# AlterPang/Multi_ORB_SLAM

Measured on AMD Instinct MI355X. Metric: frames/sec (N-cam extract+match), higher is better.
Workload: dtype u8; 1 GPU; configs[1]: one 2-cam 640x480 rig per GPU, 8-level pyramid, 1000 feat/cam; HIP FAST+rBRIEF extract + SearchByProjection + cross-camera Hamming top-2; cams_per_gpu=2, rig_cams=2, rigs=1, width=640, height=480, nfeatures=1000, nlevels=8, frame_unit=one rig timestep (2 cameras)

## Files before the change

### include/orb_debug.h

```cpp
#ifndef ORB_DEBUG_H
#define ORB_DEBUG_H
#include "orbx.h"
#include "orbm.h"
#include "orbf.h"
#include "orbv.h"
#ifdef __cplusplus
extern "C" {
#endif

int orbx_debug_candidates(orbx_extractor* ex, int cam, int level, orb_keypoint* out, int cap, int* n);
int orbx_debug_distribute_octree(const orb_keypoint* in, int n, int min_x, int max_x, int min_y, int max_y,
                                 int n_features, orb_keypoint* out, int cap, int* n_out);
int orbx_debug_last_path(const orbx_extractor* ex);
int orbx_debug_level0_in_place(const orbx_extractor* ex);
int orbx_debug_pyramid_form(const orbx_extractor* ex);
int orbx_debug_pyramid_plan(int tile_w, int tile_h, int split);

int orbm_debug_last_resolve(const orbm_matcher* m, int* out4);
#define ORBM_FORM_NONE 0
#define ORBM_FORM_HOST 1
#define ORBM_FORM_MONO2_ANG 2
#define ORBM_FORM_MONO2 3
#define ORBM_FORM_MONO4_WORKLIST 4
#define ORBM_FORM_MONO4_WAVES 5
#define ORBM_FORM_JACOBI_LDSQ 6
#define ORBM_FORM_JACOBI 7
#define ORBM_FORM_CAMS 8
#define ORBM_FORM_SWEEPS 9
int orbm_debug_last_resolve_form(const orbm_matcher* m, int* out2);
int orbm_debug_last_refresh(const orbm_matcher* m, int* out5);
int orbm_debug_last_pose(const orbm_matcher* m, int* out2);
int orbm_debug_last_sim3(const orbm_matcher* m, int* out2);
int orbm_debug_last_sim3opt(const orbm_matcher* m, int* out2);
int orbm_debug_last_pnp(const orbm_matcher* m, int* out4);
int orbm_debug_pnp_buffers(const orbm_matcher* m, unsigned long long* out3);
int orbm_debug_time_project(orbm_matcher* m, const orbm_frame* f, const orbm_query* q, int nq, int th_high, int iters,
                            float* avg_us, long long* n_gated);

int orbv_debug_last_join(const orbv_workspace* w, int* out4);

int orbf_debug_exchange_timing(orbf_frontend* f, int on);
int orbf_debug_exchange_us(const orbf_frontend* f, float* out2);
long orbf_debug_exchange_redos(const orbf_frontend* f);

#ifdef __cplusplus
}
#endif
#endif
```

### multi_orb_slam_amd/_lib.py

```python
import ctypes as C
import os
import subprocess
import numpy as np

_PKG = os.path.dirname(os.path.abspath(__file__))
CSRC = os.path.join(_PKG, "csrc")
LIB_PATH = os.environ.get("MORB_LIB_PATH") or os.path.join(_PKG, "lib", "libmorb.so")

KP_DTYPE = np.dtype([("x", "<f4"), ("y", "<f4"), ("size", "<f4"), ("angle", "<f4"), ("response", "<f4"),
                     ("octave", "<i4"), ("class_id", "<i4")])
QUERY_DTYPE = np.dtype([("u", "<f4"), ("v", "<f4"), ("radius", "<f4"), ("ur", "<f4"), ("min_level", "<i4"),
                        ("max_level", "<i4"), ("cam", "<i4"), ("blocks", "<i4"), ("angle", "<f4"),
                        ("desc", "u1", (32,))])
WINDOW_DTYPE = np.dtype([("u", "<f4"), ("v", "<f4"), ("radius", "<f4"), ("cam", "<i4"), ("min_level", "<i4"), ("max_level", "<i4")])
assert KP_DTYPE.itemsize == 28 and QUERY_DTYPE.itemsize == 68 and WINDOW_DTYPE.itemsize == 24
POINT_DTYPE = np.dtype([("pos", "<f4", (3,)), ("normal", "<f4", (3,)), ("min_dist", "<f4"), ("max_dist", "<f4"),
                        ("blocks", "<i4"), ("desc", "u1", (32,))])
TRACK_DTYPE = np.dtype([("proj_x", "<f4"), ("proj_y", "<f4"), ("proj_xr", "<f4"), ("view_cos", "<f4"), ("level", "<i4"),
                        ("in_view", "<i4")])
assert POINT_DTYPE.itemsize == 68 and TRACK_DTYPE.itemsize == 24
REFRESH_DTYPE = np.dtype([("desc", "u1", (32,)), ("normal", "<f4", (3,)), ("min_dist", "<f4"), ("max_dist", "<f4"),
                          ("best_obs", "<i4"), ("best_median", "<i4")])
assert REFRESH_DTYPE.itemsize == 60
REFRESH_DESCRIPTOR, REFRESH_NORMAL_DEPTH, REFRESH_CAP = 1, 2, 256
# ... 136 lines not shown


_lib = None


def lib():
    global _lib
    if _lib is not None:
        return _lib
    if not os.path.exists(LIB_PATH):
        raise OrbError(ORB_E_NO_DEVICE, "HIP library %s is not built (run `python -c 'import __graft_entry__ as g; "
                       "g.build()'` or `make -C multi_orb_slam_amd/csrc`); there is no CPU fallback" % LIB_PATH)
    L = C.CDLL(LIB_PATH)
    vp, i32, f32 = C.c_void_p, C.c_int, C.c_float
    L.orb_last_error.restype = C.c_char_p
    L.orbx_tables.argtypes = [vp] * 7
    L.orbx_create.argtypes = [vp, i32, i32, i32, i32, vp]
    L.orbx_destroy.argtypes = [vp]; L.orbx_destroy.restype = None
    L.orbx_extract.argtypes = [vp, i32] + [vp] * 8
    L.orbx_upload.argtypes = [vp, i32, vp, i32, i32, i32]
    L.orbx_upload_device.argtypes = [vp, i32, vp, i32, i32, i32]
    L.orbx_run.argtypes = [vp]
    L.orbx_count.argtypes = [vp, i32]
    L.orbx_download.argtypes = [vp, i32, vp, vp, i32]
    L.orbx_device_keypoints.argtypes = [vp, i32]; L.orbx_device_keypoints.restype = vp
    L.orbx_device_descriptors.argtypes = [vp, i32]; L.orbx_device_descriptors.restype = vp
    L.orbx_stream.argtypes = [vp]; L.orbx_stream.restype = vp
    L.orbx_wait_for_stream.argtypes = [vp, vp]
    L.orbx_bind_output.argtypes = [vp, i32, vp, vp, i32]
    L.orbx_debug_level.argtypes = [vp, i32, i32, vp, i32, vp, vp]
    L.orbx_debug_candidates.argtypes = [vp, i32, i32, vp, i32, vp]
    L.orbx_debug_distribute_octree.argtypes = [vp, i32, i32, i32, i32, i32, i32, vp, i32, vp]
    L.orbx_set_profiling.argtypes = [vp, i32]
    L.orbx_stage_times_us.argtypes = [vp, vp]
    L.orbm_create.argtypes = [i32, vp]
    L.orbm_destroy.argtypes = [vp]; L.orbm_destroy.restype = None
    L.orbm_stream.argtypes = [vp]; L.orbm_stream.restype = vp
    L.orbm_descriptor_distance.argtypes = [vp, vp]
    L.orbm_three_maxima.argtypes = [vp, i32, vp]; L.orbm_three_maxima.restype = None
    L.orbm_hamming_top2.argtypes = [vp, vp, i32, vp, i32, vp, vp, vp]
    L.orbm_use_matrix_cores.argtypes = [i32]
    L.orbm_use_fp4_top2.argtypes = [i32]
    L.orbm_top2_scratch_bytes.argtypes = [i32, i32]; L.orbm_top2_scratch_bytes.restype = C.c_size_t
    L.orbm_hamming_top2_device.argtypes = [vp, i32, vp, i32, vp, vp, vp, vp, vp]
    L.orbm_hamming_matrix.argtypes = [vp, vp, i32, vp, i32, vp]
    L.orbm_hamming_matrix_device.argtypes = [vp, i32, vp, i32, vp, vp]
    L.orbm_frame_create.argtypes = [vp, vp, vp]
    L.orbm_frame_create_resident.argtypes = [vp, vp, vp, vp]
    L.orbm_frame_destroy.argtypes = [vp]; L.orbm_frame_destroy.restype = None
    L.orbm_set_stream.argtypes = [vp, vp]
    L.orbm_wait_for_stream.argtypes = [vp, vp]
    L.orbm_frame_from_device.argtypes = [vp, vp, i32, f32, f32, f32, f32, f32, vp]
    L.orbm_frame_download.argtypes = [vp, vp, vp, vp, vp, vp]
    L.orbm_frame_count.argtypes = [vp]
    L.orbx_debug_last_path.argtypes = [vp]
    L.orbx_debug_level0_in_place.argtypes = [vp]
    L.orbx_debug_pyramid_form.argtypes = [vp]
    L.orbx_debug_pyramid_plan.argtypes = [i32, i32, i32]
    L.orbf_create.argtypes = [vp, i32, i32, i32, i32, vp]
    L.orbf_create_depth.argtypes = [vp, i32, i32, i32, i32, i32, vp]
    L.orbf_destroy.argtypes = [vp]; L.orbf_destroy.restype = None
    L.orbf_set_depth.argtypes = [vp, i32, vp, i32]
    L.orbf_configure.argtypes = [vp, f32, i32, i32]
    L.orbf_step.argtypes = [vp, vp, vp, i32, i32, vp]
    L.orbf_step_motion.argtypes = [vp, vp, vp, i32, vp]
    L.orbf_reset.argtypes = [vp]
    L.orbf_run_stream.argtypes = [vp, vp, i32, i32, i32, i32, vp, vp, i32, C.c_float, vp]
    L.orbf_prefetch.argtypes = [vp, vp]
    L.orbf_step_begin.argtypes = [vp, vp, vp, i32, i32, vp]
    L.orbf_step_motion_begin.argtypes = [vp, vp, vp, i32, vp]
    L.orbf_step_end.argtypes = [vp, vp]
    L.orbm_cross_top2_gathered_enqueue.argtypes = [vp, vp, i32, C.c_size_t, i32, i32, i32, vp, i32]
    L.orbm_cross_top2_gathered_collect.argtypes = [vp, vp, vp, vp, vp, vp]
    L.orbf_export_block.argtypes = [vp, vp, vp, vp]
    L.orbf_exchange_unique_id.argtypes = [vp]
    L.orbf_exchange_init.argtypes = [vp, vp, i32, i32]
    L.orbf_exchange_active.argtypes = [vp]
    L.orbf_step_motion_ahead.argtypes = [vp, vp, vp, vp, i32, i32, f32, vp, vp]
    L.orbf_ahead_depth.argtypes = [vp]
    L.orbf_exchange_placement.argtypes = [vp]
    L.orbf_debug_exchange_timing.argtypes = [vp, C.c_int]
    L.orbf_debug_exchange_us.argtypes = [vp, C.POINTER(C.c_float)]
    L.orbf_debug_exchange_redos.argtypes = [vp]; L.orbf_debug_exchange_redos.restype = C.c_long
    L.orbf_exchange_init_loopback.argtypes = [vp, i32, i32, i32]
    L.orbf_exchange_shutdown.argtypes = [vp]
    L.orbf_exchange_peer_handle_bytes.argtypes = []; L.orbf_exchange_peer_handle_bytes.restype = C.c_size_t
    L.orbf_exchange_peer_export.argtypes = [vp, i32, i32, vp]
    L.orbf_exchange_peer_open.argtypes = [vp, vp]
    L.orbf_peek_block.argtypes = [vp, vp, vp, vp, vp]
    L.orbm_cross_top2_gathered_views.argtypes = [vp, vp, vp, vp]
    L.orbm_cross_top2_gathered.argtypes = [vp, vp, i32, C.c_size_t, i32, i32, i32, vp, vp, vp, vp, vp]
    L.orbf_extractor.argtypes = [vp]; L.orbf_extractor.restype = vp
    L.orbf_matcher.argtypes = [vp]; L.orbf_matcher.restype = vp
    L.orbm_debug_last_resolve.argtypes = [vp, vp]
    L.orbm_debug_last_resolve_form.argtypes = [vp, vp]
    L.orbm_queries_from_motion.argtypes = [vp, vp, vp, vp, i32, f32, f32, f32, vp, f32, vp, vp, vp]
    L.orbm_count_ratio_accepted.argtypes = [vp, vp, i32, i32, f32]
    L.orbm_set_calibration.argtypes = [vp, vp]
    L.orbm_undistort_points.argtypes = [vp, vp, vp, i32, vp, vp]
    L.orbm_image_bounds.argtypes = [vp, i32, i32, vp]
    L.orbf_set_calibration.argtypes = [vp, vp]
    L.orbm_cross_top2.argtypes = [vp, vp, vp, vp, vp]
    L.orbm_cross_top2_blocks.argtypes = [vp, vp, vp, i32, i32, i32, vp, vp, vp]
    L.orbm_frame_grid.argtypes = [vp, vp, vp]
    L.orbm_features_in_area.argtypes = [vp, vp, i32, f32, f32, f32, i32, i32, vp, i32, vp]
    L.orbm_project_candidates.argtypes = [vp, vp, vp, i32, i32, vp, vp, vp]
    L.orbm_project_best.argtypes = [vp, vp, vp, i32, vp, i32, vp, i32, vp, vp]
    L.orbm_search_by_projection.argtypes = [vp, vp, vp, i32, vp, i32, i32, vp, vp]
    L.orbm_search_by_projection_windows.argtypes = [vp, vp, vp, vp, i32, vp, i32, i32, vp, vp]
    L.orbm_debug_time_project.argtypes = [vp, vp, vp, i32, i32, i32, vp, vp]
    L.orbm_search_by_projection_points.argtypes = [vp, vp, vp, i32, vp, f32, i32, vp, vp]
    L.orbm_points_create.argtypes = [vp, i32, vp]
    L.orbm_points_destroy.argtypes = [vp]; L.orbm_points_destroy.restype = None
    L.orbm_points_write.argtypes = [vp, vp, i32, i32, vp]
    L.orbm_points_count.argtypes = [vp]
    L.orbm_search_local_points.argtypes = [vp, vp, vp, i32, vp, vp, vp, f32, i32, vp, vp, vp, vp]
    L.orbm_level_thresholds.argtypes = [f32, i32, vp]
    L.orbm_frustum_host.argtypes = [vp, i32, vp, vp, vp, vp, vp]
    L.orbm_refresh_points.argtypes = [vp, vp, vp]
    L.orbm_refresh_points_host.argtypes = [vp, vp]
    L.orbm_debug_last_refresh.argtypes = [vp, vp]
    L.orbm_pose_optimize.argtypes = [vp, vp, i32, vp, vp, vp, vp, vp, vp, vp]
    L.orbm_pose_optimize_host.argtypes = [vp, i32, vp, vp, vp, vp, vp, i32, vp, vp]
    L.orbm_pose_optimize_resident.argtypes = [vp, vp, vp, vp, vp, vp, vp]
    L.orbm_debug_last_pose.argtypes = [vp, vp]
    L.orbm_pose_sincos.argtypes = [C.c_double, vp, vp]; L.orbm_pose_sincos.restype = None
    L.orbm_sim3_ransac.argtypes = [vp, vp, i32, vp, vp, vp, vp, vp, vp, vp, vp, vp, vp, vp]
    L.orbm_sim3_ransac_host.argtypes = [vp, i32, vp, vp, vp, vp, vp, vp, vp, vp, vp, i32, vp, vp]
    L.orbm_sim3_walk.argtypes = [vp, i32, i32, i32, i32, i32, vp]
    L.orbm_sim3_iterations.argtypes = [C.c_double, i32, i32, i32]
    L.orbm_sim3_atan2.argtypes = [C.c_double, C.c_double]; L.orbm_sim3_atan2.restype = C.c_double
    L.orbm_debug_last_sim3.argtypes = [vp, vp]
    L.orbm_sim3_optimize.argtypes = [vp, vp, i32, vp, vp, vp, vp, vp, vp, vp, vp, vp]
    L.orbm_sim3_optimize_host.argtypes = [vp, i32, vp, vp, vp, vp, vp, vp, vp, i32, vp, vp]
    L.orbm_sim3opt_exp.argtypes = [C.c_double]; L.orbm_sim3opt_exp.restype = C.c_double
    L.orbm_sim3opt_expmap.argtypes = [vp, i32, vp]
    L.orbm_sim3opt_ldlt7.argtypes = [vp, vp, vp]
    L.orbm_debug_last_sim3opt.argtypes = [vp, vp]
    L.orbm_pnp_ransac.argtypes = [vp, vp, i32, vp, vp, vp, vp, vp, vp, vp, vp, vp, vp, vp, i32]
    L.orbm_pnp_ransac_host.argtypes = [vp, i32, vp, vp, vp, vp, vp, vp, vp, vp, vp, vp, vp, i32]
    L.orbm_pnp_walk.argtypes = [vp, i32, i32, vp, vp, i32, i32, i32, i32, i32, vp]
    L.orbm_pnp_parameters.argtypes = [C.c_double, i32, i32, i32, C.c_float, i32, vp, vp]
    L.orbm_pnp_svd.argtypes = [vp, i32, i32, vp, vp, vp]
    L.orbm_pnp_qr_solve.argtypes = [vp, i32, i32, vp, vp]
    L.orbm_pnp_compute_pose.argtypes = [vp, vp, i32, vp, vp, vp, vp]; L.orbm_pnp_compute_pose.restype = C.c_double
    L.orbm_debug_last_pnp.argtypes = [vp, vp]
    L.orbm_debug_pnp_buffers.argtypes = [vp, vp]
    f64 = C.c_double
    L.orbv_create.argtypes = [i32, i32, vp, vp, vp, vp, i32, vp]
    L.orbv_load_text.argtypes = [C.c_char_p, i32, vp]
    L.orbv_destroy.argtypes = [vp]; L.orbv_destroy.restype = None
    L.orbv_info.argtypes = [vp, vp, vp, vp, vp]
    L.orbv_stream.argtypes = [vp]; L.orbv_stream.restype = vp
    L.orbv_transform.argtypes = [vp, vp, i32, i32, vp, vp, vp]
    L.orbv_transform_device.argtypes = [vp, vp, i32, i32, vp, vp, vp]
    L.orbv_bow_vectors.argtypes = [vp, vp, i32, i32, vp, vp, vp, vp, vp, vp, vp]
    L.orbv_score_l1.argtypes = [vp, vp, i32, vp, vp, i32]; L.orbv_score_l1.restype = f64
    L.orbv_workspace_create.argtypes = [i32, vp]
    L.orbv_workspace_destroy.argtypes = [vp]; L.orbv_workspace_destroy.restype = None
    L.orbv_search_by_bow.argtypes = [vp, vp, vp, i32, i32, f32, i32, vp, vp]
    L.orbv_search_for_triangulation.argtypes = [vp, vp, vp, vp, i32, i32, vp, vp]
    L.orbv_debug_last_join.argtypes = [vp, vp]
    L.orbv_keyframe_create.argtypes = [vp, vp, vp]
    L.orbv_keyframe_destroy.argtypes = [vp]; L.orbv_keyframe_destroy.restype = None
    L.orbv_keyframe_count.argtypes = [vp]
    L.orbv_keyframe_from_device.argtypes = [vp, vp, vp, i32, vp, vp]
# ... 29 lines not shown
```

### multi_orb_slam_amd/csrc/extractor.hip

```cpp
#include <algorithm>
#include <cfloat>
#include <cstdlib>
#include <chrono>
#include <atomic>
#include <cmath>
#include <condition_variable>
#include <functional>
#include <memory>
#include <mutex>
#include <thread>
#include <vector>

#include "../../include/orbx.h"
#include "../../include/orb_debug.h"
#include "octree.h"
#include "orb_common.h"
#include "frame_sink.h"

namespace {

using morb::DevBuf;

constexpr int EDGE_THRESHOLD = 19;
constexpr int MIN_BORDER = 16;
// ... 2442 lines not shown
    MORB_ARG(ex != nullptr);
    if (ex->inflight == 0) return ORB_OK;
    MORB_HIP(hipSetDevice(ex->device));
    MORB_HIP(hipEventSynchronize(ex->ev_done[(ex->run_seq - (unsigned)ex->inflight) & 1]));
    return finish_device_path(ex);
}

int orbx_finish_completed(orbx_extractor* ex) {
    MORB_ARG(ex != nullptr);
    if (ex->inflight == 0) return ORB_OK;
    return finish_device_path(ex);
}

int orbx_adopt_stream(orbx_extractor* ex, void* stream) {
    MORB_ARG(ex && stream && ex->inflight == 0);
    MORB_HIP(hipSetDevice(ex->device));
    if (ex->stream) {
        MORB_HIP(hipStreamSynchronize(ex->stream));
        if (ex->stream_owned) (void)hipStreamDestroy(ex->stream);
    }
    ex->stream = static_cast<hipStream_t>(stream); ex->stream_owned = false;
    return ORB_OK;
}

int orbx_discard(orbx_extractor* ex) {
    MORB_ARG(ex != nullptr);
    if (ex->inflight == 0) return ORB_OK;
    MORB_HIP(hipSetDevice(ex->device));
    MORB_HIP(hipEventSynchronize(ex->ev_done[(ex->run_seq - (unsigned)ex->inflight) & 1]));
    --ex->inflight;
    return ORB_OK;
}

int orbx_set_defer_done(orbx_extractor* ex, int on) {
    MORB_ARG(ex != nullptr);
    ex->defer_done = on != 0;
    return ORB_OK;
}

int orbx_record_done(orbx_extractor* ex) {
    MORB_ARG(ex && ex->inflight > 0);
    MORB_HIP(hipSetDevice(ex->device));
    MORB_HIP(hipEventRecord(ex->ev_done[(ex->run_seq - 1u) & 1u], ex->stream));
    return ORB_OK;
}

int orbx_set_inplace_level0(orbx_extractor* ex, int on) {
    MORB_ARG(ex != nullptr);
    if (ex->l0_optin != (on != 0)) { ex->l0_optin = on != 0; ex->tables_dirty = true; }
    return ORB_OK;
}

int orbx_set_pinned_ingest(orbx_extractor* ex, int on) {
    MORB_ARG(ex != nullptr);
    ex->pinned_ingest = on != 0;
    return ORB_OK;
}

int orbx_set_chain_graph(orbx_extractor* ex, int on) {
    MORB_ARG(ex != nullptr);
    ex->graph_next_run = on != 0;
    return ORB_OK;
}

int orbx_set_chain_tail(orbx_extractor* ex, orbx_tail_fn fn, void* user, int tag) {
    MORB_ARG(ex != nullptr);
    ex->tail_fn = fn; ex->tail_user = user; ex->tail_tag = tag;
    return ORB_OK;
}

int orbx_set_frame_sink(orbx_extractor* ex, const FrameSink* sink) {
    MORB_ARG(ex != nullptr && (sink == nullptr || ex->n_cams <= 4));
    if (sink) ex->sink = *sink; else memset(&ex->sink, 0, sizeof(ex->sink));
    return ORB_OK;
}

const int* orbx_device_counts(const orbx_extractor* ex) { return ex ? ex->d_n_out.p + ((ex->run_seq - 1u) & 1u) * (ex->n_cams + 1) : nullptr; }
int orbx_pending(const orbx_extractor* ex) { return ex ? ex->inflight : 0; }
int orbx_peek_status(const orbx_extractor* ex) {
    if (!ex || ex->inflight == 0) return -1;
    const unsigned oldest = (ex->run_seq - (unsigned)ex->inflight) & 1u;
    return ex->h_oct[oldest * (ex->n_cams + 1) + ex->n_cams];
}
void* orbx_done_event(const orbx_extractor* ex) { return ex ? (void*)ex->ev_done[(ex->run_seq - 1u) & 1u] : nullptr; }

static inline const L0Src* l0_table(const orbx_extractor* ex) { return ex->l0_on ? (const L0Src*)ex->d_l0.p : nullptr; }

static int launch_pyramid_fast(orbx_extractor* ex, hipStream_t st, const IngestArgs* fused = nullptr) {
    const int ML = ex->max_levels;
    if (ex->profiling) MORB_HIP(hipEventRecord(ex->ev[0], st));
    if (ex->tiled_ok) {
        PyrArgs A;
        for (int c = 0; c < 64; ++c) {
            A.src[c] = fused && c < ex->n_cams ? fused->src[c] : nullptr; A.stride[c] = fused ? fused->stride[c] : 0;
            A.tx[c] = c < ex->n_cams ? ex->pyr_tx[c] : 0; A.ty[c] = c < ex->n_cams ? ex->pyr_ty[c] : 0;
            A.w[c] = c < ex->n_cams ? (short)ex->cur_w[c] : 0; A.h[c] = c < ex->n_cams ? (short)ex->cur_h[c] : 0;
        }
        hipLaunchKernelGGL(k_pyramid_tiled<256>, dim3(ex->pyr_tx_max, ex->pyr_ty_max, ex->n_cams), dim3(256), (size_t)ex->pyr_lds, st, A,
                           (const LevelInfo*)ex->d_levels.p, ML, ex->d_pyr.p, ex->cam_pitch, (const int2*)ex->d_xtab.p,
                           (const int4*)ex->d_ytab.p, (const int4*)ex->d_pyr_sx.p, (const int4*)ex->d_pyr_sy.p, ex->pyr_tx_max, ex->pyr_ty_max,
                           ex->pyr_tab_cap, ex->pyr_tile);
    } else {
    auto level_dims = [&](int l, int* mw, int* mh) {
        *mw = 0; *mh = 0;
        if (l >= ML) return;
        for (int c = 0; c < ex->n_cams; ++c) {
            const LevelInfo& Lv = ex->levels[(size_t)c * ML + l];
            *mw = std::max(*mw, Lv.w); *mh = std::max(*mh, Lv.h);
        }
    };
    if (ex->tiled4) {
        for (int pi = 0; pi < 2; ++pi) {
            const orbx_extractor::TilePlan& P = ex->tp[pi];
            if (P.last <= P.base || P.tx_max == 0) continue;
            Tile4Args T;
            T.L = (const LevelInfo*)ex->d_levels.p; T.pyr = ex->d_pyr.p; T.cam_pitch = ex->cam_pitch; T.xgrp = (const int4*)ex->d_xgrp.p;
            T.ytab = (const int4*)ex->d_ytab.p; T.sx = (const int4*)P.d_sx.p; T.sy = (const int4*)P.d_sy.p; T.l0 = l0_table(ex);
            T.max_levels = ML; T.base = P.base; T.last = P.last; T.tw = P.tw; T.th = P.th; T.halo_x = P.halo_x; T.halo_y = P.halo_y;
            T.tx_max = P.tx_max; T.ty_max = P.ty_max; T.gcap = P.gcap; T.rcap = P.rcap;
            for (int c = 0; c < 64; ++c) { T.tx[c] = c < ex->n_cams ? P.tx[c] : 0; T.ty[c] = c < ex->n_cams ? P.ty[c] : 0; }
            if (P.threads == 512) hipLaunchKernelGGL(k_pyramid_tiled4<512>, dim3(P.tx_max, P.ty_max, ex->n_cams), dim3(512), (size_t)P.lds, st, T);
            else hipLaunchKernelGGL(k_pyramid_tiled4<256>, dim3(P.tx_max, P.ty_max, ex->n_cams), dim3(256), (size_t)P.lds, st, T);
        }
    } else
    for (int l = 1; l < ML; ++l) {
        int mw = 0, mh = 0;
        level_dims(l, &mw, &mh);
        if (mw == 0) continue;
        dim3 grid((mw + 255) / 256, (mh + 3) / 4, ex->n_cams), block(64, 4, 1);
        hipLaunchKernelGGL(k_resize, grid, block, 0, st, (const LevelInfo*)ex->d_levels.p, ML, l, ex->d_pyr.p, ex->cam_pitch,
                           (const int2*)ex->d_xtab.p, (const int4*)ex->d_ytab.p);
    }
    }
    if (ex->profiling) MORB_HIP(hipEventRecord(ex->ev[1], st));
    static const int form_env = [] { const char* e = getenv("MORB_FAST_FORM"); return e ? atoi(e) : 0; }();
    const bool throughput = form_env ? form_env == 2 : ex->total_cells >= 8192;
    if (throughput)
        hipLaunchKernelGGL((k_fast_cells<128, 8>), dim3(ex->total_cells), dim3(128), fast_cells_lds(ex->cell_h_max, ex->cell_px_max), st,
                           (const LevelInfo*)ex->d_levels.p, (const int2*)ex->d_cell_map.p, (const uint8_t*)ex->d_pyr.p, ex->cam_pitch, ML,
                           ex->d_cell_cnt.p, ex->d_cell_items.p, ex->cell_h_max, ex->cell_px_max, l0_table(ex));
    else
        hipLaunchKernelGGL((k_fast_cells<256, 4>), dim3(ex->total_cells), dim3(256), fast_cells_lds(ex->cell_h_max, ex->cell_px_max), st,
                           (const LevelInfo*)ex->d_levels.p, (const int2*)ex->d_cell_map.p, (const uint8_t*)ex->d_pyr.p, ex->cam_pitch, ML,
                           ex->d_cell_cnt.p, ex->d_cell_items.p, ex->cell_h_max, ex->cell_px_max, l0_table(ex));
    if (ex->profiling) MORB_HIP(hipEventRecord(ex->ev[2], st));
    MORB_HIP(hipGetLastError());
    return ORB_OK;
}

static int launch_tree_describe(orbx_extractor* ex, hipStream_t st, unsigned slot, const FrameSink& sink) {
    const int ML = ex->max_levels;
    int* d_h_oct = ex->d_h_oct + slot * (ex->n_cams + 1);
    MirrorArgs mir;
    mir.kps = nullptr; mir.desc = nullptr;
    if (ex->mirror_kps) { mir.kps = ex->mirror_kps; mir.desc = ex->mirror_desc; }
    for (int c = 0; c < 64; ++c) mir.base[c] = 0;
    hipLaunchKernelGGL(k_octree, dim3(ex->n_cams * ML), dim3(1024), sizeof(OctLdsR), st, (const LevelInfo*)ex->d_levels.p,
                       (const int*)ex->d_cell_cnt.p, (const uint32_t*)ex->d_cell_items.p, ex->d_sel_oct.p, ex->d_sel_cnt.p,
                       ex->d_oct_status.p, ML, ex->oct_max_keys);
    if (ex->profiling) MORB_HIP(hipEventRecord(ex->ev[4], st));
    hipLaunchKernelGGL(k_describe, dim3((ex->total_sel_slots + 3) / 4), dim3(256), 0, st, (const LevelInfo*)ex->d_levels.p, ML,
                       (const uint8_t*)ex->d_pyr.p, ex->cam_pitch, (const SelKp*)ex->d_sel_oct.p, ex->total_sel_slots,
                       (orb_keypoint* const*)ex->d_out_kps.p, (uint8_t* const*)ex->d_out_desc.p, mir,
                       SelListArgs{(const unsigned short*)ex->d_slot_blk.p, (const int*)ex->d_sel_cnt.p,
                                   (const int*)ex->d_oct_status.p, ex->d_n_out.p + slot * (ex->n_cams + 1), d_h_oct, ex->n_cams},
                       sink, l0_table(ex), (const DescribeTables*)ex->d_desc_tabs.p);
// ... 401 lines not shown
```

### multi_orb_slam_amd/csrc/frame_sink.h

```cpp
#pragma once
#include <stdint.h>
#include "../../include/orb_types.h"

struct orbx_extractor;

struct FrameSink {
    float *x, *y, *ur, *depth, *ang;
    int* oct;
    orb_keypoint* kps;
    uint32_t* desc;
    int* cell_of;
    float *h_ur, *h_depth;
    float *h_unx, *h_uny;
    orb_calibration calib;
    const float* cam_depth[4];
    int cam_depth_stride[4];
    float mbf, minX, minY, invW, invH;
};

extern "C" int orbx_set_frame_sink(orbx_extractor* ex, const FrameSink* sink);

extern "C" void* orbx_done_event(const orbx_extractor* ex);
extern "C" int orbx_peek_status(const orbx_extractor* ex);

typedef int (*orbx_tail_fn)(void* user, void* stream);
extern "C" int orbx_set_chain_tail(orbx_extractor* ex, orbx_tail_fn fn, void* user, int tag);
extern "C" int orbx_set_chain_graph(orbx_extractor* ex, int on);
extern "C" int orbx_set_defer_done(orbx_extractor* ex, int on);
extern "C" int orbx_set_pinned_ingest(orbx_extractor* ex, int on);
extern "C" int orbx_set_inplace_level0(orbx_extractor* ex, int on);
extern "C" int orbx_record_done(orbx_extractor* ex);
extern "C" int orbx_finish_completed(orbx_extractor* ex);
extern "C" int orbx_discard(orbx_extractor* ex);
extern "C" int orbx_adopt_stream(orbx_extractor* ex, void* stream);
```

### multi_orb_slam_amd/csrc/frontend.hip

```cpp
#include <algorithm>
#include <atomic>
#include <chrono>
#include <cmath>
#include <cstdarg>
#include <cstdlib>
#include <condition_variable>
#include <mutex>
#include <string>
#include <thread>
#include <vector>

#include "../../include/orbm.h"
#include "orb_common.h"
#include "frame_sink.h"
#include "matcher_internal.h"
#include <deque>
#include "../../include/orbf.h"
#include "../../include/orb_debug.h"

using namespace morb;


struct orbf_frontend {
    int device = 0, n_cams = 0, max_w = 0, max_h = 0;
// ... 10 lines not shown
    float mbf = 40.f;
    int th_high = ORBM_TH_HIGH, check_ori = 1;
    orb_calibration calib = {0, 0, 0, 0, 0, 0, 0, 0, 0};
    int cap_total = 0;
    static constexpr int NSETS = NEX + 3;
    struct ResultSet {
        PinnedBuf<orb_keypoint> kps; PinnedBuf<uint8_t> desc; PinnedBuf<float> ur, depth, unx, uny;
        CrossOut cross;
        bool cross_valid = false;
    } rs[NSETS];
    int last_flags = 0;
    int cur = 0;
    int last_set = 0;
    morb::StageBuf h_queries;
    std::vector<orbm_query> q_host;
    bool motion_on_device = true;
    PinnedBuf<int32_t> h_match;
    orbm_frame* pframe[NSETS] = {};
    int pframe_W[NSETS] = {}, pframe_H[NSETS] = {};
    struct InFlight { std::vector<orbf_image> images; std::vector<uint64_t> fp; int set = 0, W = 0, H = 0, e = 0; bool done = false; };
    std::deque<InFlight> inflight;
    std::deque<std::vector<orbf_image>> announced;
    int last_e = 0;
    bool poll_ok = true;
    static constexpr int NX = 8, NXC = 3;
    struct XSlot {
        DevBuf<uint8_t> recv, list;
        DevBuf<int32_t> gstart;
        PinnedBuf<int32_t> gcnt;
        CrossOut out;
        hipEvent_t done = nullptr, t_done = nullptr;
        long seq = -1;
        long job = 0;
        std::vector<orbf_image> images; std::vector<uint64_t> fp;
    } xs[NX];
    void* xcomm = nullptr; int xworld = 0, xrank = 0;
    void* xc[NXC + 1] = {};
    int x_placement = 0;
    long step_seq = 0, x_next = 0;
    long x_redos = 0;
    long x_spare_until = -1;
    struct XJob { long id, seq; const uint8_t* send; int rows; hipStream_t st; bool redo; };
    std::thread x_thread;
    std::mutex x_mu;
    std::condition_variable x_cv;
    std::deque<XJob> x_jobs;
    long x_pushed = 0, x_issued = 0;
    int x_rc = 0; std::string x_err;
    bool x_quit = false, x_async = false;
    long set_xseq[NEX + 3] = {-1, -1, -1, -1, -1, -1};
    bool x_timing = false; hipEvent_t ev_x[2] = {nullptr, nullptr}; float x_us[2] = {0.f, 0.f};
    bool xloop = false;
    morb::PeerComm* xpeer = nullptr;
    bool x_one_comm = false;
    bool x_broken = false;
    long x_timeout_ms = 15000;
    bool overlap_ok = true;
    int clean_steps = 0;
    struct Pending {
        bool active = false, async_path = false, fr_persistent = false, block_ready = false, cross_from_set = false, forked = false;
        long seq = 0;
        bool seq_taken = false;
        bool inline_match = false;
        bool mirror_requested = false, mirror_pending = false;
        int set = 0, e = 0, W = 0, H = 0, nq = 0, flags = 0, n = 0;
        bool ext_done = false;
        bool use_ms = false; MotionSrc ms; orbf_motion motion;
        bool from_motion = false;
        orbm_frame* fr = nullptr;
        SearchJob J{nullptr, nullptr, 0, nullptr, false, 0.f, 0, 0, 64, false};
        std::vector<orbf_image> images;
        std::vector<orbm_cam_features> cams;
        std::chrono::steady_clock::time_point t_impl, t_enqueued;
    } pending;
    hipEvent_t ev_extracted = nullptr;
    hipEvent_t ev_ready[NSETS] = {};
    hipEvent_t ev_cross[NSETS] = {};
    bool cross_pending[NSETS] = {};
    orbm_frame* last_frame = nullptr; bool last_frame_owned = false;
    int prev_n = 0;
    std::vector<int32_t> prev_cam_of;
    std::vector<float> scale_factors;
    std::chrono::steady_clock::time_point t_entry;
};

static int getenv_int(const char* name, int dflt) { const char* e = getenv(name); return e ? atoi(e) : dflt; }

static bool small_rig(const orbf_frontend* f) { return f->n_cams <= 4 && f->cap_total <= 8192 && !f->mt->host_resolve; }


int orbf_create(const orbx_params* params, int n_cams, int max_width, int max_height, int device, orbf_frontend** out) {
    return orbf_create_depth(params, n_cams, max_width, max_height, device, 0, out);
}

int orbf_create_depth(const orbx_params* params, int n_cams, int max_width, int max_height, int device, int ahead_depth, orbf_frontend** out) {
    MORB_ARG(params && out && n_cams >= 1 && n_cams <= 64 && ahead_depth >= 0 && ahead_depth <= orbf_frontend::NEX);
    orbf_frontend* f = new orbf_frontend();
    f->device = device; f->n_cams = n_cams; f->max_w = max_width; f->max_h = max_height;
    int rc = orbx_create(params, n_cams, max_width, max_height, device, &f->exs[0]);
    f->ex = f->exs[0];
    if (!rc) rc = orbx_set_inplace_level0(f->exs[0], 1);
    if (!rc) rc = orbm_create(device, &f->mt);
    if (rc) { orbf_destroy(f); return rc; }
    f->d_depth.assign(n_cams, nullptr); f->depth_stride.assign(n_cams, 0); f->counts.assign(n_cams, 0);
    { const char* pe = getenv("MORB_POLL"); f->poll_ok = !(pe && atoi(pe) == 0); }
    f->motion_on_device = getenv_int("MORB_MOTION_ON_DEVICE", 1) != 0;
    f->x_timeout_ms = std::max(1L, (long)getenv_int("MORB_EXCHANGE_TIMEOUT_MS", 15000));
    f->scale_factors.assign(params[0].nlevels, 1.f);
    if ((rc = orbx_tables(&params[0], f->scale_factors.data(), nullptr, nullptr, nullptr, nullptr, nullptr))) { orbf_destroy(f); return rc; }
    for (int c = 0; c < n_cams; ++c) { f->cam_cap.push_back(params[c].nfeatures + 4 * params[c].nlevels); f->cap_total += f->cam_cap.back(); }
    const size_t cap = (size_t)f->cap_total;
    if (hipEventCreateWithFlags(&f->ev_extracted, hipEventDisableTiming) != hipSuccess) { morb::set_error("hipEventCreate failed"); orbf_destroy(f); return ORB_E_HIP; }
    for (int k = 0; k < orbf_frontend::NSETS; ++k)
        if (hipEventCreateWithFlags(&f->ev_ready[k], hipEventDisableTiming | hipEventReleaseToSystem) != hipSuccess ||
            hipEventCreateWithFlags(&f->ev_cross[k], hipEventDisableTiming | hipEventReleaseToSystem) != hipSuccess) { morb::set_error("hipEventCreate failed"); orbf_destroy(f); return ORB_E_HIP; }
    { const int d = ahead_depth > 0 ? ahead_depth : getenv_int("MORB_AHEAD_DEPTH", 3); f->n_ex = d < 1 ? 1 : (d > orbf_frontend::NEX ? orbf_frontend::NEX : d); }
    f->params.assign(params, params + n_cams);
    for (int e = 1; e < f->n_ex && !rc; ++e) {
        rc = orbx_create(params, n_cams, max_width, max_height, device, &f->exs[e]);
        if (!rc) rc = orbx_set_inplace_level0(f->exs[e], 1);
    }
    for (int k = 0; k < orbf_frontend::NSETS && !rc; ++k)
        if ((rc = f->rs[k].kps.reserve(cap)) || (rc = f->rs[k].desc.reserve(cap * 32)) || (rc = f->rs[k].ur.reserve(cap)) ||
            (rc = f->rs[k].depth.reserve(cap)) || (rc = f->rs[k].unx.reserve(cap)) || (rc = f->rs[k].uny.reserve(cap))) break;
    if (!rc) rc = f->h_match.reserve(cap);
    if (rc) { orbf_destroy(f); return rc; }
    *out = f;
    return ORB_OK;
}

static void x_stop(orbf_frontend* f);

void orbf_destroy(orbf_frontend* f) {
    if (!f) return;
    (void)hipSetDevice(f->device);
    if (f->xcomm) (void)orbf_exchange_shutdown(f);
    x_stop(f);
    if (f->xpeer) { morb::peer_close(f->xpeer); f->xpeer = nullptr; }
    for (int i = 0; i < 2; ++i) if (f->ev_x[i]) (void)hipEventDestroy(f->ev_x[i]);
    for (auto& X : f->xs) {
        X.recv.release(); X.list.release(); X.gstart.release(); X.gcnt.release(); X.out.release();
        if (X.done) (void)hipEventDestroy(X.done);
        if (X.t_done) (void)hipEventDestroy(X.t_done);
    }
    for (int e = 0; e < orbf_frontend::NEX_ALL; ++e) if (f->exs[e]) (void)hipStreamSynchronize((hipStream_t)orbx_stream(f->exs[e]));
    if (f->mt) (void)hipStreamSynchronize(f->mt->stream);
    if (f->last_frame && f->last_frame_owned) orbm_frame_destroy(f->last_frame);
    for (int k = 0; k < orbf_frontend::NSETS; ++k) if (f->pframe[k]) orbm_frame_destroy(f->pframe[k]);
    if (f->exs[orbf_frontend::SPARE]) { orbx_destroy(f->exs[orbf_frontend::SPARE]); f->exs[orbf_frontend::SPARE] = nullptr; }
    if (f->mt) orbm_destroy(f->mt);
    for (int e = 0; e < orbf_frontend::NEX_ALL; ++e) if (f->exs[e]) orbx_destroy(f->exs[e]);
    for (int k = 0; k < orbf_frontend::NSETS; ++k) { f->rs[k].kps.release(); f->rs[k].desc.release(); f->rs[k].ur.release(); f->rs[k].depth.release(); f->rs[k].unx.release(); f->rs[k].uny.release(); f->rs[k].cross.release(); }
    f->h_queries.release(); f->h_match.release();
    if (f->ev_extracted) (void)hipEventDestroy(f->ev_extracted);
    for (int k = 0; k < orbf_frontend::NSETS; ++k) if (f->ev_ready[k]) (void)hipEventDestroy(f->ev_ready[k]);
    for (int k = 0; k < orbf_frontend::NSETS; ++k) if (f->ev_cross[k]) (void)hipEventDestroy(f->ev_cross[k]);
    delete f;
}

orbx_extractor* orbf_extractor(orbf_frontend* f) { return f ? f->ex : nullptr; }
orbm_matcher* orbf_matcher(orbf_frontend* f) { return f ? f->mt : nullptr; }

int orbf_set_depth(orbf_frontend* f, int cam, const float* d_depth, int stride_floats) {
    MORB_ARG(f && cam >= 0 && cam < f->n_cams);
    f->d_depth[cam] = d_depth; f->depth_stride[cam] = stride_floats;
    return ORB_OK;
}

static int orbf_drain(orbf_frontend* f);

int orbf_set_calibration(orbf_frontend* f, const orb_calibration* calib) {
    MORB_ARG(f != nullptr);
    int rc = orbf_drain(f);
    if (rc) return rc;
    f->announced.clear();
    if (calib) f->calib = *calib; else memset(&f->calib, 0, sizeof(f->calib));
    return orbm_set_calibration(f->mt, calib);
}

int orbf_configure(orbf_frontend* f, float mbf, int th_high, int check_orientation) {
    MORB_ARG(f && th_high >= 0 && th_high <= 256);
    f->mbf = mbf; f->th_high = th_high; f->check_ori = check_orientation ? 1 : 0;
    return ORB_OK;
}

static int orbf_step_impl(orbf_frontend* f, const orbf_image* images, const orbm_query* queries, int nq, int flags,
                          orbf_result* out, bool queries_in_pinned, const orbf_motion* motion = nullptr);
static int orbf_step_begin_impl(orbf_frontend* f, const orbf_image* images, const orbm_query* queries, int nq, int flags,
                                bool queries_in_pinned, int* block_ready, const orbf_motion* motion = nullptr);
static int orbf_step_end_impl(orbf_frontend* f, orbf_result* out);
static int orbf_drain(orbf_frontend* f);

int orbf_step(orbf_frontend* f, const orbf_image* images, const orbm_query* queries, int nq, int flags, orbf_result* out) {
    MORB_ARG(f && images && out && nq >= 0 && (nq == 0 || queries));
    f->t_entry = std::chrono::steady_clock::now();
    return orbf_step_impl(f, images, queries, nq, flags, out, false);
}

static int orbf_drain(orbf_frontend* f);

int orbf_reset(orbf_frontend* f) {
    MORB_ARG(f != nullptr);
    f->prev_n = 0; f->announced.clear(); f->overlap_ok = true;
    if (f->pending.active) {
        if (f->pending.fr && !f->pending.fr_persistent) { (void)hipStreamSynchronize(f->mt->stream); orbm_frame_destroy(f->pending.fr); }
        f->pending.active = false; f->pending.fr = nullptr;
    }
    const int rc = orbf_drain(f);
    if (f->xcomm && f->x_next > f->step_seq) f->step_seq = f->x_next;
    return rc;
}

int orbf_export_block(orbf_frontend* f, const uint8_t** d_block, size_t* block_bytes, int* cap_rows) {
    MORB_ARG(f && d_block && block_bytes && cap_rows);
    const orbm_frame* F = (f->pending.active && f->pending.fr) ? f->pending.fr : f->last_frame;
    if (!F) { morb::set_error("no step to export"); return ORB_E_ARG; }
    *d_block = F->b->d_desc.p;
    *cap_rows = F->desc_rows;
    *block_bytes = (size_t)F->desc_rows * 32 + ORBM_BLOCK_TRAILER;
    return ORB_OK;
}

int orbf_exchange_unique_id(uint8_t* out128) {
    MORB_ARG(out128 != nullptr);
    return exchange_unique_id(out128);
}

static int orbf_drain(orbf_frontend* f);
static void x_issuer_main(orbf_frontend* f);
static void x_stop(orbf_frontend* f);
static int exchange_queues(orbf_frontend* f) {
    int placement = 3;
    if (const char* e = getenv("MORB_EXCHANGE_PLACEMENT")) { if (!strcmp(e, "inline")) placement = 1; }
    if (f->x_one_comm) placement = 1;
    f->x_broken = false;
    f->x_placement = placement;
    f->mt->side_inline = true;
    f->x_next = f->step_seq;
    for (auto& X : f->xs) {
        X.seq = -1; X.job = 0;
        if (!X.done) MORB_HIP(hipEventCreateWithFlags(&X.done, hipEventDisableTiming));
    }
    f->x_rc = 0; f->x_err.clear(); f->x_pushed = f->x_issued = 0;
    f->x_async = placement == 3;
    if (f->x_async) f->x_thread = std::thread(x_issuer_main, f);
    return ORB_OK;
}

int orbf_exchange_placement(const orbf_frontend* f) { return f ? (f->xcomm ? f->x_placement : 0) : ORB_E_ARG; }

int orbf_debug_exchange_timing(orbf_frontend* f, int on) {
    MORB_ARG(f != nullptr);
    MORB_HIP(hipSetDevice(f->device));
    if (on) for (int i = 0; i < 2; ++i) if (!f->ev_x[i]) MORB_HIP(hipEventCreate(&f->ev_x[i]));
    if (on) for (auto& X : f->xs) if (!X.t_done) MORB_HIP(hipEventCreate(&X.t_done));
    f->x_timing = on != 0;
    return ORB_OK;
}
long orbf_debug_exchange_redos(const orbf_frontend* f) { return f ? f->x_redos : -1; }
int orbf_debug_exchange_us(const orbf_frontend* f, float* out2) {
    MORB_ARG(f && out2);
    out2[0] = f->x_us[0]; out2[1] = f->x_us[1];
    return ORB_OK;
}

int orbf_exchange_init(orbf_frontend* f, const uint8_t* uid128, int world, int rank) {
    MORB_ARG(f && uid128 && world >= 1 && rank >= 0 && rank < world && world * f->n_cams <= 512 && !f->xcomm);
    MORB_HIP(hipSetDevice(f->device));
    void* comm = nullptr;
    int rc = exchange_comm_init(&comm, world, uid128, rank);
    if (rc) return rc;
    f->xc[0] = comm;
    int mine = 1;
    for (int k = 1; k <= orbf_frontend::NXC; ++k) {
        (void)exchange_comm_clone(comm, world, rank, &f->xc[k]);
        if (!f->xc[k]) { mine = 0; break; }
    }
    int all = mine;
    {
        uint8_t* d = nullptr;
        bool ok = hipMalloc((void**)&d, (size_t)world + 1) == hipSuccess;
        const uint8_t v = (uint8_t)mine;
        ok = ok && hipMemcpy(d, &v, 1, hipMemcpyHostToDevice) == hipSuccess;
        hipStream_t ts = nullptr;
        ok = ok && hipStreamCreateWithFlags(&ts, hipStreamNonBlocking) == hipSuccess;
        ok = ok && exchange_allgather(comm, d, d + 1, 1, ts) == ORB_OK && hipStreamSynchronize(ts) == hipSuccess;
        if (ts) (void)hipStreamDestroy(ts);
        std::vector<uint8_t> flags(world, 0);
        ok = ok && hipMemcpy(flags.data(), d + 1, world, hipMemcpyDeviceToHost) == hipSuccess;
        if (d) (void)hipFree(d);
        if (!ok) { (void)hipGetLastError(); exchange_comm_destroy(comm); f->xc[0] = nullptr; morb::set_error("multi-GPU exchange: the ranks could not agree on their communicators"); return ORB_E_HIP; }
        for (int r = 0; r < world; ++r) all = all && flags[r];
    }
    f->x_one_comm = !all;
    if (!all) for (int k = 1; k <= orbf_frontend::NXC; ++k) { if (f->xc[k]) exchange_comm_destroy(f->xc[k]); f->xc[k] = nullptr; }
    f->xcomm = comm; f->xworld = world; f->xrank = rank;
    return exchange_queues(f);
}

size_t orbf_exchange_peer_handle_bytes(void) { return morb::peer_handle_bytes(); }

int orbf_exchange_peer_export(orbf_frontend* f, int world, int rank, uint8_t* handle_out) {
    MORB_ARG(f && handle_out && world >= 1 && world <= 64 && rank >= 0 && rank < world && world * f->n_cams <= 512 && !f->xcomm && !f->xpeer);
    MORB_HIP(hipSetDevice(f->device));
    const size_t block = (size_t)f->cap_total * 32 + ORBM_BLOCK_TRAILER;
    return morb::peer_export(&f->xpeer, world, rank, block, orbf_frontend::NX, f->x_timeout_ms, handle_out);
}

int orbf_exchange_peer_open(orbf_frontend* f, const uint8_t* handles) {
    MORB_ARG(f && handles && f->xpeer && !f->xcomm);
    MORB_HIP(hipSetDevice(f->device));
    int rc = morb::peer_open(f->xpeer, handles);
    if (rc) { morb::peer_close(f->xpeer); f->xpeer = nullptr; return rc; }
    f->xcomm = f->xpeer; f->xworld = morb::peer_world(f->xpeer); f->xrank = morb::peer_rank(f->xpeer);
    f->x_one_comm = false;
    return exchange_queues(f);
}

int orbf_exchange_active(const orbf_frontend* f) { return f && f->xcomm ? f->xworld : 0; }

int orbf_exchange_init_loopback(orbf_frontend* f, int group, int world, int rank) {
    MORB_ARG(f && world >= 1 && rank >= 0 && rank < world && world * f->n_cams <= 512 && !f->xcomm);
    MORB_HIP(hipSetDevice(f->device));
    int rc;
    for (int k = 0; k <= orbf_frontend::NXC; ++k) {
        LoopComm* C = nullptr;
        if ((rc = loop_join(group * (orbf_frontend::NXC + 1) + k, world, rank, &C))) {
            for (int j = 0; j < k; ++j) { loop_leave(static_cast<LoopComm*>(f->xc[j])); f->xc[j] = nullptr; }
            return rc;
        }
        f->xc[k] = C;
    }
    f->xcomm = f->xc[0]; f->xworld = world; f->xrank = rank; f->xloop = true;
    return exchange_queues(f);
}

int orbf_exchange_shutdown(orbf_frontend* f) {
    MORB_ARG(f != nullptr);
    x_stop(f);
    if (!f->xcomm) {
        if (f->xpeer) { (void)hipSetDevice(f->device); morb::peer_close(f->xpeer); f->xpeer = nullptr; }
        return ORB_OK;
    }
    MORB_HIP(hipSetDevice(f->device));
    if (f->x_broken && !f->xloop && !f->xpeer)
        for (int k = orbf_frontend::NXC; k >= 0; --k) if (f->xc[k]) { exchange_comm_abort(f->xc[k]); f->xc[k] = nullptr; }
    for (int e = 0; e < orbf_frontend::NEX_ALL; ++e) if (f->exs[e]) (void)hipStreamSynchronize((hipStream_t)orbx_stream(f->exs[e]));
    if (f->mt) { if (f->mt->side_stream) (void)hipStreamSynchronize(f->mt->side_stream); (void)hipStreamSynchronize(f->mt->stream); }
    if (f->xpeer) { morb::peer_close(f->xpeer); f->xpeer = nullptr; }
    else for (int k = orbf_frontend::NXC; k >= 0; --k) {
        if (!f->xc[k]) continue;
        if (f->xloop) loop_leave(static_cast<LoopComm*>(f->xc[k]));
        else exchange_comm_destroy(f->xc[k]);
        f->xc[k] = nullptr;
    }
    f->xcomm = nullptr; f->xworld = 0; f->xrank = 0; f->xloop = false; f->x_placement = 0; f->x_one_comm = false; f->x_broken = false;
    if (f->mt) f->mt->side_inline = false;
    return ORB_OK;
}

static std::vector<uint64_t> image_fingerprints(const orbf_image* images, int n);

static int exchange_calls(orbf_frontend* f, const orbf_frontend::XJob& J) {
    orbf_frontend::XSlot& X = f->xs[J.seq % orbf_frontend::NX];
    const size_t block = (size_t)J.rows * 32 + ORBM_BLOCK_TRAILER;
    int rc;
    const uint8_t* recv = X.recv.p;
    if (f->xpeer) {
        const int slot = (int)(J.seq % orbf_frontend::NX);
        rc = morb::peer_allgather(f->xpeer, slot, J.redo ? 1 : 0, (unsigned)(J.seq + 1), J.send, J.st);
        recv = morb::peer_recv(f->xpeer, slot, J.redo ? 1 : 0);
    } else {
        void* comm = f->x_one_comm ? f->xc[0] : f->xc[J.redo ? orbf_frontend::NXC : (int)(J.seq % orbf_frontend::NXC)];
        rc = f->xloop ? loop_allgather(static_cast<LoopComm*>(comm), J.send, X.recv.p, block, J.st)
                      : exchange_allgather(comm, J.send, X.recv.p, block, J.st);
    }
    if (rc) return rc;
    if ((rc = gathered_enqueue_to(J.st, recv, f->xworld, block, J.rows, f->n_cams, f->xrank, X.list.p, X.gstart.p, X.gcnt.dp, X.out))) return rc;
    if (f->x_timing && X.t_done) (void)hipEventRecord(X.t_done, J.st);
    MORB_HIP(hipEventRecord(X.done, J.st));
    return ORB_OK;
}

static void x_issuer_main(orbf_frontend* f) {
    (void)hipSetDevice(f->device);
    std::unique_lock<std::mutex> lk(f->x_mu);
    for (;;) {
        f->x_cv.wait(lk, [&] { return f->x_quit || !f->x_jobs.empty(); });
        if (f->x_jobs.empty()) return;
        const orbf_frontend::XJob J = f->x_jobs.front();
        lk.unlock();
        const int rc = f->x_rc ? f->x_rc : exchange_calls(f, J);
        lk.lock();
        if (rc && !f->x_rc) { f->x_rc = rc; f->x_err = orb_last_error(); }
        f->x_jobs.pop_front();
        f->x_issued = J.id;
        f->x_cv.notify_all();
    }
}

static int x_failed(orbf_frontend* f) {
    if (f->x_rc) morb::set_error("%s", f->x_err.c_str());
    return f->x_rc;
}
static int x_wait_job(orbf_frontend* f, long id) {
    if (!f->x_async || id <= 0) return ORB_OK;
    std::unique_lock<std::mutex> lk(f->x_mu);
    f->x_cv.wait(lk, [&] { return f->x_issued >= id; });
    return x_failed(f);
}
static int x_wait_stream(orbf_frontend* f, hipStream_t st) {
    if (!f->x_async) return ORB_OK;
    std::unique_lock<std::mutex> lk(f->x_mu);
    f->x_cv.wait(lk, [&] { for (const auto& J : f->x_jobs) if (!st || J.st == st) return false; return true; });
    return x_failed(f);
}
static void x_stop(orbf_frontend* f) {
    if (!f->x_thread.joinable()) return;
    { std::lock_guard<std::mutex> lk(f->x_mu); f->x_quit = true; f->x_cv.notify_all(); }
    f->x_thread.join();
    f->x_quit = false; f->x_async = false;
// ... 29 lines not shown
            std::string who;
            for (int r = 0; r < f->xworld; ++r) if ((miss >> r) & 1) who += (who.empty() ? "" : ", ") + std::to_string(r);
            morb::set_error("multi-GPU exchange: rank(s) %s did not deliver the %sblock of step %ld within %ld ms (MORB_EXCHANGE_TIMEOUT_MS): dead or far behind",
                            who.c_str(), redo ? "re-shipped " : "", seq, f->x_timeout_ms);
            return ORB_E_TIMEOUT;
        }
    }
    return ORB_OK;
}

static int exchange_issue(orbf_frontend* f, long seq, const orbm_frame* F, hipStream_t st, bool redo, const orbf_image* images, int set = -1) {
    orbf_frontend::XSlot& X = f->xs[seq % orbf_frontend::NX];
    const size_t block = (size_t)F->desc_rows * 32 + ORBM_BLOCK_TRAILER;
    MORB_ARG(F->desc_rows == f->cap_total);
    const int n_cams = f->xworld * f->n_cams;
    int rc;
    if ((rc = x_wait_job(f, X.job))) return rc;
    if ((!f->xpeer && (rc = X.recv.reserve((size_t)f->xworld * block))) || (rc = X.list.reserve((size_t)f->xworld * F->desc_rows * 32)) ||
        (rc = X.gstart.reserve(n_cams + 1 + 4)) || (rc = X.gcnt.reserve(n_cams + 3)) || (rc = X.out.reserve(F->desc_rows, f->xworld * F->desc_rows)))
        return rc;
    orbf_frontend::XJob J{0, seq, F->b->d_desc.p, F->desc_rows, st, redo};
    if (f->x_async) {
        std::lock_guard<std::mutex> lk(f->x_mu);
        if ((rc = x_failed(f))) return rc;
        J.id = ++f->x_pushed;
        f->x_jobs.push_back(J);
        f->x_cv.notify_all();
    } else if ((rc = exchange_calls(f, J))) return rc;
    X.job = J.id;
    if (!redo) {
        X.seq = seq;
        if (images) { X.images.assign(images, images + f->n_cams); X.fp = image_fingerprints(images, f->n_cams); }
        else { X.images.clear(); X.fp.clear(); }
        f->x_next = seq + 1;
        if (set >= 0) f->set_xseq[set] = seq;
    }
    return ORB_OK;
}

static bool same_images(const std::vector<orbf_image>& a, const orbf_image* b, int n);
static bool same_content(const std::vector<uint64_t>& fp, const orbf_image* b, int n);
static std::vector<uint64_t> image_fingerprints(const orbf_image* images, int n);

int orbf_peek_block(orbf_frontend* f, const orbf_image* images, const uint8_t** d_block, size_t* block_bytes, int* cap_rows) {
    MORB_ARG(f && images && d_block && block_bytes && cap_rows);
    *d_block = nullptr; *block_bytes = 0; *cap_rows = 0;
    if (f->pending.active || f->inflight.empty() || !same_images(f->inflight.front().images, images, f->n_cams) ||
        !same_content(f->inflight.front().fp, images, f->n_cams)) return ORB_OK;
    const orbf_frontend::InFlight& I = f->inflight.front();
    MORB_HIP(hipSetDevice(f->device));
    if (hipEventQuery(f->ev_ready[I.set]) != hipSuccess) { (void)hipGetLastError(); return ORB_OK; }
    if (orbx_peek_status(f->exs[I.e]) != 0) return ORB_OK;
    const orbm_frame* F = f->pframe[I.set];
    if (!F) return ORB_OK;
    *d_block = F->b->d_desc.p; *cap_rows = F->desc_rows; *block_bytes = (size_t)F->desc_rows * 32 + ORBM_BLOCK_TRAILER;
    return ORB_OK;
}

int orbf_export_features(orbf_frontend* f, orbf_device_features* out) {
    MORB_ARG(f && out);
    const orbm_frame* F = f->last_frame;
    if (!F || (f->pending.active && f->pending.fr)) { morb::set_error("orbf_export_features: no completed step (call it after orbf_step / orbf_step_end)"); return ORB_E_ARG; }
    memset(out, 0, sizeof(*out));
    out->n_cams = f->n_cams; out->n_total = 0;
    for (int c = 0; c < f->n_cams && c < 8; ++c) { out->counts[c] = f->counts[c]; out->n_total += f->counts[c]; }
    out->d_desc = F->b->d_desc.p; out->d_angle = F->b->d_ang.p; out->d_un_x = F->b->d_x.p; out->d_un_y = F->b->d_y.p;
    out->d_octave = F->b->d_oct.p; out->d_uright = F->b->d_ur.p;
    out->stream = f->mt->stream;
    return ORB_OK;
}

int orbf_prefetch(orbf_frontend* f, const orbf_image* next_images) {
    MORB_ARG(f && next_images);
    if ((int)(f->inflight.size() + f->announced.size()) >= f->n_ex + 1) { morb::set_error("too many future timesteps announced (at most %d beyond the next step)", f->n_ex); return ORB_E_ARG; }
    f->announced.emplace_back(next_images, next_images + f->n_cams);
    return ORB_OK;
}

int orbf_ahead_depth(const orbf_frontend* f) { return f ? f->n_ex : ORB_E_ARG; }

static void begin_failed(orbf_frontend* f) {
    if (f->pending.seq_taken && f->step_seq == f->pending.seq + 1) f->step_seq = f->pending.seq;
    f->pending.active = false; f->pending.seq_taken = false;
}

int orbf_step_begin(orbf_frontend* f, const orbf_image* images, const orbm_query* queries, int nq, int flags, int* block_ready) {
    MORB_ARG(f && images && nq >= 0 && (nq == 0 || queries));
    f->t_entry = std::chrono::steady_clock::now();
    int rc = orbf_step_begin_impl(f, images, queries, nq, flags, false, block_ready);
    if (rc) begin_failed(f);
    return rc;
}

static int queries_from_previous_step(orbf_frontend* f, const orbf_motion* motion, int* nq_out);

int orbf_step_motion_begin(orbf_frontend* f, const orbf_image* images, const orbf_motion* motion, int flags, int* block_ready) {
    MORB_ARG(f && images && motion);
    f->t_entry = std::chrono::steady_clock::now();
    int rc = orbf_step_begin_impl(f, images, nullptr, 0, flags, true, block_ready, motion);
    if (rc) begin_failed(f);
    return rc;
}

int orbf_step_end(orbf_frontend* f, orbf_result* out) {
    MORB_ARG(f && out);
    return orbf_step_end_impl(f, out);
}

static int queries_from_previous_step(orbf_frontend* f, const orbf_motion* motion, int* nq_out) {
    const int nq = f->prev_n;
    *nq_out = nq;
    if (!nq) return ORB_OK;
    int rc;
    if ((rc = f->h_queries.reserve((size_t)nq * sizeof(orbm_query)))) return rc;
    const orbf_frontend::ResultSet& R = f->rs[f->cur];
    return orbm_queries_from_motion(R.kps.p, R.desc.p, R.depth.p, f->prev_cam_of.data(), nq, motion->du, motion->dv, motion->th,
                                    f->scale_factors.data(), f->mbf, reinterpret_cast<orbm_query*>(f->h_queries.p),
                                    R.unx.p, R.uny.p);
}

int orbf_run_stream(orbf_frontend* f, const orbf_image* ring, int ring_len, int t0, int steps, int ahead, int* announced_upto,
                    const orbf_motion* motion, int th_low, float ratio, orbf_stream_stats* out) {
    MORB_ARG(f && ring && ring_len >= 1 && t0 >= 0 && steps >= 0 && ahead >= 0 && announced_upto && motion && out);
    const int ahead_max = std::min(f->n_ex + 1, (int)orbf_frontend::NEX);
    if (ahead > ahead_max) { morb::set_error("orbf_run_stream: ahead = %d, this handle takes at most %d (min(orbf_ahead_depth() + 1, 3))", ahead, ahead_max); return ORB_E_ARG; }
    memset(out, 0, sizeof(*out));
    const auto t_start = std::chrono::steady_clock::now();
    auto images_of = [&](int t) { return ring + (size_t)(t % ring_len) * f->n_cams; };
    orbf_result r;
    for (int t = t0; t < t0 + steps; ++t) {
        for (int a = std::max(*announced_upto + 1, t + 1); ahead > 0 && a <= t + ahead; ++a) {
            int rc = orbf_prefetch(f, images_of(a));
            if (rc) return rc;
            *announced_upto = a;
        }
        int rc = orbf_step_motion(f, images_of(t), motion, ORBF_NO_QUERY_RECORDS, &r);
        if (rc) return rc;
        if (*announced_upto < t) *announced_upto = t;
        const int nx = r.cross_best_dist ? orbm_count_ratio_accepted(r.cross_best_dist, r.cross_second_dist, r.n_total, th_low, ratio) : 0;
        if (nx < 0) return nx;
        out->features += r.n_total; out->temporal_matches += r.nmatches; out->cross_accepted += nx;
        uint64_t h = out->digest ^ ((uint64_t)(uint32_t)r.n_total << 40) ^ ((uint64_t)(uint32_t)r.nmatches << 20) ^ (uint64_t)(uint32_t)nx;
        h *= 0x9E3779B97F4A7C15ull; h ^= h >> 29;
        out->digest = h;
    }
    out->seconds = std::chrono::duration<double>(std::chrono::steady_clock::now() - t_start).count();
    return ORB_OK;
}

int orbf_step_motion(orbf_frontend* f, const orbf_image* images, const orbf_motion* motion, int flags, orbf_result* out) {
    MORB_ARG(f && images && motion && out);
    f->t_entry = std::chrono::steady_clock::now();
    return orbf_step_impl(f, images, nullptr, 0, flags, out, true, motion);
}

int orbf_step_motion_ahead(orbf_frontend* f, const orbf_image* images, const orbf_image* next_images, const orbf_motion* motion,
                           int flags, int th_low, float ratio, orbf_result* out, int* n_cross) {
    MORB_ARG(f && images && motion && out && n_cross);
    int rc;
    if (next_images && (rc = orbf_prefetch(f, next_images))) return rc;
    if ((rc = orbf_step_motion(f, images, motion, flags, out))) return rc;
    *n_cross = out->cross_best_dist ? orbm_count_ratio_accepted(out->cross_best_dist, out->cross_second_dist, out->n_total, th_low, ratio) : -1;
    return *n_cross < -1 ? *n_cross : ORB_OK;
}

static uint64_t image_fingerprint(const orbf_image& im) {
    if (im.generation || im.on_device || !im.data || im.width <= 0 || im.height <= 0) return 0;
    uint64_t h = 0x9E3779B97F4A7C15ull ^ ((uint64_t)im.width << 32) ^ (uint64_t)im.height;
    const int span = std::min(64, im.width);
    for (int k = 0; k < 32; ++k) {
        const int row = (int)(((long long)k * im.height) / 32);
        const int col = im.width > span ? (k * 149) % (im.width - span + 1) : 0;
        const uint8_t* p = im.data + (size_t)row * im.stride + col;
        for (int b = 0; b + 8 <= span; b += 8) { uint64_t v; memcpy(&v, p + b, 8); h = (h ^ v) * 0x9E3779B97F4A7C15ull; h ^= h >> 29; }
    }
    return h | 1;
}

static std::vector<uint64_t> image_fingerprints(const orbf_image* images, int n) {
    std::vector<uint64_t> fp(n);
    for (int c = 0; c < n; ++c) fp[c] = image_fingerprint(images[c]);
    return fp;
}

static bool same_content(const std::vector<uint64_t>& fp, const orbf_image* b, int n) {
    if ((int)fp.size() != n) return false;
    for (int c = 0; c < n; ++c) if (fp[c] != image_fingerprint(b[c])) return false;
    return true;
}

static bool same_images(const std::vector<orbf_image>& a, const orbf_image* b, int n) {
    if ((int)a.size() != n) return false;
    for (int c = 0; c < n; ++c)
        if (a[c].data != b[c].data || a[c].width != b[c].width || a[c].height != b[c].height || a[c].stride != b[c].stride ||
            (a[c].on_device != 0) != (b[c].on_device != 0) || a[c].generation != b[c].generation)
            return false;
    return true;
}


static void fill_cam_capacities(orbf_frontend* f, orbx_extractor* ex, orbm_cam_features* cams) {
    for (int c = 0; c < f->n_cams; ++c) {
        cams[c].d_kps = orbx_device_keypoints(ex, c); cams[c].d_desc = orbx_device_descriptors(ex, c);
        cams[c].n = f->cam_cap[c]; cams[c].d_depth = f->d_depth[c]; cams[c].depth_stride = f->depth_stride[c];
    }
}

static int enqueue_extract(orbf_frontend* f, int e, const orbf_image* images, int set, int* W_out, int* H_out, int* went_async,
                           bool with_cross, bool defer_events = false, bool defer_mirror = false, long seq = -1) {
    orbm_matcher* m = f->mt;
    orbx_extractor* ex = f->exs[e];
    int rc, W = 0, H = 0;
    for (int c = 0; c < f->n_cams; ++c) {
        const orbf_image& im = images[c];
        rc = im.on_device ? orbx_upload_device(ex, c, im.data, im.width, im.height, im.stride)
                          : orbx_upload(ex, c, im.data, im.width, im.height, im.stride);
        if (rc) return rc;
        W = std::max(W, im.width); H = std::max(H, im.height);
    }
    if (W == 0 || H == 0) { W = f->max_w; H = f->max_h; }
    *W_out = W; *H_out = H;
    orbf_frontend::ResultSet& R = f->rs[set];
    R.cross_valid = false;
    if (f->xcomm && (rc = x_wait_stream(f, (hipStream_t)orbx_stream(ex)))) return rc;
    if (f->xcomm && f->set_xseq[set] >= 0) {
        const orbf_frontend::XSlot& X = f->xs[f->set_xseq[set] % orbf_frontend::NX];
        if (X.seq == f->set_xseq[set]) MORB_HIP(hipStreamWaitEvent((hipStream_t)orbx_stream(ex), X.done, 0));
        f->set_xseq[set] = -1;
    }
    if ((rc = orbx_set_host_mirror(ex, defer_mirror ? nullptr : R.kps.dp, defer_mirror ? nullptr : R.desc.dp, f->cap_total))) return rc;
    *went_async = 0;
    const bool small = small_rig(f);
    std::vector<orbm_cam_features> cams(f->n_cams);
    fill_cam_capacities(f, ex, cams.data());
    float bd[4];
    if ((rc = orbm_image_bounds(&f->calib, W, H, bd))) return rc;
    if (f->pframe[set] && (f->pframe_W[set] != W || f->pframe_H[set] != H || f->pframe[set]->minX != bd[0] ||
                           f->pframe[set]->minY != bd[1] || f->pframe[set]->maxX != bd[2] || f->pframe[set]->maxY != bd[3])) {
        if (f->xcomm) {
            if ((rc = x_wait_stream(f, nullptr))) return rc;
            for (auto& X : f->xs) if (X.done && X.seq >= 0 && !f->x_broken) (void)x_wait_done(f, X, X.seq, false);
        }
        orbm_frame_destroy(f->pframe[set]); f->pframe[set] = nullptr;
    }
// ... 6 lines not shown
            rc = frame_prepare_sink(m, cams.data(), f->n_cams, f->mbf, bd[0], bd[1], bd[2], bd[3], &f->pframe[set], &sink);
            f->pframe_W[set] = W; f->pframe_H[set] = H;
        } else {
            orbm_frame* F = f->pframe[set];
            F->n_total = f->cap_total; F->counts_on_device = true; F->host_valid = false;
            rc = frame_sink_of(m, F, cams.data(), f->n_cams, f->mbf, &sink);
        }
        if (rc) return rc;
        if ((rc = orbx_set_frame_sink(ex, &sink))) return rc;
    } else {
        if (!f->pframe[set]) {
            m->frame_min_rows = f->cap_total;
            rc = frame_shell(m, f->cap_total, f->n_cams, bd[0], bd[1], bd[2], bd[3], true, &f->pframe[set]);
            m->frame_min_rows = 0;
            if (rc) return rc;
            f->pframe_W[set] = W; f->pframe_H[set] = H;
        } else {
            orbm_frame* F = f->pframe[set];
            F->n_total = f->cap_total; F->counts_on_device = true; F->host_valid = false;
        }
    }
    struct Tail {
        orbf_frontend* f; orbx_extractor* ex; orbm_cam_features* cams; const float* bd; int set; bool small, with_cross;
        int phases = 3;
        static int run(void* u, void* stream) {
            Tail& T = *static_cast<Tail*>(u);
            orbm_matcher* m = T.f->mt;
            orbf_frontend::ResultSet& R = T.f->rs[T.set];
            orbm_frame* frp = T.f->pframe[T.set];
            hipStream_t keep = m->stream;
            m->stream = (hipStream_t)stream;
            int rc = ORB_OK;
            if (T.phases & 1)
                rc = frame_from_device_impl(m, T.cams, T.f->n_cams, T.f->mbf, T.bd[0], T.bd[1], T.bd[2], T.bd[3], orbx_device_counts(T.ex),
                                            &frp, T.small);
            if (!rc && (T.phases & 2) && T.with_cross && T.f->n_cams > 1) {
                const int ncap = frp->n_total;
                rc = cross_enqueue_to(m->stream, frp->b->d_desc.p, ncap, frp->b->d_cam_start.p, T.f->n_cams, 0, ncap, frp->b->d_ntotal.p,
                                      R.cross.i.dp, R.cross.b.dp, R.cross.s.dp, R.cross.scratch.p);
            }
            m->stream = keep;
            return rc;
        }
    } tail{f, ex, cams.data(), bd, set, small, with_cross};
    const bool cross_here = with_cross && f->n_cams > 1;
    if (cross_here && (rc = R.cross.reserve(f->cap_total, f->cap_total))) return rc;
    if (small) { if ((rc = m->h_ring.reserve((64 * sizeof(CamFeat) + 65 * sizeof(int) + 64 * sizeof(int)) * 4))) return rc; }
    if (small && (rc = orbx_set_chain_tail(ex, &Tail::run, &tail, 1 + set * 2 + (cross_here ? 1 : 0)))) return rc;
    const int before = orbx_pending(ex);
    rc = orbx_run_async(ex);
    if (small) { (void)orbx_set_frame_sink(ex, nullptr); (void)orbx_set_chain_tail(ex, nullptr, nullptr, 0); }
    if (rc) return rc;
    *went_async = orbx_pending(ex) > before ? 1 : 0;
    f->cross_pending[set] = false;
    if (*went_async) {
        const bool split = !small && cross_here && !defer_events;
        if (!small) { tail.phases = split ? 1 : 3; if ((rc = Tail::run(&tail, orbx_stream(ex)))) return rc; }
        R.cross_valid = cross_here;
        if (!defer_events) {
            hipError_t he = hipEventRecord(f->ev_ready[set], (hipStream_t)orbx_stream(ex));
            if (he != hipSuccess) { morb::set_error("hipEventRecord: %s", hipGetErrorString(he)); return ORB_E_HIP; }
        }
        if (split) {
            tail.phases = 2;
            if ((rc = Tail::run(&tail, orbx_stream(ex)))) return rc;
            MORB_HIP(hipEventRecord(f->ev_cross[set], (hipStream_t)orbx_stream(ex)));
            f->cross_pending[set] = true;
        }
        if (f->xcomm && f->x_placement == 3 && seq >= 0 && seq == f->x_next && (rc = exchange_issue(f, seq, f->pframe[set], (hipStream_t)orbx_stream(ex), false, images, set)))
            return rc;
    }
    return ORB_OK;
}

static int ensure_extractor(orbf_frontend* f, int e) {
    if (f->exs[e]) return ORB_OK;
    int rc = orbx_create(f->params.data(), f->n_cams, f->max_w, f->max_h, f->device, &f->exs[e]);
    if (!rc) rc = orbx_set_inplace_level0(f->exs[e], 1);
    if (!rc && e == orbf_frontend::SPARE) rc = orbx_adopt_stream(f->exs[e], f->mt->stream);
    return rc;
}

static int orbf_drain(orbf_frontend* f) {
    MORB_HIP(hipSetDevice(f->device));
    if (f->xcomm) { const int xr = x_wait_stream(f, nullptr); if (xr) return xr; }
    if (f->xcomm && f->x_placement == 3 && !f->inflight.empty()) f->x_spare_until = std::max(f->x_spare_until, f->x_next - 1);
    if (f->xcomm && f->x_placement == 3) {
        for (const auto& I : f->inflight) MORB_HIP(hipEventSynchronize(f->ev_ready[I.set]));
    } else
    for (int e = 0; e < orbf_frontend::NEX_ALL; ++e) if (f->exs[e]) MORB_HIP(hipStreamSynchronize((hipStream_t)orbx_stream(f->exs[e])));
    MORB_HIP(hipStreamSynchronize(f->mt->stream));
    if (f->mt->side_stream) MORB_HIP(hipStreamSynchronize(f->mt->side_stream));
    for (int e = 0; e < orbf_frontend::NEX_ALL; ++e)
        while (f->exs[e] && orbx_pending(f->exs[e]) > 0) { int rc = orbx_discard(f->exs[e]); if (rc < 0) return rc; }
    f->inflight.clear();
    return ORB_OK;
}

static void next_slot(orbf_frontend* f, int* e, int* set, long seq) {
    *set = (f->last_set + 1) % orbf_frontend::NSETS;
    if (*set == f->cur) *set = (*set + 1) % orbf_frontend::NSETS;
    *e = (f->inflight.empty() || f->n_ex < 2) ? 0 : (f->last_e + 1) % f->n_ex;
    if (f->xcomm && seq <= f->x_spare_until) *e = orbf_frontend::SPARE;
    f->last_set = *set; f->last_e = *e;
}

static int step_enqueue(orbf_frontend* f, orbf_frontend::Pending& P, bool first_attempt);

static int queries_from_previous_step(orbf_frontend* f, const orbf_motion* motion, int* nq_out);

static int orbf_step_begin_impl(orbf_frontend* f, const orbf_image* images, const orbm_query* queries, int nq, int flags,
                                bool queries_in_pinned, int* block_ready, const orbf_motion* motion) {
    orbf_frontend::Pending& P = f->pending;
    MORB_ARG(!P.active);
    P = orbf_frontend::Pending();
    P.t_impl = std::chrono::steady_clock::now();
    MORB_HIP(hipSetDevice(f->device));
    orbm_matcher* m = f->mt;
    int rc, went_async = 0;
    const orbm_frame* prev_frame = f->last_frame && !f->last_frame_owned ? f->last_frame : nullptr;
    if (f->last_frame && f->last_frame_owned) orbm_frame_destroy(f->last_frame);
    f->last_frame = nullptr; f->last_frame_owned = false;
    if (f->xcomm) flags |= ORBF_SKIP_CROSS;
    P.images.assign(images, images + f->n_cams);
    P.nq = nq; P.flags = flags; P.from_motion = motion != nullptr;
    P.seq = f->step_seq++; P.seq_taken = true;
    if (f->xcomm && f->x_next > P.seq) {
        const orbf_frontend::XSlot& X = f->xs[P.seq % orbf_frontend::NX];
        if (X.seq != P.seq || !same_images(X.images, images, f->n_cams) || !same_content(X.fp, images, f->n_cams)) {
            morb::set_error("multi-GPU exchange: the images of this step differ from the ones announced for it (orbf_prefetch), whose "
                            "descriptors have been shipped to the other ranks already -- with an exchange active announcements are binding");
            return ORB_E_ARG;
        }
    }

    if (!f->inflight.empty() && same_images(f->inflight.front().images, images, f->n_cams) &&
        same_content(f->inflight.front().fp, images, f->n_cams)) {
        const orbf_frontend::InFlight& I = f->inflight.front();
        P.set = I.set; P.e = I.e; P.W = I.W; P.H = I.H; went_async = 1;
        P.ext_done = I.done;
        f->inflight.pop_front();
    } else {
        if (!f->inflight.empty()) {
            if ((rc = orbf_drain(f))) return rc;
            f->announced.clear();
        }
        if (!f->announced.empty() && same_images(f->announced.front(), images, f->n_cams)) f->announced.pop_front();
        next_slot(f, &P.e, &P.set, P.seq);
        if ((rc = ensure_extractor(f, P.e))) return rc;
        P.inline_match = small_rig(f) && !f->xcomm;
        if (P.inline_match) { (void)orbx_set_chain_graph(f->exs[P.e], 0); (void)orbx_set_defer_done(f->exs[P.e], 1); }
        P.mirror_requested = P.inline_match && !(flags & ORBF_SKIP_CROSS) && f->n_cams > 1;
        (void)orbx_set_pinned_ingest(f->exs[P.e], 1);
        rc = enqueue_extract(f, P.e, images, P.set, &P.W, &P.H, &went_async, !(flags & ORBF_SKIP_CROSS) && !P.inline_match, P.inline_match,
                             P.mirror_requested, P.seq);
        (void)orbx_set_pinned_ingest(f->exs[P.e], 0);
        P.mirror_pending = P.mirror_requested;
        if (P.inline_match) { (void)orbx_set_chain_graph(f->exs[P.e], 1); (void)orbx_set_defer_done(f->exs[P.e], 0); }
        if (rc) return rc;
        if (P.inline_match && !went_async) P.inline_match = false;
    }
    if (motion && f->motion_on_device && prev_frame && f->prev_n > 0 && prev_frame->n_total == f->prev_n &&
        prev_frame->n_cams == f->n_cams && f->scale_factors.size() <= 16) {
        const FrameBufs* B = prev_frame->b;
        nq = f->prev_n; P.nq = nq;
        P.use_ms = true; P.motion = *motion;
        P.ms = MotionSrc{B->d_x.p, B->d_y.p, B->d_depth.p, B->d_ang.p, B->d_oct.p, (const uint4*)B->d_desc.p, B->d_cam_start.p, f->n_cams,
                         {}, motion->du, motion->dv, motion->th, f->mbf, nullptr};
        for (size_t l = 0; l < f->scale_factors.size(); ++l) P.ms.scale[l] = f->scale_factors[l];
        f->q_host.resize((size_t)nq);
        queries = nullptr;
    } else if (motion) {
        if ((rc = queries_from_previous_step(f, motion, &nq))) return rc;
        queries = reinterpret_cast<const orbm_query*>(f->h_queries.p); queries_in_pinned = true;
        P.nq = nq;
    }
    if (nq && !P.use_ms) {
        if ((rc = f->h_queries.reserve((size_t)nq * sizeof(orbm_query))) || (rc = m->d_queries.reserve((size_t)nq * sizeof(orbm_query))))
            return rc;
        if (!queries_in_pinned) memcpy(f->h_queries.p, queries, (size_t)nq * sizeof(orbm_query));
        f->h_queries.publish();
    }
    P.J = SearchJob{nullptr, P.use_ms ? f->q_host.data() : reinterpret_cast<const orbm_query*>(f->h_queries.p), nq, nullptr, false, 0.f,
                    f->th_high, f->check_ori, 64, false};
    P.J.q_dev = nq && !P.use_ms ? reinterpret_cast<const orbm_query*>(f->h_queries.dp) : nullptr;
    P.J.msrc = P.use_ms ? &P.ms : nullptr;
    if (P.use_ms && (int)prev_frame->cam_start.size() == f->n_cams + 1)
    {
        for (int c = 0; c < f->n_cams; ++c) P.J.q_cam_max = std::max(P.J.q_cam_max, prev_frame->cam_start[c + 1] - prev_frame->cam_start[c]);
        P.J.q_cam_start = prev_frame->cam_start.data();
    }
    P.J.want_tags = f->poll_ok;
    if ((rc = f->h_match.reserve(std::max(f->cap_total, 1)))) return rc;
    P.async_path = went_async != 0;
    P.block_ready = false;
    if (P.async_path && !P.inline_match && (P.ext_done || hipEventQuery(f->ev_ready[P.set]) == hipSuccess)) {
        P.ext_done = true;
        P.block_ready = orbx_peek_status(f->exs[P.e]) == 0;
    } else { P.ext_done = false; (void)hipGetLastError(); }
    if ((rc = step_enqueue(f, P, true))) return rc;
    P.active = true;
    if (block_ready) *block_ready = P.block_ready ? 1 : 0;
    return ORB_OK;
}

static int step_enqueue(orbf_frontend* f, orbf_frontend::Pending& P, bool first_attempt) {
    orbm_matcher* m = f->mt;
    hipStream_t st = m->stream;
    orbx_extractor* ex = f->exs[P.e];
    hipStream_t st_e = (hipStream_t)orbx_stream(ex);
    orbf_frontend::ResultSet& R = f->rs[P.set];
    const bool do_cross = !(P.flags & ORBF_SKIP_CROSS);
    int rc;
    std::vector<orbm_cam_features>& cams = P.cams;
    cams.resize(f->n_cams);
    const bool inline_match = P.async_path && P.inline_match;
    struct StreamSwap {
        orbm_matcher* m; hipStream_t keep; bool on;
        ~StreamSwap() { if (on) m->stream = keep; }
    } swap{m, m->stream, inline_match};
    if (inline_match) { m->stream = st_e; st = st_e; }
    if (P.async_path) {
        P.fr = f->pframe[P.set]; P.fr_persistent = true;
        if (!inline_match && !P.ext_done) MORB_HIP(hipStreamWaitEvent(st, f->ev_ready[P.set], 0));
        P.n = P.fr->n_total;
    } else {
        rc = orbx_finish(ex);
        if (rc < 0) return rc;
        MORB_HIP(hipEventRecord(f->ev_extracted, st_e));
        MORB_HIP(hipStreamWaitEvent(st, f->ev_extracted, 0));
        P.n = 0;
        for (int c = 0; c < f->n_cams; ++c) {
            cams[c].d_kps = orbx_device_keypoints(ex, c); cams[c].d_desc = orbx_device_descriptors(ex, c);
            cams[c].n = orbx_count(ex, c);
            cams[c].d_depth = f->d_depth[c]; cams[c].depth_stride = f->depth_stride[c];
            P.n += cams[c].n;
        }
        m->mirror_kps = nullptr; m->mirror_desc = nullptr; m->mirror_ur = R.ur.dp; m->mirror_depth = R.depth.dp;
        m->mirror_unx = R.unx.dp; m->mirror_uny = R.uny.dp;
        m->frame_min_rows = f->cap_total;
        float bd[4];
        rc = orbm_image_bounds(&f->calib, P.W, P.H, bd);
        P.fr = nullptr;
        if (!rc) rc = frame_from_device_impl(m, cams.data(), f->n_cams, f->mbf, bd[0], bd[1], bd[2], bd[3], nullptr, &P.fr);
        m->frame_min_rows = 0;
        m->mirror_ur = nullptr; m->mirror_depth = nullptr; m->mirror_unx = nullptr; m->mirror_uny = nullptr;
        if (rc) return rc;
        P.fr_persistent = false;
    }
    orbm_frame* fr = P.fr;
    const int n = P.n;
    P.J.cur = fr; P.J.cap = 64; P.J.device_path = false;
    P.cross_from_set = do_cross && P.async_path && R.cross_valid;
    bool forked = do_cross && n > 0 && !P.cross_from_set;
    SideJob side;
    const bool fused_side = forked && inline_match && first_attempt && P.nq > 0 && P.nq <= 65535 && !m->host_resolve &&
                            morb::side_fusable(n, n);
    if (fused_side) {
        if ((rc = morb::side_reserve(m, n, n))) return rc;
        memset(&side, 0, sizeof(side));
        side.d_desc = fr->b->d_desc.p; side.n = n; side.d_cam_start = fr->b->d_cam_start.p; side.n_cams = f->n_cams;
        side.d_range = fr->b->d_ntotal.p;
        side.o_idx = m->h_c0.dp; side.o_best = m->h_c1.dp; side.o_second = m->h_c2.dp;
        side.scratch = m->d_cscratch.p;
        side.with_mirror = P.mirror_pending;
        if (P.mirror_pending && (rc = morb::frame_mirror_job(fr, R.kps.dp, R.desc.dp, R.unx.dp, R.uny.dp, R.ur.dp, R.depth.dp, &side.mirror)))
            return rc;
        P.mirror_pending = false;
        P.J.side = &side;
        forked = false;
    }
    P.forked = forked;
    hipStream_t sd = forked ? morb::side_stream(m) : nullptr;
    if (forked && !sd) { if (!P.fr_persistent) orbm_frame_destroy(fr); P.fr = nullptr; return ORB_E_HIP; }
    if (forked) {
        hipError_t fe = hipEventRecord(m->ev_fork, st);
        if (fe == hipSuccess) fe = hipStreamWaitEvent(sd, m->ev_fork, 0);
        if (fe != hipSuccess) { morb::set_error("stream fork: %s", hipGetErrorString(fe)); if (!P.fr_persistent) orbm_frame_destroy(fr); P.fr = nullptr; return ORB_E_HIP; }
    }
    const bool x_probe = f->x_timing && f->xcomm && first_attempt;
    if (x_probe) (void)hipEventRecord(f->ev_x[0], st);
    rc = search_enqueue(m, P.J, true);
    if (x_probe) (void)hipEventRecord(f->ev_x[1], st);
    if (P.mirror_pending && !forked) {
        if (!rc) rc = frame_mirror_enqueue(fr, st, R.kps.dp, R.desc.dp, R.unx.dp, R.uny.dp, R.ur.dp, R.depth.dp);
        P.mirror_pending = false;
    }
    if (forked) {
        if (!rc) rc = cross_enqueue(m, sd, fr->b->d_desc.p, n, fr->b->d_cam_start.p, f->n_cams, 0, n,
                                    P.async_path ? fr->b->d_ntotal.p : nullptr);
        if (P.mirror_pending) {
            if (!rc) rc = frame_mirror_enqueue(fr, sd, R.kps.dp, R.desc.dp, R.unx.dp, R.uny.dp, R.ur.dp, R.depth.dp);
            P.mirror_pending = false;
        }
        hipError_t je = hipEventRecord(m->ev_join, sd);
        if (je == hipSuccess) je = hipStreamWaitEvent(st, m->ev_join, 0);
        if (!rc && je != hipSuccess) { morb::set_error("stream join: %s", hipGetErrorString(je)); rc = ORB_E_HIP; }
    }
    if (inline_match && first_attempt) {
        const int rd = orbx_record_done(ex);
        hipError_t he = hipEventRecord(f->ev_ready[P.set], st);
        if (!rc && rd) rc = rd;
        if (!rc && he != hipSuccess) { morb::set_error("hipEventRecord: %s", hipGetErrorString(he)); rc = ORB_E_HIP; }
    }
    if (rc) { (void)hipStreamSynchronize(st); if (!P.fr_persistent) orbm_frame_destroy(fr); P.fr = nullptr; return rc; }
    if (first_attempt && f->xcomm && P.async_path && P.block_ready && f->x_next == P.seq) {
        if ((rc = exchange_issue(f, P.seq, fr, st, false, P.images.data()))) return rc;
        m->foreign_work = true;
    }
    while (P.async_path && first_attempt && f->overlap_ok && !f->announced.empty() && (int)f->inflight.size() < std::max(f->n_ex, 2)) {
        if (f->xcomm && P.seq + 1 + (long)f->inflight.size() <= f->x_spare_until) break;
        const int prev_e = f->inflight.empty() ? P.e : f->inflight.back().e;
        const int e2 = f->n_ex > 1 ? (prev_e + 1) % f->n_ex : 0;
        if ((rc = ensure_extractor(f, e2))) { (void)hipStreamSynchronize(st); return rc; }
        if (orbx_pending(f->exs[e2]) >= 2) break;
        int set2 = (f->last_set + 1) % orbf_frontend::NSETS;
        if (set2 == f->cur) set2 = (set2 + 1) % orbf_frontend::NSETS;
        if (set2 == P.set) set2 = (set2 + 1) % orbf_frontend::NSETS;
        int w2 = 0, h2 = 0, async2 = 0;
        rc = enqueue_extract(f, e2, f->announced.front().data(), set2, &w2, &h2, &async2, !(P.flags & ORBF_SKIP_CROSS), false, false,
                             P.seq + 1 + (long)f->inflight.size());
        if (rc) { (void)hipStreamSynchronize(st); return rc; }
        f->last_set = set2; f->last_e = e2;
        if (async2) {
            orbf_frontend::InFlight I;
            I.images = f->announced.front(); I.set = set2; I.W = w2; I.H = h2; I.e = e2;
            I.fp = image_fingerprints(I.images.data(), f->n_cams);
            f->inflight.push_back(std::move(I));
            f->announced.pop_front();
        } else {
            f->overlap_ok = false;
            f->announced.clear();
        }
    }
    P.t_enqueued = std::chrono::steady_clock::now();
    return ORB_OK;
}

static int orbf_step_end_impl(orbf_frontend* f, orbf_result* out) {
    orbf_frontend::Pending& P = f->pending;
    MORB_ARG(P.active && out);
    P.active = false;
    auto us_between = [](std::chrono::steady_clock::time_point a, std::chrono::steady_clock::time_point b) {
        return std::chrono::duration<float, std::micro>(b - a).count();
    };
    MORB_HIP(hipSetDevice(f->device));
    orbm_matcher* m = f->mt;
    orbx_extractor* ex = f->exs[P.e];
    struct StreamSwap {
        orbm_matcher* m; hipStream_t keep; bool on;
        ~StreamSwap() { if (on) m->stream = keep; }
    } swap{m, m->stream, P.async_path && P.inline_match};
    if (swap.on) m->stream = (hipStream_t)orbx_stream(ex);
    hipStream_t st = m->stream;
    orbf_frontend::ResultSet& R = f->rs[P.set];
    int rc, nmatches = 0;
    auto t_synced = P.t_impl;
    struct FillQ {
        static void run(void* ctx) {
            orbf_frontend* f = static_cast<orbf_frontend*>(ctx);
            const orbf_frontend::Pending& P = f->pending;
            const orbf_frontend::ResultSet& Rp = f->rs[f->cur];
            (void)orbm_queries_from_motion(Rp.kps.p, Rp.desc.p, Rp.depth.p, f->prev_cam_of.data(), P.nq, P.motion.du, P.motion.dv, P.motion.th,
                                           f->scale_factors.data(), f->mbf, f->q_host.data(), Rp.unx.p, Rp.uny.p);
        }
    };
    bool have_records = !P.use_ms;
    if (P.use_ms && P.nq > 0) {
        if (P.flags & ORBF_NO_QUERY_RECORDS) { P.J.q_fill = &FillQ::run; P.J.q_fill_ctx = f; }
        else { FillQ::run(f); have_records = true; }
    }
    if (!f->inflight.empty() && !f->inflight.front().done) {
        if (hipEventQuery(f->ev_ready[f->inflight.front().set]) == hipSuccess) f->inflight.front().done = true;
        else (void)hipGetLastError();
    }
    for (int attempt = 0; attempt < 2; ++attempt) {
        if (attempt == 1 && (rc = step_enqueue(f, P, false))) return rc;
        const auto t0 = std::chrono::steady_clock::now();
        hipError_t herr = hipSuccess;
        bool polled = false;
        if (f->poll_ok && P.async_path && P.J.pollable && !P.forked && !m->foreign_work) {
            volatile int32_t* flag = m->h_match.p;
            for (int spin = 0; spin < 400000; ++spin) {
                if ((*flag >> 20) == P.J.seq) { polled = true; break; }
                __builtin_ia32_pause();
            }
        }
        if (!polled) herr = hipStreamSynchronize(st);
        m->foreign_work = false;
        out->gpu_wait_us = std::chrono::duration<float, std::micro>(std::chrono::steady_clock::now() - t0).count();
        out->host_us[0] = us_between(f->t_entry, P.t_impl); out->host_us[1] = us_between(P.t_impl, P.t_enqueued); out->host_us[2] = out->gpu_wait_us;
        t_synced = std::chrono::steady_clock::now();
        if (herr != hipSuccess) {
            morb::set_error("hipStreamSynchronize: %s", hipGetErrorString(herr));
            if (!P.fr_persistent && P.fr) orbm_frame_destroy(P.fr);
            return ORB_E_HIP;
        }
        if (P.async_path) {
            rc = polled ? orbx_finish_completed(ex) : orbx_finish(ex);
            if (rc < 0) return rc;
            if (rc == 1 || rc == 2) {
                if (rc == 2 || !f->inflight.empty()) {
                    if ((rc = orbf_drain(f))) return rc;
                    f->announced.clear();
                    f->overlap_ok = false;
                    int w2, h2, a2;
                    if (f->xcomm && P.seq <= f->x_spare_until) {
                        P.e = orbf_frontend::SPARE;
                        if ((rc = ensure_extractor(f, P.e))) return rc;
                        ex = f->exs[P.e];
                    }
                    if ((rc = enqueue_extract(f, P.e, P.images.data(), P.set, &w2, &h2, &a2, false))) return rc;
                    if (a2) { rc = orbx_finish(ex); if (rc < 0) return rc; }
                }
                P.fr = nullptr; P.fr_persistent = false;
                P.async_path = false;
                P.mirror_pending = P.mirror_requested;
                f->clean_steps = 0;
                continue;
            }
            for (int c = 0; c < f->n_cams; ++c) f->counts[c] = orbx_count(ex, c);
            frame_set_counts(P.fr, f->counts.data());
            P.n = P.fr->n_total;
            if (!f->overlap_ok && ++f->clean_steps >= 3) f->overlap_ok = true;
        } else {
            for (int c = 0; c < f->n_cams; ++c) f->counts[c] = P.cams[c].n;
        }
        break;
    }
    if (!P.async_path || !f->overlap_ok) f->announced.clear();
    const int n = P.n, nq = P.nq;
    const bool do_cross = !(P.flags & ORBF_SKIP_CROSS) && n > 0;
    rc = search_finish(m, P.J, f->h_match.p, &nmatches);
    if (rc) { if (!P.fr_persistent) orbm_frame_destroy(P.fr); return rc; }
    f->last_frame = P.fr; f->last_frame_owned = !P.fr_persistent;
    f->cur = P.set;
    f->prev_n = n;
    f->prev_cam_of.resize(n);
    for (int c = 0, g = 0; c < f->n_cams; ++c)
        for (int k = 0; k < f->counts[c]; ++k) f->prev_cam_of[g++] = c;
    out->n_queries = nq;
    if (P.use_ms && (P.flags & ORBF_NO_QUERY_RECORDS)) have_records = P.J.q_fill == nullptr;
    out->queries = !P.use_ms ? reinterpret_cast<const orbm_query*>(f->h_queries.p) : (have_records && nq > 0 ? f->q_host.data() : nullptr);
    if (P.from_motion && (P.flags & ORBF_NO_QUERY_RECORDS) && !P.use_ms) out->queries = nullptr;
    out->n_cams = f->n_cams; out->n_total = n; out->counts = f->counts.data();
    out->kps = R.kps.p; out->desc = R.desc.p; out->uright = R.ur.p; out->depth = R.depth.p;
    out->un_x = R.unx.p; out->un_y = R.uny.p;
    out->nmatches = nmatches; out->match_of_feature = f->h_match.p;
    const bool from_set = P.cross_from_set && P.async_path;
    if (f->cross_pending[P.set]) {
        if (from_set && do_cross) MORB_HIP(hipEventSynchronize(f->ev_cross[P.set]));
        f->cross_pending[P.set] = false;
    }
    out->cross_best_idx = do_cross ? (from_set ? R.cross.i.p : m->h_c0.p) : nullptr;
    out->cross_best_dist = do_cross ? (from_set ? R.cross.b.p : m->h_c1.p) : nullptr;
    out->cross_second_dist = do_cross ? (from_set ? R.cross.s.p : m->h_c2.p) : nullptr;
    out->rig_cams = 0; out->rig_counts = nullptr;
    if (f->xcomm) {
        orbf_frontend::XSlot& X = f->xs[P.seq % orbf_frontend::NX];
        if (f->x_next == P.seq && (rc = exchange_issue(f, P.seq, f->last_frame, st, false, P.images.data()))) return rc;
        MORB_ARG(X.seq == P.seq);
        if ((rc = x_wait_job(f, X.job))) return rc;
        if ((rc = x_wait_done(f, X, P.seq, false))) return rc;
        const int gc = f->xworld * f->n_cams;
        if (X.gcnt.p[gc + 2] != 0) {
            if ((rc = exchange_issue(f, P.seq, f->last_frame, st, true, nullptr))) return rc;
            ++f->x_redos;
            if ((rc = x_wait_job(f, X.job))) return rc;
            if ((rc = x_wait_done(f, X, P.seq, true))) return rc;
            if (X.gcnt.p[gc + 2] != 0) { morb::set_error("multi-GPU exchange: a block shipped again is still marked unfinished"); return ORB_E_HIP; }
        }
        m->foreign_work = false;
        if (f->x_timing && f->ev_x[0] && X.t_done) {
            float a = 0.f, b = 0.f;
            if (hipEventElapsedTime(&a, f->ev_x[0], f->ev_x[1]) == hipSuccess) f->x_us[0] = a * 1000.f; else (void)hipGetLastError();
            if (hipEventElapsedTime(&b, f->ev_x[0], X.t_done) == hipSuccess) f->x_us[1] = b * 1000.f;
            else { (void)hipGetLastError(); f->x_us[1] = 0.f; }
        }
        out->cross_best_idx = X.out.i.p; out->cross_best_dist = X.out.b.p; out->cross_second_dist = X.out.s.p;
        out->rig_cams = gc; out->rig_counts = X.gcnt.p;
        if (X.gcnt.p[gc + 1] != 0) {
            morb::set_error("multi-GPU exchange: %d per-camera counts of the gathered blocks were out of range (ranks disagree on "
                            "their capacities, or a block is corrupt)", X.gcnt.p[gc + 1]);
            return ORB_E_ARG;
        }
    }
    if (f->exs[orbf_frontend::SPARE] && P.e != orbf_frontend::SPARE && P.seq > f->x_spare_until && orbx_pending(f->exs[orbf_frontend::SPARE]) == 0) {
        (void)hipStreamSynchronize((hipStream_t)orbx_stream(f->exs[orbf_frontend::SPARE]));
        orbx_destroy(f->exs[orbf_frontend::SPARE]);
        f->exs[orbf_frontend::SPARE] = nullptr;
    }
    out->host_us[3] = us_between(t_synced, std::chrono::steady_clock::now());
    return ORB_OK;
}

static int orbf_step_impl(orbf_frontend* f, const orbf_image* images, const orbm_query* queries, int nq, int flags,
                          orbf_result* out, bool queries_in_pinned, const orbf_motion* motion) {
    int rc = orbf_step_begin_impl(f, images, queries, nq, flags, queries_in_pinned, nullptr, motion);
    if (rc) { begin_failed(f); return rc; }
    return orbf_step_end_impl(f, out);
}
```

### multi_orb_slam_amd/csrc/matcher_internal.h

```cpp
#pragma once
#include <hip/hip_runtime.h>
#include <condition_variable>
#include <map>
#include <mutex>
#include <vector>
#include "../../include/orbm.h"
#include "../../include/orbx.h"
#include "orb_common.h"
#include "frame_sink.h"
#include "mirror_dev.h"

using morb::DevBuf;
using morb::PinnedBuf;

struct FrameDev {
    int n_total, n_cams;
    const int* n_total_dev;
    const float* un_x; const float* un_y; const float* uright;
    const int* octave;
    const uint4* desc;
    const int* cell_start; const int* items;
    float minX, minY, invW, invH;
};

// ... 93 lines not shown
    mutable std::vector<int32_t> octave, cell_start, items;
    mutable std::vector<float> angle;
    mutable bool host_valid = false;
    std::vector<int32_t> cam_start;
    bool camera_major = true;
    FrameDev dev() const {
        FrameDev F;
        F.n_total = n_total; F.n_cams = n_cams; F.n_total_dev = counts_on_device ? b->d_ntotal.p : nullptr; F.un_x = b->d_x.p; F.un_y = b->d_y.p; F.uright = b->d_ur.p;
        F.octave = b->d_oct.p; F.desc = (const uint4*)b->d_desc.p; F.cell_start = b->d_cell_start.p; F.items = b->d_items.p;
        F.minX = minX; F.minY = minY; F.invW = invW; F.invH = invH;
        return F;
    }
};

struct MotionSrc {
    const float* x; const float* y; const float* depth; const float* angle;
    const int* octave; const uint4* desc; const int* cam_start; int n_cams;
    float scale[16];
    float du, dv, th, mbf;
    orbm_query* rec_out;
};

struct SearchJob {
    const orbm_frame* cur; const orbm_query* q; int nq; const uint8_t* occupied;
    bool points; float nnratio; int th_high, check_ori;
    int cap; bool device_path;
    bool pollable = false;
    bool want_tags = false; int seq = 0;
    const orbm_query* q_dev = nullptr;
    const uint8_t* occ_dev = nullptr;
    const orbm_window* win2_dev = nullptr;
    const struct SideJob* side = nullptr;
    bool multi = false;
    const MotionSrc* msrc = nullptr;
    int q_cam_max = 0;
    const int* q_cam_start = nullptr;
    void (*q_fill)(void*) = nullptr; void* q_fill_ctx = nullptr;
    int form = 0;
};

struct MergeJob;
struct SideJob {
    const uint8_t* d_desc; int n; const int* d_cam_start; int n_cams; const int* d_range;
    int *o_idx, *o_best, *o_second;
    void* scratch;
    bool with_mirror; morb::MirrorJob mirror;
};

struct CrossOut {
    PinnedBuf<int32_t> i, b, s;
    DevBuf<uint8_t> scratch;
    int reserve(int nq, int n);
    void release() { i.release(); b.release(); s.release(); scratch.release(); }
};

namespace morb {
FrameBufs* take_bufs(orbm_matcher* m);
int reserve_frame(FrameBufs* b, int n, int n_cams);
int ensure_host_copies(const orbm_frame* f);
int frame_raise_lds_limit();
int frame_shell(orbm_matcher* m, int n, int n_cams, float min_x, float min_y, float max_x, float max_y, bool counts_on_device,
                orbm_frame** out);
int frame_prepare_sink(orbm_matcher* m, const orbm_cam_features* cams, int n_cams, float mbf, float min_x, float min_y,
                       float max_x, float max_y, orbm_frame** out, FrameSink* sink);
int frame_sink_of(orbm_matcher* m, orbm_frame* F, const orbm_cam_features* cams, int n_cams, float mbf, FrameSink* sink);
int frame_mirror_enqueue(orbm_frame* F, void* stream, orb_keypoint* h_kps, uint8_t* h_desc, float* h_unx, float* h_uny, float* h_ur,
                         float* h_depth);
int frame_mirror_job(orbm_frame* F, orb_keypoint* h_kps, uint8_t* h_desc, float* h_unx, float* h_uny, float* h_ur, float* h_depth,
                     MirrorJob* out);
struct ProjectArgs;
int launch_project_side(hipStream_t st, const ProjectArgs& P, const SideJob& S, struct ::MergeJob* defer_merge = nullptr);
int launch_merge(hipStream_t st, const struct ::MergeJob& M);
bool side_fusable(int nq, int n);
int side_reserve(orbm_matcher* m, int nq, int n);
int frame_from_device_impl(orbm_matcher* m, const orbm_cam_features* cams, int n_cams, float mbf, float min_x, float min_y,
                           float max_x, float max_y, const int* d_counts, orbm_frame** out, bool sink_filled = false);
void frame_set_counts(orbm_frame* F, const int* counts);
int phases_frame_build(unsigned long long* out64);
int points_view(const orbm_points* p, const orbm_matcher* m, const orbm_point** d_rows, const orbm_point** h_rows, int* count);
int search_raise_lds_limits();
int search_enqueue(orbm_matcher* m, SearchJob& J, bool queries_already_on_device = false);
int search_finish(orbm_matcher* m, SearchJob& J, int32_t* match_of_feature, int* nmatches);
int phases_resolve(unsigned long long* out64);
int cross_enqueue_to(hipStream_t st, const uint8_t* d_desc, int n, const int* d_cam_start, int n_cams, int q_off, int nq,
                     const int* d_n, int* o_idx, int* o_best, int* o_second, void* scratch);
int cross_enqueue(orbm_matcher* m, hipStream_t st, const uint8_t* d_desc, int n, const int* d_cam_start, int n_cams, int q_off,
                  int nq, const int* d_n = nullptr);
int gathered_enqueue_to(hipStream_t st, const uint8_t* d_gathered, int world, size_t block_bytes, int cap_rows, int cams_per_rank, int rank,
                        uint8_t* d_list, int* d_gstart, int* h_gcnt_dp, CrossOut& out);
struct LoopComm;
int exchange_rccl_available();
int exchange_unique_id(uint8_t* out128);
int exchange_comm_init(void** comm, int world, const uint8_t* uid128, int rank);
int exchange_comm_clone(void* comm, int world, int rank, void** out);
int exchange_comm_async_error(void* comm);
void exchange_comm_abort(void* comm);
void exchange_comm_destroy(void* comm);
int exchange_allgather(void* comm, const void* sendbuf, void* recvbuf, size_t bytes, hipStream_t st);
int loop_join(int group, int world, int rank, LoopComm** out);
void loop_leave(LoopComm* c);
int loop_allgather(LoopComm* C, const void* sendbuf, void* recvbuf, size_t bytes, hipStream_t st);
struct PeerComm;
size_t peer_handle_bytes();
int peer_world(const PeerComm* C);
int peer_rank(const PeerComm* C);
int peer_export(PeerComm** out, int world, int rank, size_t block, int nslots, long timeout_ms, uint8_t* handle);
int peer_open(PeerComm* C, const uint8_t* handles);
void peer_close(PeerComm* C);
const uint8_t* peer_recv(const PeerComm* C, int slot, int gen);
int peer_allgather(PeerComm* C, int slot, int gen, unsigned version, const void* send, hipStream_t st);
unsigned long long peer_missing(const PeerComm* C, int slot, int gen);
}
```

### multi_orb_slam_amd/csrc/search.hip

```cpp
#include <algorithm>
#include <cmath>
#include <cstdlib>
#include <type_traits>
#include <vector>

#include "../../include/orbm.h"
#include "../../include/orb_debug.h"
#include "orb_common.h"
#include "frame_sink.h"
#include "matcher_internal.h"
#include "hamming_dev.h"
#include "project_dev.h"
#include "resolve_dev.h"

using namespace morb;

namespace {
__global__ __launch_bounds__(256) void k_project(ProjectArgs A) {
    MORB_LATENCY_KERNEL_WIDE();
    const int qi = __builtin_amdgcn_readfirstlane(blockIdx.x * 4 + (threadIdx.x >> 6));
    if (qi >= A.nq) return;
    project_wave(A, qi, threadIdx.x & 63);
}

constexpr int RESOLVE_MAX_Q = 65535;
MORB_PHASE_DECL(g_ph_res);
MORB_PHASE_DECL(g_ph_chg);
#ifdef MORB_PHASE_CLOCKS
#define MORB_CHG_SLOT(it) ((it) < 15 ? (unsigned long long*)&g_ph_chg[it] : nullptr)
#else
#define MORB_CHG_SLOT(it) nullptr
#endif


template <bool POINTS, bool LDSQ>
__global__ __launch_bounds__(1024) void k_resolve(FrameDev F, const int2* __restrict__ qmeta , int nq, int cap,
                                                  const int* __restrict__ cand_idx, const uint16_t* __restrict__ cand_dist,
                                                  const int* __restrict__ cand_count, const uint8_t* __restrict__ occupied,
                                                  const float* __restrict__ f_angle, int th_high, float nnratio,
                                                  int check_ori, int max_it, int* __restrict__ choice,
                                                  const int* __restrict__ topk ,
                                                  int* __restrict__ match_of_feature, int* __restrict__ status, int tagb) {
    extern __shared__ __attribute__((aligned(16))) int s_claim[];
    __shared__ int s_hist[ORBM_HISTO_LENGTH];
    __shared__ int s_keep[3];
    __shared__ int s_red, s_nres2[2];
    const int tid = threadIdx.x, T = blockDim.x;
    const int lane = tid & 63;
    MORB_PHASE(g_ph_res, 0);
    const int NT = F.n_total_dev ? *F.n_total_dev : F.n_total;
    const int* tk_key = topk;
    const int* tk_g = topk + RESOLVE_K * nq;
    const JacobiLds L(F.n_total, nq);
    int* s_claim2 = lds_at<int>(s_claim, L.claim2());
    unsigned short* l_cnt = lds_at<unsigned short>(s_claim, L.cnt());
    int* l_choice = lds_at<int>(s_claim, L.choice());
    int* l_gd = lds_at<int>(s_claim, L.gd());
    float* l_ang = lds_at<float>(s_claim, L.ang());
    float* l_fang = lds_at<float>(s_claim, L.fang());
    unsigned char* l_fl = lds_at<unsigned char>(s_claim, L.fl());
    if (tid == 0) { s_red = 0; s_nres2[0] = 0; s_nres2[1] = 0; }
    for (int g = tid; g < F.n_total; g += T) {
        s_claim[g] = 0x7fffffff; s_claim2[g] = 0x7fffffff;
        if (LDSQ && !POINTS && check_ori) l_fang[g] = f_angle[g];
    }
    int mx = 0;
    for (int i = tid; i < nq; i += T) {
        const int cnt_i = cand_count[i];
        mx = max(mx, cnt_i);
        l_cnt[i] = (unsigned short)min(cnt_i, 65535);
        if (LDSQ) {
            l_choice[i] = -1;
            const int2 qm = qmeta[i];
            l_fl[i] = (unsigned char)((qm.x & 1) | (topk[(2 * RESOLVE_K) * nq + i] > RESOLVE_K ? 2 : 0));
            l_ang[i] = __int_as_float(qm.y);
#pragma unroll
            for (int k = 0; k < RESOLVE_K; ++k) {
                l_gd[k * nq + i] = (tk_key[k * nq + i] & 0xffff0000) | (tk_g[k * nq + i] & 0xffff);
            }
        } else {
            choice[i] = -1;
        }
    }
    mx = (int)(0x7fffffffu - wave_min_u32(0x7fffffffu - (unsigned)mx));
    if (lane == 0) atomicMax(&s_red, mx);
    __syncthreads();
    const int maxcount = s_red;
    if (maxcount > cap) {
        if (tid == 0) { status[1] = tagb | 0; status[2] = tagb | 0; status[3] = tagb | maxcount; status[0] = tagb | 2; }
        return;
    }
    MORB_PHASE(g_ph_res, 2);
    constexpr int NEED = POINTS ? 2 : 1;
    int it = 0, changed = 1;
    constexpr int RQ = LDSQ ? 2 : 4;
    int gdr[RQ][RESOLVE_K], flr[RQ], chr[RQ];
// ... 785 lines not shown
    }
    return 0;
    };
    const int code = run();
    __syncthreads();
    if (code == 0 && tid < ORBM_HISTO_LENGTH) { const int v = s_hist[tid]; if (v) atomicAdd(&state[48 + tid], v); }
    if (tid == 64 && code == 1) atomicOr(&state[8], 1);
    if (tid == 65) atomicMax(&state[6], it);
    __threadfence();
    __syncthreads();
    if (tid == 0) {
        __hip_atomic_fetch_add(&state[9], 1, __ATOMIC_ACQ_REL, __HIP_MEMORY_SCOPE_AGENT);
        int spins = 0;
        while (__hip_atomic_load(&state[9], __ATOMIC_ACQUIRE, __HIP_MEMORY_SCOPE_AGENT) < n_res && ++spins < (1 << 22)) __builtin_amdgcn_s_sleep(1);
        if (spins >= (1 << 22)) atomicOr(&state[8], 1);
        const int gmax = __hip_atomic_load(&state[0], __ATOMIC_RELAXED, __HIP_MEMORY_SCOPE_AGENT);
        s_code = gmax > cap ? 2 : (__hip_atomic_load(&state[8], __ATOMIC_RELAXED, __HIP_MEMORY_SCOPE_AGENT) ? 1 : 0);
    }
    __syncthreads();
    const int all = s_code;
    MORB_PHASE(g_ph_res, 6);
    if (all == 0) {
        int kept = 0;
        if (check_ori) {
            if (tid < 64) {
                int keep[3];
                three_maxima_wave(tid < ORBM_HISTO_LENGTH ? __hip_atomic_load(&state[48 + tid], __ATOMIC_RELAXED, __HIP_MEMORY_SCOPE_AGENT) : 0, lane, keep);
                if (tid == 0) { s_keep[0] = keep[0]; s_keep[1] = keep[1]; s_keep[2] = keep[2]; }
            }
            __syncthreads();
#pragma unroll
            for (int b = 0; b < RQ; ++b) {
                const int c = cur[b], bin = bin_of[b];
                if (c >= 0 && bin >= 0 && bin != s_keep[0] && bin != s_keep[1] && bin != s_keep[2]) { s_owner[c] = -2; --acc; }
            }
        }
        kept = __builtin_amdgcn_readlane(wave_incl_scan(acc), 63);
        if (lane == 0 && kept) atomicAdd(&state[1], kept);
        __syncthreads();
        const int NT = F.n_total_dev ? *F.n_total_dev : F.n_total;
        write_matches(match_of_feature + f0, s_owner, nf, tagb, tid, T);
        if (cam == 0) write_no_match_tail(match_of_feature, NT, F.n_total, tagb, tid, T);
    }
    __threadfence_system();
    __syncthreads();
    if (tid == 0) s_last = __hip_atomic_fetch_add(&state[10], 1, __ATOMIC_ACQ_REL, __HIP_MEMORY_SCOPE_AGENT) == n_res - 1;
    __syncthreads();
    if (!s_last) return;
    const bool merged = merge_wait(MJ, &s_code);
    if (tid == 0) {
        const int matches = __hip_atomic_load(&state[1], __ATOMIC_RELAXED, __HIP_MEMORY_SCOPE_AGENT);
        status[1] = tagb | (all ? 0 : matches); status[2] = tagb | __hip_atomic_load(&state[6], __ATOMIC_RELAXED, __HIP_MEMORY_SCOPE_AGENT);
        status[3] = tagb | __hip_atomic_load(&state[0], __ATOMIC_RELAXED, __HIP_MEMORY_SCOPE_AGENT);
        status[0] = tagb | (all ? all : (merged ? 0 : 3));
    }
    __syncthreads();
    if (tid < RS_STATE_INTS) state[tid] = 0;
    MORB_PHASE(g_ph_res, 7);
#ifdef MORB_PHASE_CLOCKS
    if (tid == 0) { g_ph_res[1] = 2; g_ph_res[62] = (unsigned long long)it; }
#endif
}

}

int morb::search_raise_lds_limits() {
    const void* fns[] = {(const void*)k_resolve<true, false>, (const void*)k_resolve<false, false>, (const void*)k_resolve<true, true>,
                         (const void*)k_resolve<false, true>, (const void*)k_resolve_mono<2, true>, (const void*)k_resolve_mono<2, false>,
                         (const void*)k_resolve_mono<4, true>, (const void*)k_resolve_mono<4, false>, (const void*)k_resolve_cams};
    for (const void* fn : fns) MORB_HIP(hipFuncSetAttribute(fn, hipFuncAttributeMaxDynamicSharedMemorySize, 150 * 1024));
    return ORB_OK;
}

int morb::phases_resolve(unsigned long long* out64) {
#ifdef MORB_PHASE_CLOCKS
    if (out64[0] == 0xC4A26Eull)
        return hipMemcpyFromSymbol(out64, HIP_SYMBOL(g_ph_chg), 64 * sizeof(unsigned long long)) == hipSuccess ? 0 : -1;
    return hipMemcpyFromSymbol(out64, HIP_SYMBOL(g_ph_res), 64 * sizeof(unsigned long long)) == hipSuccess ? 0 : -1;
#else
    (void)out64; return -1;
#endif
}

static int run_project(orbm_matcher* m, const orbm_frame* f, const orbm_query* q, int nq, int cap, int gate_right,
                       int with_dist, bool upload_queries, bool to_host, int transposed = 0,
                       const uint8_t* d_occupied = nullptr, int* d_topk = nullptr, int short_th = 256,
                       const float* d_inv_sigma2 = nullptr, const orbm_query* q_device_visible = nullptr, int2* d_qmeta = nullptr,
                       const orbm_window* d_win2 = nullptr, const SideJob* side = nullptr, const MotionSrc* msrc = nullptr,
                       bool msrc_records = false, MergeJob* defer_merge = nullptr) {
    int rc;
    if ((rc = m->d_queries.reserve((size_t)nq * sizeof(orbm_query))) || (rc = m->d_i0.reserve((size_t)nq * cap)) ||
        (rc = m->d_u16.reserve((size_t)nq * cap)) || (rc = m->d_i1.reserve(nq)))
        return rc;
    if (upload_queries)
        MORB_HIP(hipMemcpyAsync(m->d_queries.p, q, (size_t)nq * sizeof(orbm_query), hipMemcpyHostToDevice, m->stream));
    ProjectArgs A;
    A.F = f->dev(); A.q = q_device_visible ? q_device_visible : (const orbm_query*)m->d_queries.p; A.nq = nq; A.cap = cap;
    A.gate_right = gate_right; A.with_dist = with_dist; A.transposed = transposed;
    A.cand_idx = m->d_i0.p; A.cand_dist = m->d_u16.p; A.cand_count = m->d_i1.p;
    A.occupied = d_occupied; A.topk = d_topk; A.short_th = short_th; A.inv_sigma2 = d_inv_sigma2; A.qmeta = d_qmeta; A.win2 = d_win2;
    if (msrc) {
        A.from_motion = 1; A.ms = *msrc; A.q = nullptr;
        A.ms.rec_out = msrc_records ? (orbm_query*)m->d_queries.p : nullptr;
    }
    if (side) {
        if ((rc = launch_project_side(m->stream, A, *side, defer_merge))) return rc;
    } else {
        hipLaunchKernelGGL(k_project, dim3((nq + 3) / 4), dim3(256), 0, m->stream, A);
    }
    MORB_HIP(hipGetLastError());
    if (to_host) {
        if ((rc = m->h_i0.reserve((size_t)nq * cap)) || (rc = m->h_u16.reserve((size_t)nq * cap)) || (rc = m->h_i1.reserve(nq)))
            return rc;
        MORB_HIP(hipMemcpyAsync(m->h_i1.p, m->d_i1.p, (size_t)nq * 4, hipMemcpyDeviceToHost, m->stream));
        MORB_HIP(hipMemcpyAsync(m->h_i0.p, m->d_i0.p, (size_t)nq * cap * 4, hipMemcpyDeviceToHost, m->stream));
        if (with_dist) MORB_HIP(hipMemcpyAsync(m->h_u16.p, m->d_u16.p, (size_t)nq * cap * 2, hipMemcpyDeviceToHost, m->stream));
        MORB_HIP(hipStreamSynchronize(m->stream));
    }
    return ORB_OK;
}

static int project_all(orbm_matcher* m, const orbm_frame* f, const orbm_query* q, int nq, int gate_right, int with_dist,
                       int* cap_out, int cap0 = 64, const orbm_window* d_win2 = nullptr) {
    int cap = cap0;
    bool first = true;
    for (;;) {
        int rc = run_project(m, f, q, nq, cap, gate_right, with_dist, first, true, 0, nullptr, nullptr, 256, nullptr, nullptr, nullptr, d_win2);
        if (rc) return rc;
        first = false;
        int mx = 0;
        for (int i = 0; i < nq; i++) mx = std::max(mx, m->h_i1.p[i]);
        if (mx <= cap) break;
        cap = (mx + 63) & ~63;
    }
    *cap_out = cap;
    return ORB_OK;
}

int orbm_features_in_area(orbm_matcher* m, const orbm_frame* f, int cam, float x, float y, float r, int min_level,
                          int max_level, int32_t* out, int cap, int* n) {
    MORB_ARG(m && f && n && (cap == 0 || out));
    MORB_HIP(hipSetDevice(m->device));
    orbm_query Q;
    memset(&Q, 0, sizeof(Q));
    Q.u = x; Q.v = y; Q.radius = r; Q.min_level = min_level; Q.max_level = max_level; Q.cam = cam;
    int pc = 0;
    int rc = project_all(m, f, &Q, 1, 0, 0, &pc);
    if (rc) return rc;
    *n = m->h_i1.p[0];
    for (int i = 0; i < *n && i < cap; i++) out[i] = m->h_i0.p[i];
    return ORB_OK;
}

int orbm_project_candidates(orbm_matcher* m, const orbm_frame* f, const orbm_query* q, int nq, int cap_per_query,
                            int32_t* cand_idx, uint16_t* cand_dist, int32_t* cand_count) {
    MORB_ARG(m && f && nq >= 0 && cap_per_query > 0);
    if (nq == 0) return ORB_OK;
    MORB_ARG(q && cand_idx && cand_dist && cand_count);
    MORB_HIP(hipSetDevice(m->device));
    int rc = run_project(m, f, q, nq, cap_per_query, 1, 1, true, true);
    if (rc) return rc;
    bool overflow = false;
    for (int i = 0; i < nq; i++) {
        cand_count[i] = m->h_i1.p[i];
        if (cand_count[i] > cap_per_query) overflow = true;
    }
    memcpy(cand_idx, m->h_i0.p, (size_t)nq * cap_per_query * 4);
    memcpy(cand_dist, m->h_u16.p, (size_t)nq * cap_per_query * 2);
    if (overflow) { morb::set_error("candidate list longer than cap_per_query=%d", cap_per_query); return ORB_E_CAPACITY; }
    return ORB_OK;
}

int orbm_project_best(orbm_matcher* m, const orbm_frame* f, const orbm_query* q, int nq, const uint8_t* occupied, int gate,
                      const float* inv_level_sigma2, int n_levels, int32_t* best_idx, int32_t* best_dist) {
    MORB_ARG(m && f && nq >= 0 && gate >= 0 && gate <= 2);
    if (nq == 0) return ORB_OK;
    MORB_ARG(q && best_idx && best_dist);
    MORB_ARG(gate != ORBM_GATE_CHI2 || (inv_level_sigma2 && n_levels > 0 && n_levels <= 64));
    MORB_HIP(hipSetDevice(m->device));
    const int n = f->n_total;
    if (n == 0) { for (int i = 0; i < nq; ++i) { best_idx[i] = -1; best_dist[i] = 256; } return ORB_OK; }
    int rc;
    if ((rc = m->d_claim.reserve((size_t)(2 * RESOLVE_K + 1) * nq)) || (rc = m->d_occ.reserve(std::max(n, 16) + 512)) ||
        (rc = m->h_i2.reserve((size_t)2 * nq)))
        return rc;
    if (occupied) MORB_HIP(hipMemcpyAsync(m->d_occ.p, occupied, (size_t)n, hipMemcpyHostToDevice, m->stream));
    float* d_sig = nullptr;
    if (gate == ORBM_GATE_CHI2) {
        if (ensure_host_copies(f)) return ORB_E_HIP;
        for (int g = 0; g < n; ++g) MORB_ARG(f->octave[g] >= 0 && f->octave[g] < n_levels);
        d_sig = (float*)(m->d_occ.p + ((std::max(n, 16) + 15) & ~15));
// ... 6 lines not shown
    MORB_HIP(hipStreamSynchronize(m->stream));
    for (int i = 0; i < nq; ++i) {
        const int key = m->h_i2.p[i], g = m->h_i2.p[nq + i];
        best_idx[i] = g; best_dist[i] = g >= 0 ? (key >> 16) : 256;
    }
    return ORB_OK;
}

int orbm_debug_time_project(orbm_matcher* m, const orbm_frame* f, const orbm_query* q, int nq, int th_high, int iters, float* avg_us,
                            long long* n_gated) {
    MORB_ARG(m && f && q && nq > 0 && iters > 0 && avg_us && n_gated && f->n_total > 0);
    MORB_HIP(hipSetDevice(m->device));
    int rc;
    if ((rc = m->d_claim.reserve((size_t)(2 * RESOLVE_K + 1) * nq)) || (rc = m->d_qmeta.reserve(nq)) || (rc = m->h_i1.reserve(nq)))
        return rc;
    if ((rc = run_project(m, f, q, nq, 64, 1, 1, true, false, 1, nullptr, m->d_claim.p, th_high, nullptr, nullptr, m->d_qmeta.p))) return rc;
    hipEvent_t e0, e1;
    MORB_HIP(hipEventCreate(&e0)); MORB_HIP(hipEventCreate(&e1));
    MORB_HIP(hipEventRecord(e0, m->stream));
    for (int it = 0; it < iters && !rc; ++it)
        rc = run_project(m, f, q, nq, 64, 1, 1, false, false, 1, nullptr, m->d_claim.p, th_high, nullptr, nullptr, m->d_qmeta.p);
    hipError_t he = hipEventRecord(e1, m->stream);
    if (he == hipSuccess) he = hipEventSynchronize(e1);
    float ms = 0.f;
    if (he == hipSuccess) he = hipEventElapsedTime(&ms, e0, e1);
    (void)hipEventDestroy(e0); (void)hipEventDestroy(e1);
    if (rc) return rc;
    MORB_HIP(he);
    MORB_HIP(hipMemcpyAsync(m->h_i1.p, m->d_i1.p, (size_t)nq * 4, hipMemcpyDeviceToHost, m->stream));
    MORB_HIP(hipStreamSynchronize(m->stream));
    long long tot = 0;
    for (int i = 0; i < nq; ++i) tot += m->h_i1.p[i];
    *avg_us = ms * 1e3f / (float)iters; *n_gated = tot;
    return ORB_OK;
}

static int host_resolve(orbm_matcher* m, const orbm_frame* cur, const orbm_query* q, int nq, const uint8_t* occupied,
                        bool points, float nnratio, int th_high, int check_orientation, int cap0, int32_t* match_of_feature,
                        int* nmatches, const orbm_window* d_win2 = nullptr) {
    int rc = ensure_host_copies(cur);
    if (rc) return rc;
    int cap = 0;
    if ((rc = project_all(m, cur, q, nq, 1, 1, &cap, cap0, d_win2))) return rc;
    for (int g = 0; g < cur->n_total; g++) match_of_feature[g] = -1;
    std::vector<int32_t> rot[ORBM_HISTO_LENGTH];
    int nm = 0;
    for (int i = 0; i < nq; i++) {
        const int cnt = m->h_i1.p[i];
        const int32_t* ci = m->h_i0.p + (size_t)i * cap;
        const uint16_t* cd = m->h_u16.p + (size_t)i * cap;
        int best = 256, best2 = 256, lvl = -1, lvl2 = -1, bidx = -1;
        for (int k = 0; k < cnt; k++) {
            const int g = ci[k];
            const int owner = match_of_feature[g];
            if (owner >= 0 ? q[owner].blocks != 0 : (occupied && occupied[g])) continue;
            const int d = cd[k];
            if (points) {
                if (d < best) { best2 = best; best = d; lvl2 = lvl; lvl = cur->octave[g]; bidx = g; }
                else if (d < best2) { lvl2 = cur->octave[g]; best2 = d; }
            } else if (d < best) { best = d; bidx = g; }
        }
        if (best <= th_high && bidx >= 0) {
            if (points && lvl == lvl2 && (float)best > nnratio * (float)best2) continue;
            match_of_feature[bidx] = i;
            nm++;
            if (!points && check_orientation) {
                const int bin = rotation_bin(q[i].angle, cur->angle[bidx]);
                if (bin >= 0) rot[bin].push_back(bidx);
            }
        }
    }
    if (!points && check_orientation) {
        int sizes[ORBM_HISTO_LENGTH], ind[3];
        for (int b = 0; b < ORBM_HISTO_LENGTH; b++) sizes[b] = (int)rot[b].size();
        orbm_three_maxima(sizes, ORBM_HISTO_LENGTH, ind);
        for (int b = 0; b < ORBM_HISTO_LENGTH; b++)
            if (b != ind[0] && b != ind[1] && b != ind[2])
                for (int g : rot[b]) { match_of_feature[g] = -2; nm--; }
    }
    *nmatches = nm;
    return ORB_OK;
}

int morb::search_enqueue(orbm_matcher* m, SearchJob& J, bool queries_already_on_device) {
    const int n = J.cur->n_total;
    J.device_path = false; J.pollable = false; J.multi = false;
    J.form = ORBM_FORM_NONE;
    if (J.nq == 0 || n == 0) return ORB_OK;
    J.form = ORBM_FORM_HOST;
    constexpr size_t LDS_LIMIT = 150 * 1024;
    const JacobiLds jacobi(n, J.nq);
    const bool multi = jacobi.bytes(false) > LDS_LIMIT;
    if (m->host_resolve || J.nq > RESOLVE_MAX_Q) return ORB_OK;
    if (multi) { int rcg = m->d_gclaim.reserve((size_t)2 * n + RS_STATE_INTS); if (rcg) return rcg; }
    int rc;
    if ((rc = m->d_choice.reserve(J.nq)) || (rc = m->d_claim.reserve((size_t)(2 * RESOLVE_K + 1) * J.nq)) || (rc = m->d_match.reserve(n)) ||
        (rc = m->d_status.reserve(4)) || (rc = m->h_match.reserve((size_t)n + 4)) || (rc = m->d_occ.reserve(std::max(n, 16))))
        return rc;
    if (J.occupied && !J.occ_dev) MORB_HIP(hipMemcpyAsync(m->d_occ.p, J.occupied, (size_t)n, hipMemcpyHostToDevice, m->stream));
    const uint8_t* d_occ = J.occ_dev ? J.occ_dev : (J.occupied ? m->d_occ.p : nullptr);
    const orbm_frame* cur = J.cur;
    const int nq = J.nq, cap = J.cap, th_high = J.th_high;
    const float nnratio = J.nnratio;
    if ((rc = m->d_qmeta.reserve(nq))) return rc;
    const orbm_query* q_in_place = (J.q_dev && !multi) ? J.q_dev : nullptr;
    if (J.q_dev && multi && !J.msrc) {
        if ((rc = m->d_queries.reserve((size_t)nq * sizeof(orbm_query)))) return rc;
        MORB_HIP(hipMemcpyAsync(m->d_queries.p, J.q_dev, (size_t)nq * sizeof(orbm_query), hipMemcpyDefault, m->stream));
    }
    MergeJob MJ{nullptr, nullptr, nullptr, 0, 0, nullptr, nullptr, nullptr, nullptr};
    if ((rc = run_project(m, cur, J.q, nq, cap, 1, 1, !queries_already_on_device && !J.q_dev && !J.msrc, false, 1, d_occ,
                          m->d_claim.p, J.points ? 256 : th_high, nullptr, q_in_place, m->d_qmeta.p, J.win2_dev, J.side, J.msrc, multi,
                          (J.side && !multi && !J.points) ? &MJ : nullptr)))
        return rc;
    J.side = nullptr;
    J.seq = 0;
    if (J.want_tags) { m->resolve_seq = m->resolve_seq % 2047 + 1; J.seq = m->resolve_seq; }
    static const int cam_env = [] { const char* e = getenv("MORB_RS_PER_CAMERA"); return e ? atoi(e) : 1; }();
    const int cams_min_q = cam_env > 1 ? cam_env : 0x7fffffff;
    int nf_cap = 0, q_cam_max = J.q_cam_max;
    QRanges QR; QR.n = 0;
    const bool starts_ok = cur->camera_major && (int)cur->cam_start.size() == cur->n_cams + 1 && cur->cam_start[cur->n_cams] == n;
    const bool cams_want = cam_env && !J.points && !J.win2_dev && starts_ok && (multi || (cur->n_cams >= 2 && nq >= cams_min_q));
    if (cams_want) {
        for (int c = 0; c < cur->n_cams; ++c) nf_cap = std::max(nf_cap, cur->cam_start[c + 1] - cur->cam_start[c]);
        if (!q_cam_max && !J.msrc && J.q) {
            std::vector<int>& per = m->rs_cam_count;
            per.assign((size_t)cur->n_cams, 0);
            bool sorted = cur->n_cams <= 64;
            int last = 0;
            for (int i = 0; i < nq; ++i) {
                const int c = J.q[i].cam;
                if (c >= 0 && c < cur->n_cams) q_cam_max = std::max(q_cam_max, ++per[c]);
                if (c < last || c >= cur->n_cams) sorted = false; else last = c;
            }
            if (!q_cam_max) q_cam_max = 1;
            if (sorted) { QR.n = cur->n_cams; int b = 0; for (int c = 0; c < cur->n_cams; ++c) { QR.start[c] = b; b += per[c]; } QR.start[cur->n_cams] = b; }
        } else if (J.q_cam_start && cur->n_cams <= 64 && J.q_cam_start[cur->n_cams] == nq) {
            QR.n = cur->n_cams;
            for (int c = 0; c <= cur->n_cams; ++c) QR.start[c] = J.q_cam_start[c];
        }
    }
    const size_t lds_cam = CamsLds(nf_cap, RSC_RQ * 1024).bytes();
    const bool cams_fit = cams_want && nf_cap > 0 && q_cam_max > 0 && q_cam_max <= RSC_RQ * 1024 && nq < 65536 && lds_cam <= LDS_LIMIT;
    auto launch_cams = [&](MergeJob MJc, int merge_blocks) -> int {
        int rcl;
        if (!m->d_rsync.p) {
            if ((rcl = m->d_rsync.reserve(RS_STATE_INTS))) return rcl;
            MORB_HIP(hipMemsetAsync(m->d_rsync.p, 0, RS_STATE_INTS * sizeof(int), m->stream));
        }
        hipLaunchKernelGGL(k_resolve_cams, dim3(cur->n_cams + merge_blocks), dim3(1024), lds_cam, m->stream, cur->dev(), (const int*)cur->b->d_cam_start.p,
                           (const int2*)m->d_qmeta.p, nq, cap, nf_cap, (const int*)m->d_i0.p, (const uint16_t*)m->d_u16.p,
                           (const int*)m->d_i1.p, d_occ, (const float*)cur->b->d_ang.p, th_high, J.check_ori, 4096,
                           (const int*)m->d_claim.p, m->d_rsync.p, m->h_match.dp + 4, m->h_match.dp, J.seq << 20, cur->n_cams, MJc, QR);
        MORB_HIP(hipGetLastError());
        return ORB_OK;
    };
    if (multi) {
        int* tab0 = m->d_gclaim.p; int* tab1 = tab0 + n; int* state = tab1 + n;
        if (!cams_fit) MORB_HIP(hipMemsetAsync(state, 0, RS_STATE_INTS * sizeof(int), m->stream));
        const int nb_all = (std::max(n, nq) + 255) / 256, nb_q = (nq + 255) / 256, nb_f = (n + 255) / 256;
        if (cams_fit) {
            if ((rc = launch_cams(MergeJob{nullptr, nullptr, nullptr, 0, 0, nullptr, nullptr, nullptr, nullptr}, 0))) return rc;
            J.device_path = true; J.form = ORBM_FORM_CAMS;
            J.pollable = J.seq != 0;
            return ORB_OK;
        }
        J.seq = 0;
        const int n_sweeps = std::min(RS_MAX_SWEEPS, std::max(12, m->rs_sweeps_hint));
        hipLaunchKernelGGL(k_rs_init, dim3(nb_all), dim3(256), 0, m->stream, n, nq, tab0, tab1, m->d_match.p, m->d_choice.p,
                           (const int*)m->d_i1.p, state, n_sweeps);
        J.multi = true;
        const auto sweep = J.points ? k_rs_sweep<true> : k_rs_sweep<false>;
        for (int it = 0; it < n_sweeps; ++it) {
            const int* rd = (it & 1) ? tab1 : tab0;
            int* wr = (it & 1) ? tab0 : tab1;
            hipLaunchKernelGGL(sweep, dim3(nb_q), dim3(256), 0, m->stream, cur->dev(), (const orbm_query*)m->d_queries.p, nq,
                               cap, it, (const int*)m->d_i0.p, (const uint16_t*)m->d_u16.p, (const int*)m->d_i1.p, d_occ, th_high,
                               nnratio, m->d_choice.p, (const int*)m->d_claim.p, rd, wr, state);
        }
        const int ori = J.points ? 0 : J.check_ori;
        hipLaunchKernelGGL(k_rs_owner, dim3(nb_q), dim3(256), 0, m->stream, (const orbm_query*)m->d_queries.p, nq, cap,
                           (const int*)m->d_choice.p, (const float*)cur->b->d_ang.p, ori, m->d_match.p, state);
        if (ori)
            hipLaunchKernelGGL(k_rs_reject, dim3(nb_q), dim3(256), 0, m->stream, (const orbm_query*)m->d_queries.p, nq, cap,
                               (const int*)m->d_choice.p, (const float*)cur->b->d_ang.p, m->d_match.p, state);
        hipLaunchKernelGGL(k_rs_write, dim3(nb_f), dim3(256), 0, m->stream, n, cur->dev().n_total_dev, cap, (const int*)m->d_match.p,
                           (const int*)state, m->h_match.dp + 4, m->h_match.dp);
        MORB_HIP(hipGetLastError());
        J.device_path = true; J.form = ORBM_FORM_SWEEPS;
        return ORB_OK;
    }
    const bool ldsq = jacobi.bytes(true) <= LDS_LIMIT && n < 65535;
    const size_t lds_use = jacobi.bytes(ldsq);
#define MORB_RESOLVE_LAUNCH(PT, LQ)                                                                                      \
    hipLaunchKernelGGL((k_resolve<PT, LQ>), dim3(1), dim3(1024), lds_use, m->stream, cur->dev(), (const int2*)m->d_qmeta.p, \
                       nq, cap, (const int*)m->d_i0.p, (const uint16_t*)m->d_u16.p, (const int*)m->d_i1.p, d_occ,            \
                       (const float*)cur->b->d_ang.p, th_high, nnratio, J.points ? 0 : J.check_ori, 256, m->d_choice.p,      \
                       (const int*)m->d_claim.p, m->h_match.dp + 4, m->h_match.dp, J.seq << 20)
    static const int mono_mode = [] { const char* e = getenv("MORB_RESOLVE_MONO"); return e ? atoi(e) : 2; }();
    const bool mono_env = mono_mode != 0;
    const int mono_worklist = mono_mode == 2 && nq > 2048 ? 1 : 0;
    const bool will_mono = !J.points && mono_env && n < 65535 && MonoLds(n, nq, false).bytes() <= LDS_LIMIT;
    if (MJ.S > 1 && !will_mono && !cams_fit) { if ((rc = launch_merge(m->stream, MJ))) return rc; MJ.S = 0; }
    int merge_blocks = 0;
    auto carry_merge = [&]() -> int {
        merge_blocks = MJ.S > 1 ? (MJ.nq + 1023) / 1024 : 0;
        if (!merge_blocks) return ORB_OK;
        int rcm = m->d_mergecnt.reserve(4);
        if (rcm) return rcm;
        if (!m->merge_ready) { MORB_HIP(hipMemsetAsync(m->d_mergecnt.p, 0, 16, m->stream)); m->merge_ready = true; m->merge_target = 0; }
        m->merge_target += (unsigned)merge_blocks;
        MJ.done = reinterpret_cast<unsigned*>(m->d_mergecnt.p); MJ.target = m->merge_target;
        return ORB_OK;
    };
    if (cams_fit) {
        if ((rc = carry_merge()) || (rc = launch_cams(MJ, merge_blocks))) return rc;
        MJ.S = 0;
        J.form = ORBM_FORM_CAMS;
    } else if (will_mono) {
        const bool ang = MonoLds(n, nq, true).bytes() <= LDS_LIMIT;
        const size_t ml = MonoLds(n, nq, ang).bytes();
#define MORB_MONO_LAUNCH(RQ_, ANG_)                                                                                                       \
        hipLaunchKernelGGL((k_resolve_mono<RQ_, ANG_>), dim3(1 + merge_blocks), dim3(1024), ml, m->stream, cur->dev(), (const int2*)m->d_qmeta.p, nq, cap, \
                           (const int*)m->d_i0.p, (const uint16_t*)m->d_u16.p, (const int*)m->d_i1.p, d_occ,                                \
                           (const float*)cur->b->d_ang.p, th_high, J.check_ori, 4096, (const int*)m->d_claim.p, m->h_match.dp + 4,          \
                           m->h_match.dp, J.seq << 20, MJ, mono_worklist)
        if ((rc = carry_merge())) return rc;
        if (nq <= 2048) { if (ang) MORB_MONO_LAUNCH(2, true); else MORB_MONO_LAUNCH(2, false); }
        else { if (ang) MORB_MONO_LAUNCH(4, true); else MORB_MONO_LAUNCH(4, false); }
        MJ.S = 0;
        J.form = nq <= 2048 ? (ang ? ORBM_FORM_MONO2_ANG : ORBM_FORM_MONO2) : (mono_worklist ? ORBM_FORM_MONO4_WORKLIST : ORBM_FORM_MONO4_WAVES);
#undef MORB_MONO_LAUNCH
    } else if (ldsq) { if (J.points) MORB_RESOLVE_LAUNCH(true, true); else MORB_RESOLVE_LAUNCH(false, true); J.form = ORBM_FORM_JACOBI_LDSQ; }
    else { if (J.points) MORB_RESOLVE_LAUNCH(true, false); else MORB_RESOLVE_LAUNCH(false, false); J.form = ORBM_FORM_JACOBI; }
#undef MORB_RESOLVE_LAUNCH
    MORB_HIP(hipGetLastError());
    J.device_path = true;
    J.pollable = J.seq != 0;
    return ORB_OK;
}

int morb::search_finish(orbm_matcher* m, SearchJob& J, int32_t* match_of_feature, int* nmatches) {
    const int n = J.cur->n_total;
    *nmatches = 0;
    m->last_form[0] = J.device_path ? J.form : (J.nq == 0 || n == 0 ? ORBM_FORM_NONE : ORBM_FORM_HOST); m->last_form[1] = 0;
    if (J.nq == 0 || n == 0) { for (int g = 0; g < n; g++) match_of_feature[g] = -1; return ORB_OK; }
    if (!J.device_path) {
        m->last_status[0] = -1; m->last_status[1] = 0; m->last_status[2] = 0; m->last_status[3] = 0;
    }
    auto need_q = [&] { if (J.q_fill) { J.q_fill(J.q_fill_ctx); J.q_fill = nullptr; } };
    if (!J.device_path) {
        need_q();
        return host_resolve(m, J.cur, J.q, J.nq, J.occupied, J.points, J.nnratio, J.th_high, J.check_ori, 64, match_of_feature, nmatches, J.win2_dev);
    }
    bool synced = false;
    auto word = [&](int idx, int bias) -> int {
        volatile int32_t* p = m->h_match.p + idx;
        if (!J.seq) return *p;
        for (int spin = 0;; ++spin) {
            const int w = *p;
            if ((w >> 20) == J.seq) return (w & 0xfffff) - bias;
            if (spin > 100000 && !synced) { (void)hipStreamSynchronize(m->stream); synced = true; spin = 0; }
            else if (spin > 100000) return -3;
            __builtin_ia32_pause();
        }
    };
    for (;;) {
        const int status = word(0, 0);
        m->last_status[0] = status;
        for (int k = 1; k < 4; ++k) m->last_status[k] = word(k, 0);
        if (status == -3) { morb::set_error("resolve results never arrived"); return ORB_E_HIP; }
        if (J.multi) m->rs_sweeps_hint = status == 0 ? m->last_status[2] + 4 : RS_MAX_SWEEPS;
        if (status != 0 && !synced) { MORB_HIP(hipStreamSynchronize(m->stream)); synced = true; }
        if (status == 0 || status == 3) { m->last_status[0] = 0; break; }
        if (status == 2) {
            J.cap = (m->last_status[3] + 63) & ~63;
            int rc = search_enqueue(m, J, true);
            if (rc) return rc;
            m->last_form[0] = J.form; m->last_form[1]++;
            MORB_HIP(hipStreamSynchronize(m->stream));
            synced = true;
            continue;
        }
        need_q();
        m->last_form[0] = ORBM_FORM_HOST;
        return host_resolve(m, J.cur, J.q, J.nq, J.occupied, J.points, J.nnratio, J.th_high, J.check_ori, J.cap, match_of_feature, nmatches, J.win2_dev);
    }
    if (J.seq) {
        for (int g = 0; g < n; ++g) {
            const int v = word(4 + g, 2);
            if (v == -3) { morb::set_error("resolve results never arrived"); return ORB_E_HIP; }
            match_of_feature[g] = v;
        }
    } else if (match_of_feature != m->h_match.p + 4) memcpy(match_of_feature, m->h_match.p + 4, (size_t)n * 4);
    *nmatches = m->last_status[1];
    return ORB_OK;
}

static int search_common(orbm_matcher* m, const orbm_frame* cur, const orbm_query* q, int nq, const uint8_t* occupied,
                         bool points, float nnratio, int th_high, int check_orientation, int32_t* match_of_feature,
                         int* nmatches, const orbm_window* second = nullptr) {
    SearchJob J{cur, q, nq, occupied, points, nnratio, th_high, check_orientation, 64, false};
    int rc;
    if (second && nq > 0) {
        if ((rc = m->d_win2.reserve(nq))) return rc;
        MORB_HIP(hipMemcpyAsync(m->d_win2.p, second, (size_t)nq * sizeof(orbm_window), hipMemcpyHostToDevice, m->stream));
        MORB_HIP(hipStreamSynchronize(m->stream));
        J.win2_dev = m->d_win2.p;
    }
    if (nq > 0 && cur->n_total > 0 && !m->host_resolve && nq <= RESOLVE_MAX_Q) {
        const size_t qbytes = ((size_t)nq * sizeof(orbm_query) + 255) & ~(size_t)255, obytes = occupied ? (size_t)cur->n_total : 0;
        if ((rc = m->stage_q.reserve(qbytes + obytes + 16))) return rc;
        memcpy(m->stage_q.p, q, (size_t)nq * sizeof(orbm_query));
        if (occupied) memcpy(m->stage_q.p + qbytes, occupied, obytes);
        m->stage_q.publish();
        J.q_dev = reinterpret_cast<const orbm_query*>(m->stage_q.dp);
        J.occ_dev = occupied ? m->stage_q.dp + qbytes : nullptr;
    }
    rc = search_enqueue(m, J);
    if (rc) return rc;
    if (J.device_path) MORB_HIP(hipStreamSynchronize(m->stream));
    return search_finish(m, J, match_of_feature, nmatches);
}

int orbm_search_by_projection(orbm_matcher* m, const orbm_frame* cur, const orbm_query* q, int nq,
                              const uint8_t* occupied, int th_high, int check_orientation, int32_t* match_of_feature,
                              int* nmatches) {
    MORB_ARG(m && cur && nq >= 0 && nmatches && (cur->n_total == 0 || match_of_feature) && (nq == 0 || q));
    MORB_HIP(hipSetDevice(m->device));
    return search_common(m, cur, q, nq, occupied, false, 0.f, th_high, check_orientation, match_of_feature, nmatches);
}

int orbm_search_by_projection_windows(orbm_matcher* m, const orbm_frame* cur, const orbm_query* q, const orbm_window* second, int nq,
                                      const uint8_t* occupied, int th_high, int check_orientation, int32_t* match_of_feature,
                                      int* nmatches) {
    MORB_ARG(m && cur && nq >= 0 && nmatches && (cur->n_total == 0 || match_of_feature) && (nq == 0 || (q && second)));
    MORB_HIP(hipSetDevice(m->device));
    return search_common(m, cur, q, nq, occupied, false, 0.f, th_high, check_orientation, match_of_feature, nmatches, second);
}

int orbm_search_by_projection_points(orbm_matcher* m, const orbm_frame* cur, const orbm_query* q, int nq,
                                     const uint8_t* occupied, float nnratio, int th_high, int32_t* match_of_feature,
                                     int* nmatches) {
    MORB_ARG(m && cur && nq >= 0 && nmatches && (cur->n_total == 0 || match_of_feature) && (nq == 0 || q));
    MORB_HIP(hipSetDevice(m->device));
    std::vector<orbm_query> q0(q, q + nq);
    for (auto& Q : q0) Q.cam = 0;
    return search_common(m, cur, q0.data(), nq, occupied, true, nnratio, th_high, 0, match_of_feature, nmatches);
}
```

### multi_orb_slam_amd/frontend.py

```python
import ctypes as C
import numpy as np
from . import _lib
from ._lib import KP_DTYPE, QUERY_DTYPE, FImage, FMotion, FResult, Params, check, ptr

SKIP_CROSS = 1
NO_QUERY_RECORDS = 2


def _view(addr, dtype, count, shape=None):
    if not addr or count == 0:
        return np.zeros(0 if shape is None else (0,) + tuple(shape[1:]), dtype)
    nbytes = count * np.dtype(dtype).itemsize * (int(np.prod(shape[1:])) if shape is not None else 1)
    buf = (C.c_char * nbytes).from_address(addr)
    a = np.frombuffer(buf, dtype=dtype)
    return a.reshape(shape) if shape is not None else a


class _LazyStep(dict):
    _LAZY = ("counts", "rig_counts", "host_us", "cross_dist_ptrs", "kps", "desc", "uright", "depth", "un_x", "un_y", "match_of_feature", "cross")

    def __init__(self, scalars, fe, nq):
        super().__init__(scalars)
        self._fe = fe; self._seq = fe._step_seq; self._nq = nq

# ... 83 lines not shown
            c = Calibration(*(list(calib) + [0.0] * (9 - len(calib))))
            check(_lib.lib().orbf_set_calibration(self._h, C.byref(c)))

    def configure(self, mbf=40.0, th_high=100, check_orientation=True):
        check(_lib.lib().orbf_configure(self._h, mbf, th_high, int(check_orientation)))

    @property
    def extractor_handle(self):
        return _lib.lib().orbf_extractor(self._h)

    @property
    def matcher_handle(self):
        return _lib.lib().orbf_matcher(self._h)

    def reset(self):
        check(_lib.lib().orbf_reset(self._h))

    @staticmethod
    def _fill(dst, images):
        keep = []
        for c, im in enumerate(images):
            if isinstance(im, np.ndarray):
                im = np.ascontiguousarray(im, np.uint8); keep.append(im)
                dst[c] = FImage(im.ctypes.data, im.shape[1], im.shape[0], im.strides[0], 0, 0)
            elif im is None:
                dst[c] = FImage(None, 0, 0, 0, 0, 0)
            else:
                dst[c] = FImage(im[0], im[1], im[2], im[3], 1 if (len(im) < 5 or im[4]) else 0, im[5] if len(im) > 5 else 0)
        return keep

    def export_block(self):
        p = C.c_void_p(); nb = C.c_size_t(); rows = C.c_int()
        check(_lib.lib().orbf_export_block(self._h, C.byref(p), C.byref(nb), C.byref(rows)))
        return p.value, nb.value, rows.value

    def exchange_unique_id(self):
        buf = (C.c_uint8 * 128)()
        check(_lib.lib().orbf_exchange_unique_id(buf))
        return bytes(buf)

    def exchange_init(self, uid, world, rank):
        buf = (C.c_uint8 * 128).from_buffer_copy(uid)
        check(_lib.lib().orbf_exchange_init(self._h, buf, world, rank))

    def exchange_init_loopback(self, group, world, rank):
        check(_lib.lib().orbf_exchange_init_loopback(self._h, group, world, rank))

    def exchange_peer_export(self, world, rank):
        n = int(_lib.lib().orbf_exchange_peer_handle_bytes())
        buf = (C.c_uint8 * n)()
        check(_lib.lib().orbf_exchange_peer_export(self._h, world, rank, buf))
        return bytes(buf)

    def exchange_peer_open(self, handles):
        blob = b"".join(handles)
        buf = (C.c_uint8 * len(blob)).from_buffer_copy(blob)
        check(_lib.lib().orbf_exchange_peer_open(self._h, buf))

    def exchange_shutdown(self):
        check(_lib.lib().orbf_exchange_shutdown(self._h))

    @property
    def ahead_depth(self):
        return _lib.lib().orbf_ahead_depth(self._h)

    @property
    def exchange_world(self):
        return _lib.lib().orbf_exchange_active(self._h)

    @property
    def exchange_placement(self):
        return _lib.lib().orbf_exchange_placement(self._h)

    def debug_exchange_timing(self, on=True):
        check(_lib.lib().orbf_debug_exchange_timing(self._h, 1 if on else 0))

    def debug_exchange_redos(self):
        return int(_lib.lib().orbf_debug_exchange_redos(self._h))

    def debug_exchange_us(self):
        out = (C.c_float * 2)()
        check(_lib.lib().orbf_debug_exchange_us(self._h, out))
        return float(out[0]), float(out[1])

    def peek_block(self, images):
        arr, self._keep_peek = self._image_array(images, self._imgs)
        p = C.c_void_p(); nb = C.c_size_t(); rows = C.c_int()
        check(_lib.lib().orbf_peek_block(self._h, arr, C.byref(p), C.byref(nb), C.byref(rows)))
        return (p.value, nb.value, rows.value) if p.value else None

    def export_features(self):
        from ._lib import DeviceFeatures
        d = DeviceFeatures()
        check(_lib.lib().orbf_export_features(self._h, C.byref(d)))
        return d

    def _image_array(self, images, slot):
        if type(images) is self._arr_type:
            return images, []
        try:
            key = tuple(images)
            arr = self._img_cache.get(key)
        except TypeError:
            key = arr = None
        if arr is None:
            if key is not None and all(isinstance(im, tuple) for im in images):
                arr = (FImage * self.n_cams)()
                self._fill(arr, images)
                if len(self._img_cache) < 256:
                    self._img_cache[key] = arr
                return arr, []
            arr = slot
            return arr, self._fill(arr, images)
        return arr, []

    def prefetch(self, next_images):
        if not hasattr(self, "_next_imgs"):
            self._next_imgs = (FImage * self.n_cams)()
        if not hasattr(self, "_next_keep"):
            self._next_keep = []
        arr, keep = self._image_array(next_images, self._next_imgs)
        if keep:
            self._next_keep = (self._next_keep + [keep])[-4:]
        check(_lib.lib().orbf_prefetch(self._h, arr))

    def run_stream(self, ring, t0, steps, ahead, announced_upto, motion, th_low, ratio):
        from ._lib import FStreamStats
        key = id(ring)
        cached = getattr(self, "_ring_cache", None)
        if cached is None or cached[0] != key:
            arr = (FImage * (len(ring) * self.n_cams))()
            for t, images in enumerate(ring):
                sub = (FImage * self.n_cams).from_address(C.addressof(arr) + t * self.n_cams * C.sizeof(FImage))
                self._fill(sub, images)
            self._ring_cache = cached = (key, arr, ring)
        st = FStreamStats(); upto = C.c_int(announced_upto)
        mo = FMotion(*motion)
        self._step_seq += 1
        check(_lib.lib().orbf_run_stream(self._h, cached[1], len(ring), t0, steps, ahead, C.byref(upto), C.byref(mo), th_low,
                                         C.c_float(ratio), C.byref(st)))
        return (dict(features=st.features, temporal_matches=st.temporal_matches, cross_accepted=st.cross_accepted,
                     digest=st.digest, seconds=st.seconds), upto.value)

    def step(self, images, queries=None, flags=0, copy=True, motion=None):
        self.begin(images, queries, flags, motion)
        return self.end(copy)

    def begin(self, images, queries=None, flags=0, motion=None):
        arr, self._keep = self._image_array(images, self._imgs)
        ready = self._ready
        self._step_seq += 1
        if motion is not None:
            mo = self._motion_cache.get(motion)
            if mo is None:
                mo = self._motion_cache[motion] = FMotion(*motion)
            check(_lib.lib().orbf_step_motion_begin(self._h, arr, C.byref(mo), flags, C.byref(ready)))
            self._nq = None
        else:
            nq = 0 if queries is None else len(queries)
            if nq:
                queries = np.ascontiguousarray(queries, QUERY_DTYPE)
            self._keep.append(queries)
            check(_lib.lib().orbf_step_begin(self._h, arr, ptr(queries) if nq else None, nq, flags, C.byref(ready)))
            self._nq = nq
        return bool(ready.value)

# ... 93 lines not shown
```

Before: 26030 frames/s.

## Pre-bind next motion search launch args and fast-path tagged result strip

After: 25590 frames/s. 0.983x the previous value.

```diff
diff --git a/include/orb_debug.h b/include/orb_debug.h
--- a/include/orb_debug.h
+++ b/include/orb_debug.h
@@ -43,6 +43,23 @@
 int orbf_debug_exchange_us(const orbf_frontend* f, float* out2);
 long orbf_debug_exchange_redos(const orbf_frontend* f);
 
+
+#define ORBF_STAGED_LAUNCHED 0
+#define ORBF_STAGED_NQ_LATE 1
+#define ORBF_STAGED_EVENT_WAIT 2
+#define ORBF_STAGED_GENERAL 3
+#define ORBF_GENERAL_NOT_STAGED 0
+#define ORBF_GENERAL_DROPPED 1
+#define ORBF_GENERAL_NOT_MOTION 2
+#define ORBF_GENERAL_IMAGES 3
+#define ORBF_GENERAL_FLAGS 4
+#define ORBF_GENERAL_NO_QUERIES 5
+#define ORBF_GENERAL_FORM 6
+#define ORBF_GENERAL_STALE 7
+#define ORBF_STAGED_COUNTERS 11
+int orbf_debug_staged(const orbf_frontend* f, long long* counters , float* first_launch_us);
+int orbf_debug_staged_ask(orbf_frontend* f, int ask);
+
 #ifdef __cplusplus
 }
 #endif
diff --git a/multi_orb_slam_amd/_lib.py b/multi_orb_slam_amd/_lib.py
--- a/multi_orb_slam_amd/_lib.py
+++ b/multi_orb_slam_amd/_lib.py
@@ -242,6 +242,8 @@
     L.orbf_debug_exchange_timing.argtypes = [vp, C.c_int]
     L.orbf_debug_exchange_us.argtypes = [vp, C.POINTER(C.c_float)]
     L.orbf_debug_exchange_redos.argtypes = [vp]; L.orbf_debug_exchange_redos.restype = C.c_long
+    L.orbf_debug_staged.argtypes = [vp, C.POINTER(C.c_longlong), C.POINTER(C.c_float)]
+    L.orbf_debug_staged_ask.argtypes = [vp, C.c_int]
     L.orbf_exchange_init_loopback.argtypes = [vp, i32, i32, i32]
     L.orbf_exchange_shutdown.argtypes = [vp]
     L.orbf_exchange_peer_handle_bytes.argtypes = []; L.orbf_exchange_peer_handle_bytes.restype = C.c_size_t
diff --git a/multi_orb_slam_amd/csrc/extractor.hip b/multi_orb_slam_amd/csrc/extractor.hip
--- a/multi_orb_slam_amd/csrc/extractor.hip
+++ b/multi_orb_slam_amd/csrc/extractor.hip
@@ -2548,6 +2548,11 @@
     const unsigned oldest = (ex->run_seq - (unsigned)ex->inflight) & 1u;
     return ex->h_oct[oldest * (ex->n_cams + 1) + ex->n_cams];
 }
+int orbx_peek_count(const orbx_extractor* ex, int cam) {
+    if (!ex || ex->inflight == 0 || cam < 0 || cam >= ex->n_cams) return -1;
+    const unsigned oldest = (ex->run_seq - (unsigned)ex->inflight) & 1u;
+    return ex->h_oct[oldest * (ex->n_cams + 1) + cam];
+}
 void* orbx_done_event(const orbx_extractor* ex) { return ex ? (void*)ex->ev_done[(ex->run_seq - 1u) & 1u] : nullptr; }
 
 static inline const L0Src* l0_table(const orbx_extractor* ex) { return ex->l0_on ? (const L0Src*)ex->d_l0.p : nullptr; }
diff --git a/multi_orb_slam_amd/csrc/frame_sink.h b/multi_orb_slam_amd/csrc/frame_sink.h
--- a/multi_orb_slam_amd/csrc/frame_sink.h
+++ b/multi_orb_slam_amd/csrc/frame_sink.h
@@ -22,6 +22,7 @@
 
 extern "C" void* orbx_done_event(const orbx_extractor* ex);
 extern "C" int orbx_peek_status(const orbx_extractor* ex);
+extern "C" int orbx_peek_count(const orbx_extractor* ex, int cam);
 
 typedef int (*orbx_tail_fn)(void* user, void* stream);
 extern "C" int orbx_set_chain_tail(orbx_extractor* ex, orbx_tail_fn fn, void* user, int tag);
diff --git a/multi_orb_slam_amd/csrc/frontend.hip b/multi_orb_slam_amd/csrc/frontend.hip
--- a/multi_orb_slam_amd/csrc/frontend.hip
+++ b/multi_orb_slam_amd/csrc/frontend.hip
@@ -116,7 +116,33 @@
     std::vector<int32_t> prev_cam_of;
     std::vector<float> scale_factors;
     std::chrono::steady_clock::time_point t_entry;
+    struct Staged {
+        bool valid = false;
+        int why = ORBF_GENERAL_NOT_STAGED;
+        int set = -1;
+        orbm_frame* fr = nullptr;
+        const orbm_frame* prev = nullptr;
+        bool nq_bound = false; int nq = 0;
+    } staged;
+    morb::BoundSearch* bound = nullptr;
+    bool begin_asks = true;
+    long long staged_counts[ORBF_STAGED_COUNTERS] = {};
+    float first_launch_us = 0.f;
+    struct AheadCount { bool on = false; int th_low = 0; float ratio = 0.f; const int32_t* dist = nullptr; int n = -1, value = 0; } ahead;
+    std::vector<int32_t> prev_counts;
+    bool prev_cam_of_valid = false;
 };
+
+static void staged_drop(orbf_frontend* f, int why) { f->staged.valid = false; f->staged.why = why; }
+static const int32_t* prev_cam_of(orbf_frontend* f) {
+    if (!f->prev_cam_of_valid) {
+        f->prev_cam_of.resize(f->prev_n);
+        for (int c = 0, g = 0; c < (int)f->prev_counts.size(); ++c)
+            for (int k = 0; k < f->prev_counts[c] && g < f->prev_n; ++k) f->prev_cam_of[g++] = c;
+        f->prev_cam_of_valid = true;
+    }
+    return f->prev_cam_of.data();
+}
 
 static int getenv_int(const char* name, int dflt) { const char* e = getenv(name); return e ? atoi(e) : dflt; }
 
@@ -135,6 +161,7 @@
     f->ex = f->exs[0];
     if (!rc) rc = orbx_set_inplace_level0(f->exs[0], 1);
     if (!rc) rc = orbm_create(device, &f->mt);
+    f->bound = morb::bound_search_new();
     if (rc) { orbf_destroy(f); return rc; }
     f->d_depth.assign(n_cams, nullptr); f->depth_stride.assign(n_cams, 0); f->counts.assign(n_cams, 0);
     { const char* pe = getenv("MORB_POLL"); f->poll_ok = !(pe && atoi(pe) == 0); }
@@ -186,6 +213,7 @@
     for (int e = 0; e < orbf_frontend::NEX_ALL; ++e) if (f->exs[e]) orbx_destroy(f->exs[e]);
     for (int k = 0; k < orbf_frontend::NSETS; ++k) { f->rs[k].kps.release(); f->rs[k].desc.release(); f->rs[k].ur.release(); f->rs[k].depth.release(); f->rs[k].unx.release(); f->rs[k].uny.release(); f->rs[k].cross.release(); }
     f->h_queries.release(); f->h_match.release();
+    morb::bound_search_free(f->bound); f->bound = nullptr;
     if (f->ev_extracted) (void)hipEventDestroy(f->ev_extracted);
     for (int k = 0; k < orbf_frontend::NSETS; ++k) if (f->ev_ready[k]) (void)hipEventDestroy(f->ev_ready[k]);
     for (int k = 0; k < orbf_frontend::NSETS; ++k) if (f->ev_cross[k]) (void)hipEventDestroy(f->ev_cross[k]);
@@ -198,6 +226,7 @@
 int orbf_set_depth(orbf_frontend* f, int cam, const float* d_depth, int stride_floats) {
     MORB_ARG(f && cam >= 0 && cam < f->n_cams);
     f->d_depth[cam] = d_depth; f->depth_stride[cam] = stride_floats;
+    staged_drop(f, ORBF_GENERAL_DROPPED);
     return ORB_OK;
 }
 
@@ -215,6 +244,7 @@
 int orbf_configure(orbf_frontend* f, float mbf, int th_high, int check_orientation) {
     MORB_ARG(f && th_high >= 0 && th_high <= 256);
     f->mbf = mbf; f->th_high = th_high; f->check_ori = check_orientation ? 1 : 0;
+    staged_drop(f, ORBF_GENERAL_DROPPED);
     return ORB_OK;
 }
 
@@ -228,6 +258,7 @@
 int orbf_step(orbf_frontend* f, const orbf_image* images, const orbm_query* queries, int nq, int flags, orbf_result* out) {
     MORB_ARG(f && images && out && nq >= 0 && (nq == 0 || queries));
     f->t_entry = std::chrono::steady_clock::now();
+    staged_drop(f, ORBF_GENERAL_NOT_MOTION);
     return orbf_step_impl(f, images, queries, nq, flags, out, false);
 }
 
@@ -236,6 +267,8 @@
 int orbf_reset(orbf_frontend* f) {
     MORB_ARG(f != nullptr);
     f->prev_n = 0; f->announced.clear(); f->overlap_ok = true;
+    f->prev_counts.clear(); f->prev_cam_of_valid = false;
+    staged_drop(f, ORBF_GENERAL_DROPPED);
     if (f->pending.active) {
         if (f->pending.fr && !f->pending.fr_persistent) { (void)hipStreamSynchronize(f->mt->stream); orbm_frame_destroy(f->pending.fr); }
         f->pending.active = false; f->pending.fr = nullptr;
@@ -268,6 +301,7 @@
     if (const char* e = getenv("MORB_EXCHANGE_PLACEMENT")) { if (!strcmp(e, "inline")) placement = 1; }
     if (f->x_one_comm) placement = 1;
     f->x_broken = false;
+    staged_drop(f, ORBF_GENERAL_DROPPED);
     f->x_placement = placement;
     f->mt->side_inline = true;
     f->x_next = f->step_seq;
@@ -292,6 +326,17 @@
     return ORB_OK;
 }
 long orbf_debug_exchange_redos(const orbf_frontend* f) { return f ? f->x_redos : -1; }
+int orbf_debug_staged(const orbf_frontend* f, long long* counters, float* first_launch_us) {
+    MORB_ARG(f && counters);
+    for (int k = 0; k < ORBF_STAGED_COUNTERS; ++k) counters[k] = f->staged_counts[k];
+    if (first_launch_us) *first_launch_us = f->first_launch_us;
+    return ORB_OK;
+}
+int orbf_debug_staged_ask(orbf_frontend* f, int ask) {
+    MORB_ARG(f != nullptr);
+    f->begin_asks = ask != 0;
+    return ORB_OK;
+}
 int orbf_debug_exchange_us(const orbf_frontend* f, float* out2) {
     MORB_ARG(f && out2);
     out2[0] = f->x_us[0]; out2[1] = f->x_us[1];
@@ -371,6 +416,7 @@
 
 int orbf_exchange_shutdown(orbf_frontend* f) {
     MORB_ARG(f != nullptr);
+    staged_drop(f, ORBF_GENERAL_DROPPED);
     x_stop(f);
     if (!f->xcomm) {
         if (f->xpeer) { (void)hipSetDevice(f->device); morb::peer_close(f->xpeer); f->xpeer = nullptr; }
@@ -566,14 +612,22 @@
 static void begin_failed(orbf_frontend* f) {
     if (f->pending.seq_taken && f->step_seq == f->pending.seq + 1) f->step_seq = f->pending.seq;
     f->pending.active = false; f->pending.seq_taken = false;
+    staged_drop(f, ORBF_GENERAL_DROPPED);
+}
+
+static int begin_checked(orbf_frontend* f, const orbf_image* images, const orbm_query* queries, int nq, int flags,
+                         bool queries_in_pinned, int* block_ready, const orbf_motion* motion) {
+    if (f->pending.active) { morb::set_error("a step is still pending: orbf_step_end it first"); return ORB_E_ARG; }
+    int rc = orbf_step_begin_impl(f, images, queries, nq, flags, queries_in_pinned, block_ready, motion);
+    if (rc) begin_failed(f);
+    return rc;
 }
 
 int orbf_step_begin(orbf_frontend* f, const orbf_image* images, const orbm_query* queries, int nq, int flags, int* block_ready) {
     MORB_ARG(f && images && nq >= 0 && (nq == 0 || queries));
     f->t_entry = std::chrono::steady_clock::now();
-    int rc = orbf_step_begin_impl(f, images, queries, nq, flags, false, block_ready);
-    if (rc) begin_failed(f);
-    return rc;
+    staged_drop(f, ORBF_GENERAL_NOT_MOTION);
+    return begin_checked(f, images, queries, nq, flags, false, block_ready, nullptr);
 }
 
 static int queries_from_previous_step(orbf_frontend* f, const orbf_motion* motion, int* nq_out);
@@ -581,9 +635,7 @@
 int orbf_step_motion_begin(orbf_frontend* f, const orbf_image* images, const orbf_motion* motion, int flags, int* block_ready) {
     MORB_ARG(f && images && motion);
     f->t_entry = std::chrono::steady_clock::now();
-    int rc = orbf_step_begin_impl(f, images, nullptr, 0, flags, true, block_ready, motion);
-    if (rc) begin_failed(f);
-    return rc;
+    return begin_checked(f, images, nullptr, 0, flags, true, block_ready, motion);
 }
 
 int orbf_step_end(orbf_frontend* f, orbf_result* out) {
@@ -598,7 +650,7 @@
     int rc;
     if ((rc = f->h_queries.reserve((size_t)nq * sizeof(orbm_query)))) return rc;
     const orbf_frontend::ResultSet& R = f->rs[f->cur];
-    return orbm_queries_from_motion(R.kps.p, R.desc.p, R.depth.p, f->prev_cam_of.data(), nq, motion->du, motion->dv, motion->th,
+    return orbm_queries_from_motion(R.kps.p, R.desc.p, R.depth.p, prev_cam_of(f), nq, motion->du, motion->dv, motion->th,
                                     f->scale_factors.data(), f->mbf, reinterpret_cast<orbm_query*>(f->h_queries.p),
                                     R.unx.p, R.uny.p);
 }
@@ -643,7 +695,12 @@
     MORB_ARG(f && images && motion && out && n_cross);
     int rc;
     if (next_images && (rc = orbf_prefetch(f, next_images))) return rc;
-    if ((rc = orbf_step_motion(f, images, motion, flags, out))) return rc;
+    f->ahead.on = true; f->ahead.th_low = th_low; f->ahead.ratio = ratio; f->ahead.n = -1;
+    rc = orbf_step_motion(f, images, motion, flags, out);
+    f->ahead.on = false;
+    if (rc) return rc;
+    if (out->cross_best_dist && f->ahead.n == out->n_total && f->ahead.dist == out->cross_best_dist) *n_cross = f->ahead.value;
+    else
     *n_cross = out->cross_best_dist ? orbm_count_ratio_accepted(out->cross_best_dist, out->cross_second_dist, out->n_total, th_low, ratio) : -1;
     return *n_cross < -1 ? *n_cross : ORB_OK;
 }
@@ -816,6 +873,7 @@
 }
 
 static int orbf_drain(orbf_frontend* f) {
+    staged_drop(f, ORBF_GENERAL_DROPPED);
     MORB_HIP(hipSetDevice(f->device));
     if (f->xcomm) { const int xr = x_wait_stream(f, nullptr); if (xr) return xr; }
     if (f->xcomm && f->x_placement == 3 && !f->inflight.empty()) f->x_spare_until = std::max(f->x_spare_until, f->x_next - 1);
@@ -843,6 +901,100 @@
 
 static int queries_from_previous_step(orbf_frontend* f, const orbf_motion* motion, int* nq_out);
 
+static MotionSrc motion_src_of(const orbf_frontend* f, const FrameBufs* B, float du, float dv, float th) {
+    MotionSrc ms{B->d_x.p, B->d_y.p, B->d_depth.p, B->d_ang.p, B->d_oct.p, (const uint4*)B->d_desc.p, B->d_cam_start.p, f->n_cams,
+                 {}, du, dv, th, f->mbf, nullptr};
+    for (size_t l = 0; l < f->scale_factors.size(); ++l) ms.scale[l] = f->scale_factors[l];
+    return ms;
+}
+static void motion_job(orbf_frontend* f, orbf_frontend::Pending& P, const orbm_frame* prev_frame) {
+    P.J = SearchJob{nullptr, f->q_host.data(), P.nq, nullptr, false, 0.f, f->th_high, f->check_ori, 64, false};
+    P.J.msrc = &P.ms;
+    if ((int)prev_frame->cam_start.size() == f->n_cams + 1)
+    {
+        for (int c = 0; c < f->n_cams; ++c) P.J.q_cam_max = std::max(P.J.q_cam_max, prev_frame->cam_start[c + 1] - prev_frame->cam_start[c]);
+        P.J.q_cam_start = prev_frame->cam_start.data();
+    }
+    P.J.want_tags = f->poll_ok;
+}
+
+static int enqueue_announced(orbf_frontend* f, orbf_frontend::Pending& P, hipStream_t st);
+
+static void stage_next_search(orbf_frontend* f) {
+    orbf_frontend::Pending& P = f->pending;
+    orbf_frontend::Staged& S = f->staged;
+    S.valid = false; S.why = ORBF_GENERAL_NOT_STAGED;
+    if (f->inflight.empty() || !P.async_path || !P.fr_persistent || !P.fr || f->xcomm || !f->overlap_ok ||
+        !f->motion_on_device || !f->poll_ok || P.fr->n_cams != f->n_cams || f->scale_factors.size() > 16 || !f->bound)
+        return;
+    const orbf_frontend::InFlight& I = f->inflight.front();
+    orbm_frame* fr = f->pframe[I.set];
+    if (!fr || I.set == P.set) return;
+    int nq = -1;
+    if (P.ext_done && orbx_peek_status(f->exs[P.e]) == 0) {
+        nq = 0;
+        for (int c = 0; c < f->n_cams; ++c) nq += std::max(0, orbx_peek_count(f->exs[P.e], c));
+        if (nq == 0 || nq > f->cap_total) return;
+    }
+    const MotionSrc ms = motion_src_of(f, P.fr->b, 0.f, 0.f, 0.f);
+    SearchJob J{fr, nullptr, nq > 0 ? nq : f->cap_total, nullptr, false, 0.f, f->th_high, f->check_ori, 64, false};
+    J.msrc = &ms; J.want_tags = true;
+    if (morb::search_bind(f->mt, J, J.nq, f->bound) != 1) { S.why = ORBF_GENERAL_FORM; return; }
+    S.set = I.set; S.fr = fr; S.prev = P.fr; S.nq_bound = nq > 0; S.nq = nq;
+    S.valid = true;
+}
+
+static int begin_staged(orbf_frontend* f, const orbf_image* images, int flags, int* block_ready, const orbf_motion* motion, int* why) {
+    orbf_frontend::Staged& S = f->staged;
+    orbf_frontend::Pending& P = f->pending;
+    orbm_matcher* m = f->mt;
+    if (!S.valid) { *why = S.why; return 1; }
+    *why = ORBF_GENERAL_STALE;
+    if (f->inflight.empty() || f->inflight.front().set != S.set || f->pframe[S.set] != S.fr || f->last_frame != S.prev || f->last_frame_owned ||
+        f->xcomm || S.prev->n_total != f->prev_n || (S.nq_bound && S.nq != f->prev_n) || !morb::search_bound_current(m, f->bound))
+        return 1;
+    orbf_frontend::InFlight& I = f->inflight.front();
+    if (!same_images(I.images, images, f->n_cams) || !same_content(I.fp, images, f->n_cams)) { *why = ORBF_GENERAL_IMAGES; return 1; }
+    const bool do_cross = !(flags & ORBF_SKIP_CROSS);
+    if (do_cross && !f->rs[S.set].cross_valid) { *why = ORBF_GENERAL_FLAGS; return 1; }
+    const int nq = f->prev_n;
+    if (nq <= 0) { *why = ORBF_GENERAL_NO_QUERIES; return 1; }
+    if (!I.done && f->begin_asks) {
+        if (hipEventQuery(f->ev_ready[S.set]) == hipSuccess) I.done = true; else (void)hipGetLastError();
+    }
+    if (!I.done) MORB_HIP(hipStreamWaitEvent(m->stream, f->ev_ready[S.set], 0));
+    SearchJob L{S.fr, nullptr, nq, nullptr, false, 0.f, f->th_high, f->check_ori, 64, false};
+    int rc = morb::search_launch_bound(m, f->bound, L, nq, motion->du, motion->dv, motion->th);
+    if (rc) return rc;
+    f->first_launch_us = std::chrono::duration<float, std::micro>(std::chrono::steady_clock::now() - f->t_entry).count();
+    ++f->staged_counts[ORBF_STAGED_LAUNCHED];
+    if (!S.nq_bound) ++f->staged_counts[ORBF_STAGED_NQ_LATE];
+    if (!I.done) ++f->staged_counts[ORBF_STAGED_EVENT_WAIT];
+    S.valid = false; S.why = ORBF_GENERAL_NOT_STAGED;
+    const orbm_frame* prev_frame = f->last_frame;
+    f->last_frame = nullptr; f->last_frame_owned = false;
+    P.images.assign(images, images + f->n_cams);
+    P.nq = nq; P.flags = flags; P.from_motion = true;
+    P.seq = f->step_seq++; P.seq_taken = true;
+    P.set = I.set; P.e = I.e; P.W = I.W; P.H = I.H; P.ext_done = I.done;
+    f->inflight.pop_front();
+    P.use_ms = true; P.motion = *motion;
+    P.ms = motion_src_of(f, prev_frame->b, motion->du, motion->dv, motion->th);
+    f->q_host.resize((size_t)nq);
+    motion_job(f, P, prev_frame);
+    P.J.cur = S.fr; P.J.cap = 64;
+    P.J.seq = L.seq; P.J.form = L.form; P.J.device_path = L.device_path; P.J.pollable = L.pollable; P.J.multi = false;
+    P.async_path = true; P.fr = S.fr; P.fr_persistent = true; P.n = S.fr->n_total;
+    P.cross_from_set = do_cross; P.forked = false;
+    P.cams.resize(f->n_cams);
+    P.block_ready = P.ext_done && orbx_peek_status(f->exs[P.e]) == 0;
+    if ((rc = enqueue_announced(f, P, m->stream))) return rc;
+    P.t_enqueued = std::chrono::steady_clock::now();
+    P.active = true;
+    if (block_ready) *block_ready = P.block_ready ? 1 : 0;
+    return 0;
+}
+
 static int orbf_step_begin_impl(orbf_frontend* f, const orbf_image* images, const orbm_query* queries, int nq, int flags,
                                 bool queries_in_pinned, int* block_ready, const orbf_motion* motion) {
     orbf_frontend::Pending& P = f->pending;
@@ -852,6 +1004,16 @@
     MORB_HIP(hipSetDevice(f->device));
     orbm_matcher* m = f->mt;
     int rc, went_async = 0;
+    {
+        int why = ORBF_GENERAL_NOT_MOTION;
+        if (motion && !queries) {
+            rc = begin_staged(f, images, flags, block_ready, motion, &why);
+            if (rc <= 0) return rc;
+        }
+        ++f->staged_counts[ORBF_STAGED_GENERAL + why];
+        staged_drop(f, ORBF_GENERAL_NOT_STAGED);
+        f->first_launch_us = 0.f;
+    }
     const orbm_frame* prev_frame = f->last_frame && !f->last_frame_owned ? f->last_frame : nullptr;
     if (f->last_frame && f->last_frame_owned) orbm_frame_destroy(f->last_frame);
     f->last_frame = nullptr; f->last_frame_owned = false;
@@ -896,12 +1058,9 @@
     }
     if (motion && f->motion_on_device && prev_frame && f->prev_n > 0 && prev_frame->n_total == f->prev_n &&
         prev_frame->n_cams == f->n_cams && f->scale_factors.size() <= 16) {
-        const FrameBufs* B = prev_frame->b;
         nq = f->prev_n; P.nq = nq;
         P.use_ms = true; P.motion = *motion;
-        P.ms = MotionSrc{B->d_x.p, B->d_y.p, B->d_depth.p, B->d_ang.p, B->d_oct.p, (const uint4*)B->d_desc.p, B->d_cam_start.p, f->n_cams,
-                         {}, motion->du, motion->dv, motion->th, f->mbf, nullptr};
-        for (size_t l = 0; l < f->scale_factors.size(); ++l) P.ms.scale[l] = f->scale_factors[l];
+        P.ms = motion_src_of(f, prev_frame->b, motion->du, motion->dv, motion->th);
         f->q_host.resize((size_t)nq);
         queries = nullptr;
     } else if (motion) {
@@ -915,16 +1074,12 @@
         if (!queries_in_pinned) memcpy(f->h_queries.p, queries, (size_t)nq * sizeof(orbm_query));
         f->h_queries.publish();
     }
-    P.J = SearchJob{nullptr, P.use_ms ? f->q_host.data() : reinterpret_cast<const orbm_query*>(f->h_queries.p), nq, nullptr, false, 0.f,
-                    f->th_high, f->check_ori, 64, false};
-    P.J.q_dev = nq && !P.use_ms ? reinterpret_cast<const orbm_query*>(f->h_queries.dp) : nullptr;
-    P.J.msrc = P.use_ms ? &P.ms : nullptr;
-    if (P.use_ms && (int)prev_frame->cam_start.size() == f->n_cams + 1)
-    {
-        for (int c = 0; c < f->n_cams; ++c) P.J.q_cam_max = std::max(P.J.q_cam_max, prev_frame->cam_start[c + 1] - prev_frame->cam_start[c]);
-        P.J.q_cam_start = prev_frame->cam_start.data();
-    }
-    P.J.want_tags = f->poll_ok;
+    if (P.use_ms) motion_job(f, P, prev_frame);
+    else {
+        P.J = SearchJob{nullptr, reinterpret_cast<const orbm_query*>(f->h_queries.p), nq, nullptr, false, 0.f, f->th_high, f->check_ori, 64, false};
+        P.J.q_dev = nq ? reinterpret_cast<const orbm_query*>(f->h_queries.dp) : nullptr;
+        P.J.want_tags = f->poll_ok;
+    }
     if ((rc = f->h_match.reserve(std::max(f->cap_total, 1)))) return rc;
     P.async_path = went_async != 0;
     P.block_ready = false;
@@ -932,6 +1087,7 @@
         P.ext_done = true;
         P.block_ready = orbx_peek_status(f->exs[P.e]) == 0;
     } else { P.ext_done = false; (void)hipGetLastError(); }
+    if (P.use_ms && P.async_path && (rc = morb::search_reserve(m, f->cap_total, f->cap_total, 64))) return rc;
     if ((rc = step_enqueue(f, P, true))) return rc;
     P.active = true;
     if (block_ready) *block_ready = P.block_ready ? 1 : 0;
@@ -1042,7 +1198,14 @@
         if ((rc = exchange_issue(f, P.seq, fr, st, false, P.images.data()))) return rc;
         m->foreign_work = true;
     }
-    while (P.async_path && first_attempt && f->overlap_ok && !f->announced.empty() && (int)f->inflight.size() < std::max(f->n_ex, 2)) {
+    if (first_attempt && (rc = enqueue_announced(f, P, st))) return rc;
+    P.t_enqueued = std::chrono::steady_clock::now();
+    return ORB_OK;
+}
+
+static int enqueue_announced(orbf_frontend* f, orbf_frontend::Pending& P, hipStream_t st) {
+    int rc;
+    while (P.async_path && f->overlap_ok && !f->announced.empty() && (int)f->inflight.size() < std::max(f->n_ex, 2)) {
         if (f->xcomm && P.seq + 1 + (long)f->inflight.size() <= f->x_spare_until) break;
         const int prev_e = f->inflight.empty() ? P.e : f->inflight.back().e;
         const int e2 = f->n_ex > 1 ? (prev_e + 1) % f->n_ex : 0;
@@ -1064,10 +1227,10 @@
             f->announced.pop_front();
         } else {
             f->overlap_ok = false;
+            staged_drop(f, ORBF_GENERAL_DROPPED);
             f->announced.clear();
         }
     }
-    P.t_enqueued = std::chrono::steady_clock::now();
     return ORB_OK;
 }
 
@@ -1095,7 +1258,7 @@
             orbf_frontend* f = static_cast<orbf_frontend*>(ctx);
             const orbf_frontend::Pending& P = f->pending;
             const orbf_frontend::ResultSet& Rp = f->rs[f->cur];
-            (void)orbm_queries_from_motion(Rp.kps.p, Rp.desc.p, Rp.depth.p, f->prev_cam_of.data(), P.nq, P.motion.du, P.motion.dv, P.motion.th,
+            (void)orbm_queries_from_motion(Rp.kps.p, Rp.desc.p, Rp.depth.p, prev_cam_of(f), P.nq, P.motion.du, P.motion.dv, P.motion.th,
                                            f->scale_factors.data(), f->mbf, f->q_host.data(), Rp.unx.p, Rp.uny.p);
         }
     };
@@ -1104,9 +1267,21 @@
         if (P.flags & ORBF_NO_QUERY_RECORDS) { P.J.q_fill = &FillQ::run; P.J.q_fill_ctx = f; }
         else { FillQ::run(f); have_records = true; }
     }
-    if (!f->inflight.empty() && !f->inflight.front().done) {
+    auto ask_next_ready = [&] {
+        if (f->inflight.empty() || f->inflight.front().done) return;
         if (hipEventQuery(f->ev_ready[f->inflight.front().set]) == hipSuccess) f->inflight.front().done = true;
         else (void)hipGetLastError();
+    };
+    ask_next_ready();
+    stage_next_search(f);
+    f->ahead.n = -1;
+    if (f->ahead.on && P.async_path && P.cross_from_set && P.ext_done && !f->cross_pending[P.set] && !f->xcomm && orbx_peek_status(ex) == 0) {
+        int n_now = 0;
+        for (int c = 0; c < f->n_cams; ++c) n_now += std::max(0, orbx_peek_count(ex, c));
+        if (n_now > 0 && n_now <= f->cap_total) {
+            const int v = orbm_count_ratio_accepted(R.cross.b.p, R.cross.s.p, n_now, f->ahead.th_low, f->ahead.ratio);
+            if (v >= 0) { f->ahead.n = n_now; f->ahead.dist = R.cross.b.p; f->ahead.value = v; }
+        }
     }
     for (int attempt = 0; attempt < 2; ++attempt) {
         if (attempt == 1 && (rc = step_enqueue(f, P, false))) return rc;
@@ -1117,6 +1292,7 @@
             volatile int32_t* flag = m->h_match.p;
             for (int spin = 0; spin < 400000; ++spin) {
                 if ((*flag >> 20) == P.J.seq) { polled = true; break; }
+                if ((spin & 63) == 63) ask_next_ready();
                 __builtin_ia32_pause();
             }
         }
@@ -1134,6 +1310,8 @@
             rc = polled ? orbx_finish_completed(ex) : orbx_finish(ex);
             if (rc < 0) return rc;
             if (rc == 1 || rc == 2) {
+                staged_drop(f, ORBF_GENERAL_DROPPED);
+                f->ahead.n = -1;
                 if (rc == 2 || !f->inflight.empty()) {
                     if ((rc = orbf_drain(f))) return rc;
                     f->announced.clear();
@@ -1167,12 +1345,12 @@
     const bool do_cross = !(P.flags & ORBF_SKIP_CROSS) && n > 0;
     rc = search_finish(m, P.J, f->h_match.p, &nmatches);
     if (rc) { if (!P.fr_persistent) orbm_frame_destroy(P.fr); return rc; }
+    if (m->last_form[1] > 0 || m->last_form[0] == ORBM_FORM_HOST) staged_drop(f, ORBF_GENERAL_DROPPED);
     f->last_frame = P.fr; f->last_frame_owned = !P.fr_persistent;
     f->cur = P.set;
     f->prev_n = n;
-    f->prev_cam_of.resize(n);
-    for (int c = 0, g = 0; c < f->n_cams; ++c)
-        for (int k = 0; k < f->counts[c]; ++k) f->prev_cam_of[g++] = c;
+    f->prev_counts.assign(f->counts.begin(), f->counts.end()); f->prev_cam_of_valid = false;
+    if (f->staged.valid && f->staged.nq_bound && f->staged.nq != n) staged_drop(f, ORBF_GENERAL_STALE);
     out->n_queries = nq;
     if (P.use_ms && (P.flags & ORBF_NO_QUERY_RECORDS)) have_records = P.J.q_fill == nullptr;
     out->queries = !P.use_ms ? reinterpret_cast<const orbm_query*>(f->h_queries.p) : (have_records && nq > 0 ? f->q_host.data() : nullptr);
@@ -1230,7 +1408,7 @@
 
 static int orbf_step_impl(orbf_frontend* f, const orbf_image* images, const orbm_query* queries, int nq, int flags,
                           orbf_result* out, bool queries_in_pinned, const orbf_motion* motion) {
-    int rc = orbf_step_begin_impl(f, images, queries, nq, flags, queries_in_pinned, nullptr, motion);
-    if (rc) { begin_failed(f); return rc; }
+    int rc = begin_checked(f, images, queries, nq, flags, queries_in_pinned, nullptr, motion);
+    if (rc) return rc;
     return orbf_step_end_impl(f, out);
 }
diff --git a/multi_orb_slam_amd/csrc/matcher_internal.h b/multi_orb_slam_amd/csrc/matcher_internal.h
--- a/multi_orb_slam_amd/csrc/matcher_internal.h
+++ b/multi_orb_slam_amd/csrc/matcher_internal.h
@@ -199,6 +199,13 @@
 int search_enqueue(orbm_matcher* m, SearchJob& J, bool queries_already_on_device = false);
 int search_finish(orbm_matcher* m, SearchJob& J, int32_t* match_of_feature, int* nmatches);
 int phases_resolve(unsigned long long* out64);
+struct BoundSearch;
+BoundSearch* bound_search_new();
+void bound_search_free(BoundSearch* B);
+int search_bind(orbm_matcher* m, const SearchJob& J, int nq_max, BoundSearch* B);
+int search_reserve(orbm_matcher* m, int n, int nq, int cap);
+bool search_bound_current(const orbm_matcher* m, const BoundSearch* B);
+int search_launch_bound(orbm_matcher* m, BoundSearch* B, SearchJob& J, int nq, float du, float dv, float th);
 int cross_enqueue_to(hipStream_t st, const uint8_t* d_desc, int n, const int* d_cam_start, int n_cams, int q_off, int nq,
                      const int* d_n, int* o_idx, int* o_best, int* o_second, void* scratch);
 int cross_enqueue(orbm_matcher* m, hipStream_t st, const uint8_t* d_desc, int n, const int* d_cam_start, int n_cams, int q_off,
diff --git a/multi_orb_slam_amd/csrc/search.hip b/multi_orb_slam_amd/csrc/search.hip
--- a/multi_orb_slam_amd/csrc/search.hip
+++ b/multi_orb_slam_amd/csrc/search.hip
@@ -12,6 +12,7 @@
 #include "hamming_dev.h"
 #include "project_dev.h"
 #include "resolve_dev.h"
+#include "tag_strip.h"
 
 using namespace morb;
 
@@ -963,6 +964,28 @@
 #endif
 }
 
+static int project_args(orbm_matcher* m, const orbm_frame* f, int nq, int cap, int gate_right, int with_dist, int transposed,
+                        const uint8_t* d_occupied, int* d_topk, int short_th, const float* d_inv_sigma2, const orbm_query* q_device_visible,
+                        int2* d_qmeta, const orbm_window* d_win2, const MotionSrc* msrc, bool msrc_records, ProjectArgs* out) {
+    int rc;
+    if ((rc = m->d_queries.reserve((size_t)nq * sizeof(orbm_query))) || (rc = m->d_i0.reserve((size_t)nq * cap)) ||
+        (rc = m->d_u16.reserve((size_t)nq * cap)) || (rc = m->d_i1.reserve(nq)))
+        return rc;
+    ProjectArgs& A = *out;
+    A.F = f->dev(); A.q = q_device_visible ? q_device_visible : (const orbm_query*)m->d_queries.p; A.nq = nq; A.cap = cap;
+    A.gate_right = gate_right; A.with_dist = with_dist; A.transposed = transposed;
+    A.cand_idx = m->d_i0.p; A.cand_dist = m->d_u16.p; A.cand_count = m->d_i1.p;
+    A.occupied = d_occupied; A.topk = d_topk; A.short_th = short_th; A.inv_sigma2 = d_inv_sigma2; A.qmeta = d_qmeta; A.win2 = d_win2;
+    if (msrc) {
+        A.from_motion = 1; A.ms = *msrc; A.q = nullptr;
+        A.ms.rec_out = msrc_records ? (orbm_query*)m->d_queries.p : nullptr;
+    }
+    return ORB_OK;
+}
+static inline void project_launch(hipStream_t st, const ProjectArgs& A) {
+    hipLaunchKernelGGL(k_project, dim3((A.nq + 3) / 4), dim3(256), 0, st, A);
+}
+
 static int run_project(orbm_matcher* m, const orbm_frame* f, const orbm_query* q, int nq, int cap, int gate_right,
                        int with_dist, bool upload_queries, bool to_host, int transposed = 0,
                        const uint8_t* d_occupied = nullptr, int* d_topk = nullptr, int short_th = 256,
@@ -970,24 +993,16 @@
                        const orbm_window* d_win2 = nullptr, const SideJob* side = nullptr, const MotionSrc* msrc = nullptr,
                        bool msrc_records = false, MergeJob* defer_merge = nullptr) {
     int rc;
-    if ((rc = m->d_queries.reserve((size_t)nq * sizeof(orbm_query))) || (rc = m->d_i0.reserve((size_t)nq * cap)) ||
-        (rc = m->d_u16.reserve((size_t)nq * cap)) || (rc = m->d_i1.reserve(nq)))
+    ProjectArgs A;
+    if ((rc = project_args(m, f, nq, cap, gate_right, with_dist, transposed, d_occupied, d_topk, short_th, d_inv_sigma2, q_device_visible,
+                           d_qmeta, d_win2, msrc, msrc_records, &A)))
         return rc;
     if (upload_queries)
         MORB_HIP(hipMemcpyAsync(m->d_queries.p, q, (size_t)nq * sizeof(orbm_query), hipMemcpyHostToDevice, m->stream));
-    ProjectArgs A;
-    A.F = f->dev(); A.q = q_device_visible ? q_device_visible : (const orbm_query*)m->d_queries.p; A.nq = nq; A.cap = cap;
-    A.gate_right = gate_right; A.with_dist = with_dist; A.transposed = transposed;
-    A.cand_idx = m->d_i0.p; A.cand_dist = m->d_u16.p; A.cand_count = m->d_i1.p;
-    A.occupied = d_occupied; A.topk = d_topk; A.short_th = short_th; A.inv_sigma2 = d_inv_sigma2; A.qmeta = d_qmeta; A.win2 = d_win2;
-    if (msrc) {
-        A.from_motion = 1; A.ms = *msrc; A.q = nullptr;
-        A.ms.rec_out = msrc_records ? (orbm_query*)m->d_queries.p : nullptr;
-    }
     if (side) {
         if ((rc = launch_project_side(m->stream, A, *side, defer_merge))) return rc;
     } else {
-        hipLaunchKernelGGL(k_project, dim3((nq + 3) / 4), dim3(256), 0, m->stream, A);
+        project_launch(m->stream, A);
     }
     MORB_HIP(hipGetLastError());
     if (to_host) {
@@ -1160,13 +1175,55 @@
     return ORB_OK;
 }
 
+constexpr size_t LDS_LIMIT = 150 * 1024;
+static int resolve_cam_env() { static const int v = [] { const char* e = getenv("MORB_RS_PER_CAMERA"); return e ? atoi(e) : 1; }(); return v; }
+static int resolve_mono_mode() { static const int v = [] { const char* e = getenv("MORB_RESOLVE_MONO"); return e ? atoi(e) : 2; }(); return v; }
+
+struct MonoLaunch {
+    FrameDev F; const int2* qmeta; int nq, cap;
+    const int* cand_idx; const uint16_t* cand_dist; const int* cand_count; const uint8_t* occ; const float* f_angle;
+    int th_high, check_ori; const int* topk; int* match; int* status; int tagb;
+    MergeJob MJ; int merge_blocks;
+    int rq; bool ang; size_t lds; int worklist;
+};
+static bool mono_takes(int n, int nq) { return resolve_mono_mode() != 0 && n < 65535 && MonoLds(n, nq, false).bytes() <= LDS_LIMIT; }
+static void mono_bind_nq(MonoLaunch& R, int nq) {
+    const int n = R.F.n_total;
+    R.nq = nq;
+    R.rq = nq <= 2048 ? 2 : 4;
+    R.ang = MonoLds(n, nq, true).bytes() <= LDS_LIMIT;
+    R.lds = MonoLds(n, nq, R.ang).bytes();
+    R.worklist = resolve_mono_mode() == 2 && nq > 2048 ? 1 : 0;
+}
+static MonoLaunch mono_bound(orbm_matcher* m, const orbm_frame* cur, int nq, int cap, const uint8_t* d_occ, int th_high, int check_ori) {
+    MonoLaunch R;
+    R.F = cur->dev(); R.qmeta = (const int2*)m->d_qmeta.p; R.cap = cap;
+    R.cand_idx = (const int*)m->d_i0.p; R.cand_dist = (const uint16_t*)m->d_u16.p; R.cand_count = (const int*)m->d_i1.p; R.occ = d_occ;
+    R.f_angle = (const float*)cur->b->d_ang.p; R.th_high = th_high; R.check_ori = check_ori; R.topk = (const int*)m->d_claim.p;
+    R.match = m->h_match.dp + 4; R.status = m->h_match.dp; R.tagb = 0;
+    R.MJ = MergeJob{nullptr, nullptr, nullptr, 0, 0, nullptr, nullptr, nullptr, nullptr}; R.merge_blocks = 0;
+    mono_bind_nq(R, nq);
+    return R;
+}
+static int mono_form(const MonoLaunch& R) {
+    return R.rq == 2 ? (R.ang ? ORBM_FORM_MONO2_ANG : ORBM_FORM_MONO2) : (R.worklist ? ORBM_FORM_MONO4_WORKLIST : ORBM_FORM_MONO4_WAVES);
+}
+static void mono_launch(hipStream_t st, const MonoLaunch& R) {
+#define MORB_MONO_LAUNCH(RQ_, ANG_)                                                                                                          \
+    hipLaunchKernelGGL((k_resolve_mono<RQ_, ANG_>), dim3(1 + R.merge_blocks), dim3(1024), R.lds, st, R.F, R.qmeta, R.nq, R.cap, R.cand_idx, \
+                       R.cand_dist, R.cand_count, R.occ, R.f_angle, R.th_high, R.check_ori, 4096, R.topk, R.match, R.status, R.tagb, R.MJ,   \
+                       R.worklist)
+    if (R.rq == 2) { if (R.ang) MORB_MONO_LAUNCH(2, true); else MORB_MONO_LAUNCH(2, false); }
+    else { if (R.ang) MORB_MONO_LAUNCH(4, true); else MORB_MONO_LAUNCH(4, false); }
+#undef MORB_MONO_LAUNCH
+}
+
 int morb::search_enqueue(orbm_matcher* m, SearchJob& J, bool queries_already_on_device) {
     const int n = J.cur->n_total;
     J.device_path = false; J.pollable = false; J.multi = false;
     J.form = ORBM_FORM_NONE;
     if (J.nq == 0 || n == 0) return ORB_OK;
     J.form = ORBM_FORM_HOST;
-    constexpr size_t LDS_LIMIT = 150 * 1024;
     const JacobiLds jacobi(n, J.nq);
     const bool multi = jacobi.bytes(false) > LDS_LIMIT;
     if (m->host_resolve || J.nq > RESOLVE_MAX_Q) return ORB_OK;
@@ -1194,7 +1251,7 @@
     J.side = nullptr;
     J.seq = 0;
     if (J.want_tags) { m->resolve_seq = m->resolve_seq % 2047 + 1; J.seq = m->resolve_seq; }
-    static const int cam_env = [] { const char* e = getenv("MORB_RS_PER_CAMERA"); return e ? atoi(e) : 1; }();
+    const int cam_env = resolve_cam_env();
     const int cams_min_q = cam_env > 1 ? cam_env : 0x7fffffff;
     int nf_cap = 0, q_cam_max = J.q_cam_max;
     QRanges QR; QR.n = 0;
@@ -1276,10 +1333,7 @@
                        nq, cap, (const int*)m->d_i0.p, (const uint16_t*)m->d_u16.p, (const int*)m->d_i1.p, d_occ,            \
                        (const float*)cur->b->d_ang.p, th_high, nnratio, J.points ? 0 : J.check_ori, 256, m->d_choice.p,      \
                        (const int*)m->d_claim.p, m->h_match.dp + 4, m->h_match.dp, J.seq << 20)
-    static const int mono_mode = [] { const char* e = getenv("MORB_RESOLVE_MONO"); return e ? atoi(e) : 2; }();
-    const bool mono_env = mono_mode != 0;
-    const int mono_worklist = mono_mode == 2 && nq > 2048 ? 1 : 0;
-    const bool will_mono = !J.points && mono_env && n < 65535 && MonoLds(n, nq, false).bytes() <= LDS_LIMIT;
+    const bool will_mono = !J.points && mono_takes(n, nq);
     if (MJ.S > 1 && !will_mono && !cams_fit) { if ((rc = launch_merge(m->stream, MJ))) return rc; MJ.S = 0; }
     int merge_blocks = 0;
     auto carry_merge = [&]() -> int {
@@ -1297,25 +1351,75 @@
         MJ.S = 0;
         J.form = ORBM_FORM_CAMS;
     } else if (will_mono) {
-        const bool ang = MonoLds(n, nq, true).bytes() <= LDS_LIMIT;
-        const size_t ml = MonoLds(n, nq, ang).bytes();
-#define MORB_MONO_LAUNCH(RQ_, ANG_)                                                                                                       \
-        hipLaunchKernelGGL((k_resolve_mono<RQ_, ANG_>), dim3(1 + merge_blocks), dim3(1024), ml, m->stream, cur->dev(), (const int2*)m->d_qmeta.p, nq, cap, \
-                           (const int*)m->d_i0.p, (const uint16_t*)m->d_u16.p, (const int*)m->d_i1.p, d_occ,                                \
-                           (const float*)cur->b->d_ang.p, th_high, J.check_ori, 4096, (const int*)m->d_claim.p, m->h_match.dp + 4,          \
-                           m->h_match.dp, J.seq << 20, MJ, mono_worklist)
         if ((rc = carry_merge())) return rc;
-        if (nq <= 2048) { if (ang) MORB_MONO_LAUNCH(2, true); else MORB_MONO_LAUNCH(2, false); }
-        else { if (ang) MORB_MONO_LAUNCH(4, true); else MORB_MONO_LAUNCH(4, false); }
+        MonoLaunch R = mono_bound(m, cur, nq, cap, d_occ, th_high, J.check_ori);
+        R.tagb = J.seq << 20; R.MJ = MJ; R.merge_blocks = merge_blocks;
+        mono_launch(m->stream, R);
         MJ.S = 0;
-        J.form = nq <= 2048 ? (ang ? ORBM_FORM_MONO2_ANG : ORBM_FORM_MONO2) : (mono_worklist ? ORBM_FORM_MONO4_WORKLIST : ORBM_FORM_MONO4_WAVES);
-#undef MORB_MONO_LAUNCH
+        J.form = mono_form(R);
     } else if (ldsq) { if (J.points) MORB_RESOLVE_LAUNCH(true, true); else MORB_RESOLVE_LAUNCH(false, true); J.form = ORBM_FORM_JACOBI_LDSQ; }
     else { if (J.points) MORB_RESOLVE_LAUNCH(true, false); else MORB_RESOLVE_LAUNCH(false, false); J.form = ORBM_FORM_JACOBI; }
 #undef MORB_RESOLVE_LAUNCH
     MORB_HIP(hipGetLastError());
     J.device_path = true;
     J.pollable = J.seq != 0;
+    return ORB_OK;
+}
+
+struct morb::BoundSearch { ProjectArgs A; MonoLaunch R; int nq_max; };
+static bool search_room(const orbm_matcher* m, int n, int nq, int cap) {
+    const size_t q = (size_t)nq;
+    return m->d_choice.cap >= q && m->d_claim.cap >= (size_t)(2 * RESOLVE_K + 1) * q && m->d_match.cap >= (size_t)n && m->d_status.cap >= 4 &&
+           m->h_match.cap >= (size_t)n + 4 && m->d_occ.cap >= (size_t)std::max(n, 16) && m->d_qmeta.cap >= q &&
+           m->d_queries.cap >= q * sizeof(orbm_query) && m->d_i0.cap >= q * cap && m->d_u16.cap >= q * cap && m->d_i1.cap >= q;
+}
+int morb::search_reserve(orbm_matcher* m, int n, int nq, int cap) {
+    int rc;
+    if ((rc = m->d_choice.reserve(nq)) || (rc = m->d_claim.reserve((size_t)(2 * RESOLVE_K + 1) * nq)) || (rc = m->d_match.reserve(n)) ||
+        (rc = m->d_status.reserve(4)) || (rc = m->h_match.reserve((size_t)n + 4)) || (rc = m->d_occ.reserve(std::max(n, 16))) ||
+        (rc = m->d_qmeta.reserve(nq)) || (rc = m->d_queries.reserve((size_t)nq * sizeof(orbm_query))) || (rc = m->d_i0.reserve((size_t)nq * cap)) ||
+        (rc = m->d_u16.reserve((size_t)nq * cap)) || (rc = m->d_i1.reserve(nq)))
+        return rc;
+    return ORB_OK;
+}
+morb::BoundSearch* morb::bound_search_new() { return new BoundSearch(); }
+void morb::bound_search_free(BoundSearch* B) { delete B; }
+
+int morb::search_bind(orbm_matcher* m, const SearchJob& J, int nq_max, BoundSearch* B) {
+    const int n = J.cur->n_total, cap = J.cap;
+    if (!J.msrc || J.points || J.occupied || J.occ_dev || J.win2_dev || J.side || !J.want_tags || m->host_resolve) return 0;
+    if (n <= 0 || nq_max <= 0 || nq_max > RESOLVE_MAX_Q || resolve_cam_env() > 1) return 0;
+    if (JacobiLds(n, nq_max).bytes(false) > LDS_LIMIT || !mono_takes(n, nq_max)) return 0;
+    if (!search_room(m, n, nq_max, cap)) return 0;
+    int rc;
+    if ((rc = search_reserve(m, n, nq_max, cap))) return rc;
+    if ((rc = project_args(m, J.cur, nq_max, cap, 1, 1, 1, nullptr, m->d_claim.p, J.th_high, nullptr, nullptr, m->d_qmeta.p,
+                           nullptr, J.msrc, false, &B->A)))
+        return rc;
+    B->R = mono_bound(m, J.cur, nq_max, cap, nullptr, J.th_high, J.check_ori);
+    B->nq_max = nq_max;
+    return 1;
+}
+
+bool morb::search_bound_current(const orbm_matcher* m, const BoundSearch* B) {
+    return B && B->A.cand_idx == m->d_i0.p && B->A.cand_dist == m->d_u16.p && B->A.cand_count == m->d_i1.p && B->A.topk == m->d_claim.p &&
+           B->A.qmeta == m->d_qmeta.p && B->R.status == m->h_match.dp && !m->host_resolve;
+}
+
+int morb::search_launch_bound(orbm_matcher* m, BoundSearch* B, SearchJob& J, int nq, float du, float dv, float th) {
+    MORB_ARG(B && nq > 0 && nq <= B->nq_max);
+    B->A.ms.du = du; B->A.ms.dv = dv; B->A.ms.th = th;
+    if (nq != B->R.nq) {
+        B->A.nq = nq;
+        mono_bind_nq(B->R, nq);
+    }
+    m->resolve_seq = m->resolve_seq % 2047 + 1;
+    B->R.tagb = m->resolve_seq << 20;
+    project_launch(m->stream, B->A);
+    mono_launch(m->stream, B->R);
+    MORB_HIP(hipGetLastError());
+    J.seq = m->resolve_seq; J.side = nullptr; J.multi = false;
+    J.form = mono_form(B->R); J.device_path = true; J.pollable = true;
     return ORB_OK;
 }
 
@@ -1366,10 +1470,8 @@
         return host_resolve(m, J.cur, J.q, J.nq, J.occupied, J.points, J.nnratio, J.th_high, J.check_ori, J.cap, match_of_feature, nmatches, J.win2_dev);
     }
     if (J.seq) {
-        for (int g = 0; g < n; ++g) {
-            const int v = word(4 + g, 2);
-            if (v == -3) { morb::set_error("resolve results never arrived"); return ORB_E_HIP; }
-            match_of_feature[g] = v;
+        if (tag_strip(m->h_match.p + 4, n, J.seq, 2, match_of_feature, [&](int g) { return word(4 + g, 2); }) != 0) {
+            morb::set_error("resolve results never arrived"); return ORB_E_HIP;
         }
     } else if (match_of_feature != m->h_match.p + 4) memcpy(match_of_feature, m->h_match.p + 4, (size_t)n * 4);
     *nmatches = m->last_status[1];
diff --git a/multi_orb_slam_amd/csrc/tag_strip.h b/multi_orb_slam_amd/csrc/tag_strip.h
--- /dev/null
+++ b/multi_orb_slam_amd/csrc/tag_strip.h
@@ -0,0 +1,43 @@
+#pragma once
+#include <cstdint>
+#include <cstring>
+
+namespace morb {
+
+constexpr int TAG_SHIFT = 20;
+constexpr int32_t TAG_VALUE_MASK = 0xfffff;
+constexpr int TAG_LINE_WORDS = 16;
+constexpr int TAG_NEVER = -3;
+
+static inline void tag_load(const int32_t* src, int k, int32_t* w) {
+    __asm__ __volatile__("" ::: "memory");
+    memcpy(w, src, (size_t)k * sizeof(int32_t));
+    __asm__ __volatile__("" ::: "memory");
+}
+
+template <class WaitWord>
+static inline int tag_strip(const int32_t* src, int n, int seq, int bias, int32_t* out, WaitWord&& wait_word) {
+    int i = 0;
+    while (i < n) {
+        const uintptr_t a = reinterpret_cast<uintptr_t>(src + i);
+        int k = TAG_LINE_WORDS - (int)((a & 63u) / sizeof(int32_t));
+        if (k > n - i) k = n - i;
+        int32_t w[TAG_LINE_WORDS];
+        tag_load(src + i, k, w);
+        int32_t miss = 0;
+        for (int j = 0; j < k; ++j) miss |= (w[j] >> TAG_SHIFT) ^ seq;
+        if (!miss) {
+            for (int j = 0; j < k; ++j) out[i + j] = (w[j] & TAG_VALUE_MASK) - bias;
+        } else {
+            for (int j = 0; j < k; ++j) {
+                const int v = ((w[j] >> TAG_SHIFT) == seq) ? (w[j] & TAG_VALUE_MASK) - bias : wait_word(i + j);
+                if (v == TAG_NEVER) return TAG_NEVER;
+                out[i + j] = v;
+            }
+        }
+        i += k;
+    }
+    return 0;
+}
+
+}
diff --git a/multi_orb_slam_amd/frontend.py b/multi_orb_slam_amd/frontend.py
--- a/multi_orb_slam_amd/frontend.py
+++ b/multi_orb_slam_amd/frontend.py
@@ -189,6 +189,17 @@
         out = (C.c_float * 2)()
         check(_lib.lib().orbf_debug_exchange_us(self._h, out))
         return float(out[0]), float(out[1])
+
+    STAGED_GENERAL_REASONS = ("not_staged", "dropped", "not_motion", "images", "flags", "no_queries", "form", "stale")
+
+    def debug_staged(self):
+        cnt = (C.c_longlong * 11)(); us = C.c_float(0)
+        check(_lib.lib().orbf_debug_staged(self._h, cnt, C.byref(us)))
+        return dict(staged=int(cnt[0]), nq_late=int(cnt[1]), event_wait=int(cnt[2]),
+                    general={k: int(cnt[3 + i]) for i, k in enumerate(self.STAGED_GENERAL_REASONS)}, first_launch_us=float(us.value))
+
+    def debug_staged_ask(self, ask):
+        check(_lib.lib().orbf_debug_staged_ask(self._h, 1 if ask else 0))
 
     def peek_block(self, images):
         arr, self._keep_peek = self._image_array(images, self._imgs)
```
